# devmentality/LEAStereo

Hardware: AMD Instinct MI355X
Metric: stereo pairs/s at 576×960 D=192, 1/2/4/8 GPU; EPE vs reference (higher is better)
Workload: dtype f32; 1 GPU; SceneFlow 576x960 D=192 fp32, batch 1 per GPU (BASELINE configs[1]); height=576, width=960, maxdisp=192, global_batch=1, parallelism=dp1 (pairs sharded over ranks, no collective in the step), launch=hip graph replay

## Files before the change

### include/leastereo_hip.h

```cpp
#ifndef LEASTEREO_HIP_H
#define LEASTEREO_HIP_H

#include <stddef.h>
#include <stdint.h>

#ifdef __cplusplus
extern "C" {
#endif

#define LEA_ABI_VERSION 14

#define LEA_F32 0
#define LEA_BF16 1

#define LEA_OK 0
#define LEA_E_INVALID 1001
#define LEA_E_UNSUPPORTED 1002

#define LEA_RELU 1u
#define LEA_RESIDUAL 2u
#define LEA_PAIR_SUM 4u

int lea_abi_version(void);
const char* lea_last_error(void);
// ... 107 lines not shown
                             const uint8_t* exclude, int64_t exclude_bstride, int B, int C,
                             int H, int W, float c1, float c2, const double* sums,
                             const float* scales, float* ddisp, int64_t ddisp_bstride,
                             void* stream);

size_t lea_disparity_refine_workspace_bytes(int B, int H, int W);
int lea_disparity_refine_f32(const float* guide, int64_t guide_bstride, const float* disp,
                             const float* conf, const uint8_t* exclude, int B, int C, int H,
                             int W, float lambda, float sigma, int iterations, void* workspace,
                             float* refined, float* support, void* stream);

#define LEA_LR_SPECKLE 3
size_t lea_disparity_speckle_workspace_bytes(int B, int H, int W);
int lea_disparity_speckle_f32(const float* disp, const uint8_t* exclude, int B, int H, int W,
                              float max_diff, int max_size, float fill, void* workspace,
                              int32_t* labels, int32_t* size, uint8_t* state, float* filtered,
                              void* stream);


size_t lea_conv3d_packed_elems_bf16(int cout, int cin, int k);
int lea_conv3d_pack_weights_bf16(const float* w, void* packed, int cout, int cin, int k,
                                 void* stream);

int lea_conv3d_bnrelu_bf16(const void* x, int64_t x_bstride, const void* x2, int64_t x2_bstride,
                           int cin2, const void* w_packed, const float* scale, const float* shift,
                           const void* residual, int64_t r_bstride, void* y, int64_t y_bstride,
                           int B, int cin, int cout, int D, int H, int W, int k, unsigned flags,
                           void* stream);

int lea_conv3d_bnrelu_costvolume_bf16(const void* left, const void* right, int64_t f_bstride,
                                      const void* w_packed, const float* scale, const float* shift,
                                      void* y, int64_t y_bstride, int B, int C, int cout, int D3,
                                      int H, int W, unsigned flags, void* stream);


const char* lea_conv3d_kernel_name_bf16(int B, int cout, int cin, int D, int H, int W, int k,
                                        int costvolume);

int lea_conv3d_bf16_pair_supported(int B, int cin, int cout, int D, int H, int W);

int lea_conv1x1_resampled_bf16(const void* x, int64_t x_bstride, int Di, int Hi, int Wi,
                               const void* w_packed, const float* scale, const float* shift,
                               void* y, int64_t y_bstride, int B, int cin, int cout, int D, int H,
                               int W, unsigned flags, void* stream);

int lea_resample3d_trilinear_bf16(const void* x, int64_t x_bstride, void* y, int64_t y_bstride,
                                  int B, int C, int Di, int Hi, int Wi, int Do, int Ho, int Wo,
                                  int align_corners, const float* scale, const float* shift,
                                  unsigned flags, void* stream);


int lea_to_c8_bf16(const float* x, int64_t x_bstride, void* y, int64_t y_bstride, int B, int C,
                   int64_t vol, void* stream);
int lea_from_c8_bf16(const void* x, int64_t x_bstride, float* y, int64_t y_bstride, int B, int C,
                     int64_t vol, void* stream);


size_t lea_conv2d_packed_elems_bf16(int cout, int cin);
int lea_conv2d_pack_weights_bf16(const float* w, void* packed, int cout, int cin, void* stream);
int lea_conv2d_bnrelu_bf16(const void* x, int64_t x_bstride, const void* w_packed,
                           const float* scale, const float* shift, const void* residual,
                           int64_t r_bstride, void* y, int64_t y_bstride, int B, int cin, int cout,
                           int H, int W, unsigned flags, void* stream);

size_t lea_conv3d_wino_packed_floats(int cout, int cin);
int lea_conv3d_wino_pack_weights(const float* w, float* packed, int cout, int cin, void* stream);
int lea_conv3d_bnrelu_wino(const void* x, int64_t x_bstride, const void* x2, int64_t x2_bstride,
                           int cin2, const float* w_packed, const float* scale, const float* shift,
                           const void* residual, int64_t r_bstride, void* y, int64_t y_bstride,
                           int B, int cin, int cout, int D, int H, int W, unsigned flags, int dtype,
                           void* stream);
int lea_conv3d_bnrelu_costvolume_wino(const void* left, const void* right, int64_t f_bstride,
                                      const float* w_packed, const float* scale,
                                      const float* shift, void* y, int64_t y_bstride, int B, int C,
                                      int cout, int D3, int H, int W, unsigned flags, int dtype,
                                      void* stream);
const char* lea_conv3d_wino_kernel_name(int B, int cin, int cout, int D, int H, int W, int costvolume);
int lea_conv3d_wino_down2_supported(int B, int cin, int cout, int D, int H, int W);
const char* lea_conv3d_wino_down2_kernel_name(int B, int cin, int cout, int D, int H, int W);
int lea_conv3d_bnrelu_wino_down2(const void* x, int64_t x_bstride, const float* w_packed,
                                 const float* scale, const float* shift, void* y, int64_t y_bstride,
                                 int B, int cin, int cout, int D, int H, int W, unsigned flags, int dtype,
                                 void* stream);

int lea_cv_stem_split_weights(const float* w, float* wl, float* wr, int cout, int C, void* stream);
int lea_cv_stem_combine(const void* lmaps, int64_t l_bstride, const void* rmaps, int64_t r_bstride,
                        const float* scale, const float* shift, void* y, int64_t y_bstride, int B,
                        int cout, int D3, int H, int W, unsigned flags, int dtype, void* stream);
int lea_cv_stem_down2_supported(int cout, int D3, int H, int W, int dtype);
int lea_cv_stem_combine_down2(const void* lmaps, int64_t l_bstride, const void* rmaps, int64_t r_bstride,
                              const float* scale, const float* shift, void* y, int64_t y_bstride,
                              void* y2, int64_t y2_bstride, int B, int cout, int D3, int H, int W,
                              unsigned flags, int dtype, void* stream);


size_t lea_standardize_workspace_bytes(int B);
int lea_standardize_crop_u8(const void* left, const void* right, int B, int H, int W,
                            int pix_stride, float* out_left, float* out_right, int crop_h,
                            int crop_w, void* workspace, void* stream);

size_t lea_train_transform_workspace_bytes(int B);
int lea_train_transform_u8(const void* left, const void* right, int B, int H, int W, int pix_stride,
                           const float* disp_left, const float* disp_right, const int* params,
                           float* out_left, float* out_right, float* out_target, int crop_h,
                           int crop_w, float maxdisp, int* n_valid, void* workspace, void* stream);


size_t lea_standardize_tiles_workspace_bytes(void);
int lea_standardize_tiles_u8(const void* left, const void* right, int H, int W, int pix_stride,
                             const int* origins, int N, float* out_left, float* out_right, int tile_h,
                             int tile_w, void* workspace, void* stream);

int lea_tile_blend_f32(const float* tiles, int64_t tile_bstride, const int* ys, int ny, const int* xs,
                       int nx, int tile_h, int tile_w, int guard_y0, int guard_y1, int guard_x0,
                       int guard_x1, int ramp, float* out, int H, int W, int* n_uncovered, void* stream);

size_t lea_disparity_metrics_workspace_bytes(int B, int H, int W);
int lea_disparity_metrics(const float* pred, int64_t pred_bstride, const float* gt,
                          int64_t gt_bstride, int B, int H, int W, float maxdisp, int round_pred,
                          int z_shift, int thr1, int thr2, int thr3, unsigned char* correct,
                          double* out, void* workspace, void* stream);


size_t lea_conv3d_wgrad_workspace_bytes(int B, int cin, int cout, int D, int H, int W, int k);
int lea_conv3d_wgrad(const float* x, const float* dz, float* dw, void* workspace, size_t ws_bytes,
                     int B, int cin, int cout, int D, int H, int W, int k, void* stream);

size_t lea_conv2d_wgrad_workspace_bytes(int B, int cin, int cout, int H, int W);
int lea_conv2d_wgrad(const float* x, const float* dz, float* dw, void* workspace, size_t ws_bytes,
                     int B, int cin, int cout, int H, int W, void* stream);

int lea_conv2d_s3_backward_data(const float* dz, const float* w, float* dx, int B, int cin, int cout,
                                int Hi, int Wi, void* stream);
size_t lea_conv2d_s3_wgrad_workspace_bytes(int B, int cin, int cout, int Hi, int Wi);
int lea_conv2d_s3_wgrad(const float* x, const float* dz, float* dw, void* workspace, size_t ws_bytes,
                        int B, int cin, int cout, int Hi, int Wi, void* stream);

int lea_conv3d_flip_weights(const float* w, float* wt, int cout, int cin, int k, void* stream);

size_t lea_bn_workspace_bytes(int C);
int lea_bn_forward_f32(const float* z, float* y, int B, int C, int64_t V, const float* gamma,
                       const float* beta, float* running_mean, float* running_var, float momentum,
                       float eps, int training, unsigned flags, float* mean, float* invstd,
                       void* workspace, void* stream);

int lea_bn_backward_f32(const float* dy, const float* y, const float* z, float* dz, int B, int C,
                        int64_t V, const float* gamma, const float* mean, const float* invstd,
                        int training, unsigned flags, float* dgamma, float* dbeta, void* workspace,
                        void* stream);

size_t lea_resample3d_backward_workspace_bytes(int B, int C, int Di, int Hi, int Wi, int Do, int Ho,
                                               int Wo);
int lea_resample3d_trilinear_backward(const float* dy, float* dx, void* workspace, size_t ws_bytes,
                                      int B, int C, int Di, int Hi, int Wi, int Do, int Ho, int Wo,
                                      int align_corners, void* stream);

int lea_disparity_regression_backward(const float* cost, const float* disp, const float* dout,
                                      float* dV, int B, int D3, int H3, int W3, int maxdisp,
                                      void* stream);

int lea_build_cost_volume_backward(const float* dcost, float* dleft, float* dright, int B, int C,
                                   int H, int W, int D3, void* stream);

#ifdef __cplusplus
}
#endif
// ... 2 lines not shown
```

### leastereo_amd/_lib.py

```python
from __future__ import annotations

import ctypes
import os
import threading

LIB_PATH = os.environ.get(
    "LEASTEREO_HIP_LIB",
    os.path.join(os.path.dirname(os.path.abspath(__file__)), "libleastereo_hip.so"))

ABI_VERSION = 14
LEA_F32 = 0
LEA_BF16 = 1
LEA_RELU = 1
LEA_RESIDUAL = 2
LEA_PAIR_SUM = 4
LEA_E_INVALID = 1001

_p = ctypes.c_void_p
_i = ctypes.c_int
_i64 = ctypes.c_int64
_u = ctypes.c_uint

SIGNATURES = {
    "lea_abi_version": (_i, []),
    "lea_last_error": (ctypes.c_char_p, []),
    "lea_build_cost_volume": (_i, [_p, _p, _p, _i, _i, _i, _i, _i, _i, _p]),
    "lea_conv3d_packed_floats": (ctypes.c_size_t, [_i, _i, _i]),
    "lea_conv3d_pack_weights": (_i, [_p, _p, _i, _i, _i, _p]),
    "lea_conv3d_bnrelu": (_i, [_p, _i64, _p, _i64, _i, _p, _p, _p, _p, _i64, _p, _i64,
                               _i, _i, _i, _i, _i, _i, _i, _u, _i, _p]),
    "lea_conv3d_bnrelu_resampled": (_i, [_p, _i64, _i, _i, _i, _p, _p, _p, _p, _i64, _p, _i64,
                                         _i, _i, _i, _i, _i, _i, _i, _u, _i, _p]),
    "lea_conv3d_kernel_name": (ctypes.c_char_p, [_i, _i, _i, _i, _i, _i, _i]),
    "lea_conv3d_set_tile_override": (_i, [_i, _i, _i]),
    "lea_conv3d_bnrelu_costvolume": (_i, [_p, _p, _i64, _p, _p, _p, _p, _i64, _i, _i, _i, _i, _i,
                                          _i, _u, _i, _p]),
    "lea_conv3d_costvolume_kernel_name": (ctypes.c_char_p, [_i, _i, _i, _i, _i]),
    "lea_conv2d_packed_floats": (ctypes.c_size_t, [_i, _i]),
    "lea_conv2d_pack_weights": (_i, [_p, _p, _i, _i, _p]),
    "lea_conv2d_bnrelu": (_i, [_p, _i64, _p, _p, _p, _p, _i64, _p, _i64, _i, _i, _i, _i, _i, _u,
                               _i, _p]),
    "lea_conv2d_kernel_name": (ctypes.c_char_p, [_i, _i, _i, _i]),
    "lea_conv2d_s3_bnrelu": (_i, [_p, _i64, _p, _p, _p, _p, _i64, _i, _i, _i, _i, _i, _u, _i, _p]),
    "lea_feature_stem_bnrelu": (_i, [_p, _i64, _p, _p, _p, _p, _p, _p, _p, _i64, _i, _i, _i, _i, _i, _i,
                                     _i, _p]),
    "lea_resample3d_trilinear": (_i, [_p, _i64, _p, _i64, _i, _i, _i, _i, _i, _i, _i, _i,
                                      _i, _p, _p, _u, _i, _p]),
    "lea_tapsum_workspace_bytes": (ctypes.c_size_t, [_i, _i, _i, _i, _i]),
    "lea_tapsum_upsample": (_i, [_p, _i64, _p, _i64, _i, _i, _i, _i, _i, _i, _i, _i, _p, _p, _u,
                                 _p, _i, _p]),
    "lea_disparity_regression": (_i, [_p, _p, _i, _i, _i, _i, _i, _i, _p]),
    "lea_disparity_regression_stats": (_i, [_p, _p, _p, _p, _p, _i, _i, _i, _i, _i, _i, _i, _p]),
    "lea_disparity_regression_right": (_i, [_p, _p, _i, _i, _i, _i, _i, _i, _p]),
    "lea_disparity_lr_check": (_i, [_p, _p, _p, _p, _i, _i, _i, ctypes.c_float, _p]),
    "lea_median5x5_f32": (_i, [_p, _i64, _p, _i64, _i, _i, _i, _i, _p]),
    "lea_edge_loss_workspace_bytes": (ctypes.c_size_t, [_i, _i, _i]),
    "lea_edge_loss_f32": (_i, [_p, _i64, _p, _i64, _p, _i64, _i, _i, _i, ctypes.c_float, _p, _p, _p]),
    "lea_edge_loss_grad_f32": (_i, [_p, _i64, _p, _i64, _p, _i64, _p, _p, _p, _i64, _i, _i, _i,
                                    ctypes.c_float, _p]),
    "lea_photometric_workspace_bytes": (ctypes.c_size_t, [_i, _i, _i]),
    "lea_photometric_f32": (_i, [_p, _i64, _p, _i64, _p, _i64, _p, _i64, _i, _i, _i, _i, ctypes.c_float,
                                 ctypes.c_float, ctypes.c_float, _p, _p, _p, _p, _p]),
    "lea_photometric_grad_f32": (_i, [_p, _i64, _p, _i64, _p, _i64, _p, _i64, _i, _i, _i, _i, ctypes.c_float,
                                      ctypes.c_float, _p, _p, _p, _i64, _p]),
    "lea_disparity_refine_workspace_bytes": (ctypes.c_size_t, [_i, _i, _i]),
    "lea_disparity_refine_f32": (_i, [_p, _i64, _p, _p, _p, _i, _i, _i, _i, ctypes.c_float, ctypes.c_float, _i,
                                      _p, _p, _p, _p]),
    "lea_disparity_speckle_workspace_bytes": (ctypes.c_size_t, [_i, _i, _i]),
    "lea_disparity_speckle_f32": (_i, [_p, _p, _i, _i, _i, ctypes.c_float, _i, ctypes.c_float, _p, _p, _p, _p, _p,
                                       _p]),
    "lea_conv3d_packed_elems_bf16": (ctypes.c_size_t, [_i, _i, _i]),
    "lea_conv3d_pack_weights_bf16": (_i, [_p, _p, _i, _i, _i, _p]),
    "lea_conv3d_bnrelu_bf16": (_i, [_p, _i64, _p, _i64, _i, _p, _p, _p, _p, _i64, _p, _i64,
                                    _i, _i, _i, _i, _i, _i, _i, _u, _p]),
    "lea_conv3d_bnrelu_costvolume_bf16": (_i, [_p, _p, _i64, _p, _p, _p, _p, _i64, _i, _i, _i, _i,
                                               _i, _i, _u, _p]),
    "lea_conv3d_kernel_name_bf16": (ctypes.c_char_p, [_i, _i, _i, _i, _i, _i, _i, _i]),
    "lea_conv3d_bf16_pair_supported": (_i, [_i, _i, _i, _i, _i, _i]),
    "lea_conv3d_bf16_set_tile_override": (_i, [_i, _i, _i]),
    "lea_conv3d_bf16_set_variant": (_i, [_i]),
    "lea_resample3d_trilinear_bf16": (_i, [_p, _i64, _p, _i64, _i, _i, _i, _i, _i, _i, _i, _i,
                                           _i, _p, _p, _u, _p]),
    "lea_resample_bf16_set_batch": (_i, [_i]),
    "lea_resample_bf16_set_cols": (_i, [_i]),
    "lea_conv3d_wino_set_w22": (_i, [_i]),
    "lea_conv3d_bf16_set_pair_split": (_i, [_i]),
    "lea_disparity_set_register_form": (_i, [_i]),
    "lea_tapsum_set_rows": (_i, [_i]),
    "lea_staged_rows": (_i, [_i, _i, _i, _i, _i]),
    "lea_conv1x1_resampled_bf16": (_i, [_p, _i64, _i, _i, _i, _p, _p, _p, _p, _i64, _i, _i, _i, _i, _i,
                                        _i, _u, _p]),
    "lea_to_c8_bf16": (_i, [_p, _i64, _p, _i64, _i, _i, _i64, _p]),
    "lea_conv2d_packed_elems_bf16": (ctypes.c_size_t, [_i, _i]),
    "lea_conv2d_pack_weights_bf16": (_i, [_p, _p, _i, _i, _p]),
    "lea_conv2d_bnrelu_bf16": (_i, [_p, _i64, _p, _p, _p, _p, _i64, _p, _i64, _i, _i, _i, _i, _i,
                                    _u, _p]),
    "lea_from_c8_bf16": (_i, [_p, _i64, _p, _i64, _i, _i, _i64, _p]),
    "lea_conv3d_wino_packed_floats": (ctypes.c_size_t, [_i, _i]),
    "lea_conv3d_wino_pack_weights": (_i, [_p, _p, _i, _i, _p]),
    "lea_conv3d_bnrelu_wino": (_i, [_p, _i64, _p, _i64, _i, _p, _p, _p, _p, _i64, _p, _i64,
                                    _i, _i, _i, _i, _i, _i, _u, _i, _p]),
    "lea_conv3d_bnrelu_costvolume_wino": (_i, [_p, _p, _i64, _p, _p, _p, _p, _i64, _i, _i, _i,
                                               _i, _i, _i, _u, _i, _p]),
    "lea_conv3d_wino_kernel_name": (ctypes.c_char_p, [_i, _i, _i, _i, _i, _i, _i]),
    "lea_conv3d_wino_down2_supported": (_i, [_i, _i, _i, _i, _i, _i]),
    "lea_conv3d_wino_down2_kernel_name": (ctypes.c_char_p, [_i, _i, _i, _i, _i, _i]),
    "lea_conv3d_bnrelu_wino_down2": (_i, [_p, _i64, _p, _p, _p, _p, _i64, _i, _i, _i, _i, _i, _i, _u, _i, _p]),
    "lea_conv3d_wino_set_tile_override": (_i, [_i, _i, _i]),
    "lea_conv3d_wino_set_variant": (_i, [_i]),
    "lea_conv3d_wino2_set_walk": (_i, [_i]),
    "lea_conv3d_wino2_set_halo16": (_i, [_i]),
    "lea_conv3d_wino2_set_lane_halo16": (_i, [_i]),
    "lea_conv3d_wino_set_fence": (_i, [_i]),
    "lea_resample_set_mode": (_i, [_i]),
    "lea_conv2d_set_small": (_i, [_i]),
    "lea_conv2d_kernel_name_cin": (ctypes.c_char_p, [_i, _i, _i, _i, _i]),
    "lea_conv2d_bnrelu_pair": (_i, [_p, _i64, _p, _p, _p, _p, _i64, _p, _i64, _p, _i64, _i, _i, _i, _i, _i,
                                    _i, _u, _p]),
    "lea_conv3d_wino2_set_pipeline": (_i, [_i]),
    "lea_conv3d_wino2p_set_wpre": (_i, [_i]),
    "lea_conv3d_wino44_set": (_i, [_i]),
    "lea_conv3d_wino44_set_upre": (_i, [_i]),
    "lea_conv3d_wino44_set_sched": (_i, [_i]),
    "lea_conv3d_wino44_set_group": (_i, [_i]),
    "lea_conv3d_wino_set_epi_buf": (_i, [_i]),
    "lea_conv3d_set_rs_gather": (_i, [_i]),
    "lea_conv1x1_set_vector": (_i, [_i]),
    "lea_conv3d_bf16_set_stream1x1": (_i, [_i]),
    "lea_conv3d_wino_set_small_cout": (_i, [_i]),
    "lea_conv3d_wino_set_block48": (_i, [_i]),
    "lea_cv_stem_split_weights": (_i, [_p, _p, _p, _i, _i, _p]),
    "lea_cv_stem_combine": (_i, [_p, _i64, _p, _i64, _p, _p, _p, _i64, _i, _i, _i, _i, _i, _u, _i,
                                 _p]),
    "lea_cv_stem_down2_supported": (_i, [_i, _i, _i, _i, _i]),
    "lea_cv_stem_combine_down2": (_i, [_p, _i64, _p, _i64, _p, _p, _p, _i64, _p, _i64, _i, _i, _i, _i, _i,
                                       _u, _i, _p]),
    "lea_standardize_workspace_bytes": (ctypes.c_size_t, [_i]),
    "lea_standardize_crop_u8": (_i, [_p, _p, _i, _i, _i, _i, _p, _p, _i, _i, _p, _p]),
    "lea_train_transform_workspace_bytes": (ctypes.c_size_t, [_i]),
    "lea_train_transform_u8": (_i, [_p, _p, _i, _i, _i, _i, _p, _p, _p, _p, _p, _p, _i, _i,
                                    ctypes.c_float, _p, _p, _p]),
    "lea_standardize_tiles_workspace_bytes": (ctypes.c_size_t, []),
    "lea_standardize_tiles_u8": (_i, [_p, _p, _i, _i, _i, _p, _i, _p, _p, _i, _i, _p, _p]),
    "lea_tile_blend_f32": (_i, [_p, _i64, _p, _i, _p, _i, _i, _i, _i, _i, _i, _i, _i, _p, _i, _i, _p, _p]),
    "lea_disparity_metrics_workspace_bytes": (ctypes.c_size_t, [_i, _i, _i]),
    "lea_disparity_metrics": (_i, [_p, _i64, _p, _i64, _i, _i, _i, ctypes.c_float, _i, _i,
                                   _i, _i, _i, _p, _p, _p, _p]),
    "lea_conv3d_wgrad_workspace_bytes": (ctypes.c_size_t, [_i, _i, _i, _i, _i, _i, _i]),
    "lea_conv3d_wgrad": (_i, [_p, _p, _p, _p, ctypes.c_size_t, _i, _i, _i, _i, _i, _i, _i, _p]),
    "lea_conv2d_wgrad_workspace_bytes": (ctypes.c_size_t, [_i, _i, _i, _i, _i]),
    "lea_conv2d_wgrad": (_i, [_p, _p, _p, _p, ctypes.c_size_t, _i, _i, _i, _i, _i, _p]),
    "lea_conv2d_s3_backward_data": (_i, [_p, _p, _p, _i, _i, _i, _i, _i, _p]),
    "lea_conv2d_s3_wgrad_workspace_bytes": (ctypes.c_size_t, [_i, _i, _i, _i, _i]),
    "lea_conv2d_s3_wgrad": (_i, [_p, _p, _p, _p, ctypes.c_size_t, _i, _i, _i, _i, _i, _p]),
    "lea_conv3d_flip_weights": (_i, [_p, _p, _i, _i, _i, _p]),
    "lea_bn_workspace_bytes": (ctypes.c_size_t, [_i]),
    "lea_bn_forward_f32": (_i, [_p, _p, _i, _i, _i64, _p, _p, _p, _p, ctypes.c_float, ctypes.c_float,
                                _i, _u, _p, _p, _p, _p]),
    "lea_bn_backward_f32": (_i, [_p, _p, _p, _p, _i, _i, _i64, _p, _p, _p, _i, _u, _p, _p, _p, _p]),
    "lea_disparity_regression_backward": (_i, [_p, _p, _p, _p, _i, _i, _i, _i, _i, _p]),
    "lea_build_cost_volume_backward": (_i, [_p, _p, _p, _i, _i, _i, _i, _i, _p]),
    "lea_resample3d_backward_workspace_bytes": (ctypes.c_size_t, [_i, _i, _i, _i, _i, _i, _i, _i]),
    "lea_resample3d_trilinear_backward": (_i, [_p, _p, _p, ctypes.c_size_t, _i, _i, _i, _i, _i, _i, _i, _i,
                                               _i, _p]),
}

_lib = None
_lock = threading.Lock()


class HipKernelError(RuntimeError):
    pass


def load():
    global _lib
    if _lib is not None:
        return _lib
    with _lock:
        if _lib is None:
            if not os.path.exists(LIB_PATH):
                raise HipKernelError(
                    f"{LIB_PATH} not found: build it with `make` (hipcc --offload-arch=gfx950); "
                    "the LEAStereo hot path has no fallback")
            lib = ctypes.CDLL(LIB_PATH)
            for name, (res, args) in SIGNATURES.items():
                fn = getattr(lib, name)
                fn.restype = res
                fn.argtypes = args
            _apply_env_tuning(lib)
# ... 38 lines not shown
```

### leastereo_amd/csrc/conv3d_wino.hip

```cpp
#include "wino_common.h"

namespace lea {
namespace wino {

template <int F, int Q, int MT, int NP, int TD, bool H16 = false>
struct Cfg {
  static constexpr bool DP = MT == 0;
  static constexpr int MTE = DP ? 1 : MT;
  static constexpr int TDA = DP ? 1 : TD;
  static constexpr int NSTEP = DP ? 12 : 9;
  static_assert(!DP || TD == 2, "a depth-paired tile covers two output planes");
  static constexpr int NX = F + 2;
  static constexpr int COP = 16 * MTE;
  static constexpr bool SWZ = (COP % 32) == 0;
  static constexpr int RPG = 16 / Q;
  static constexpr int TW = F * Q;
  static constexpr int TH = 4 * NP * RPG;
  static constexpr int RH = TH + 2, RW = TW + 2;
  static constexpr int PLANE = RH * RW;
  static constexpr int PLANES = TD + 2;
  static constexpr int IMG = PLANES * PLANE;
  static constexpr int XSLOTS = (IMG + 63) / 64;
  static constexpr int CIS = conflict_free_cis<F, Q>(64 * XSLOTS, RW);
  static constexpr int RWA = TW + 8;
  static constexpr int PLANEA = RH * RWA;
  static constexpr int IMGA = PLANES * PLANEA;
  static constexpr int BLK16 = IMGA / 4;
  static constexpr int PIECES16 = (BLK16 + 63) / 64;
  static constexpr int cb2(int c) {
    int base = 1;
    for (int k = 1; k <= c; ++k) {
      const int want = (k & 1 ? 2 : 0) + (k & 2 ? 32 : 0) + 1, lo = base + IMGA;
      base = lo + ((want - lo) % 64 + 64) % 64;
    }
    return base;
  }
  static_assert(!H16 || (Q == 16 && F == 4), "16-byte halo: one tile row per lane group");
  static constexpr int CSH = PIECES16 * 256;
  static constexpr int cbh(int c) { return 1 + c * CSH; }
  static_assert(!H16 || (CSH % 64 == 0 && RWA % 4 == 0 && PLANEA % 4 == 0), "b128 halo map");
  static constexpr int XS = H16 ? (cbh(CIN_B) + 3) / 4 * 4 : CIN_B * CIS;
  static constexpr int RWX = H16 ? RWA : RW;
  static constexpr int PLX = H16 ? PLANEA : PLANE;
  static constexpr int WS = NSTEP * 3 * CIN_B * COP;
  static constexpr int WSLOTS = (WS + 255) / 256;
  static constexpr int STAGE = XS + 256 * WSLOTS;
  static_assert(XS % 4 == 0 && WS % 4 == 0 && RW % 2 == 0 && PLANE % 2 == 0, "aligned LDS regions and b64 reads");
  static_assert(2 * STAGE * 4 * 2 <= 160 * 1024, "two double-buffered workgroups per CU");
};

template <int F, int Q, int MT, int NP, int TD, bool CV, bool H16 = false, bool FENCE = false>
__global__ __launch_bounds__(kConvThreads, 2) void conv3d_wino_kernel(const ConvArgs a) {
  using C = Cfg<F, Q, MT, NP, TD, H16>;
  static_assert(!(CV && H16), "16-byte halo: plain volumes only");
  constexpr int NX = C::NX;
  constexpr int XSLOTS = C::XSLOTS;
  constexpr int XSLOTS_W = (XSLOTS + kConvWaves - 1) / kConvWaves;
  constexpr int WSLOTS = C::WSLOTS;
  constexpr int WSLOTS_W = (WSLOTS + kConvWaves - 1) / kConvWaves;
  __shared__ __attribute__((aligned(16))) float smem[2 * C::STAGE];
  const unsigned lds0 = lds_addr(smem);

  const int tid = threadIdx.x;
  const int lane = tid & 63;
  const int wave = __builtin_amdgcn_readfirstlane(tid >> 6);
  const int nblk = a.nblk;
  const int xcd = blockIdx.x % 8, idx = blockIdx.x / 8;
  const int q8 = nblk / 8, r8 = nblk % 8;
  const int lin = (xcd < r8 ? xcd * (q8 + 1) : r8 * (q8 + 1) + (xcd - r8) * q8) + idx;
  const int spw = a.spw > 0 ? a.spw : 1;
  const int ngz = (a.ndz + spw - 1) / spw;
  const int cob = lin % a.ncob;
  const int rest = lin / a.ncob;
  const int gz = rest % ngz;
  const int tile = (rest / ngz) % a.ntiles;
  const int b = rest / (ngz * a.ntiles);
  const int h0 = (tile / a.tiles_w) * C::TH;
  const int w0 = (tile % a.tiles_w) * C::TW;
  const int dz0 = gz * spw, ngroups = min(spw, a.ndz - dz0);
  const int co0 = cob * C::COP;
  const int nchunks = a.cin / CIN_B;
  const int nitems = ngroups * nchunks;
  const float* wp = a.wp + (long long)cob * nchunks * C::WS;
  const int HW = a.H * a.W;
  const unsigned nrec = (unsigned)(HW * a.D) * 4u;

  unsigned hwo[XSLOTS_W];
  int pln[XSLOTS_W], wco[CV ? XSLOTS_W : 1];
#pragma unroll
  for (int t = 0; t < XSLOTS_W; ++t) {
    const int e = (wave + kConvWaves * t) * 64 + lane;
    unsigned v = 0xFFFFFFF0u;
    int pl = -1000, wc_ = 0;
    if (e < C::IMG) {
      const int p = e / C::PLANE;
      const int r = e - p * C::PLANE;
      const int rr = r / C::RW;
      const int cc = r - rr * C::RW;
      const int h = h0 + rr - 1, w = w0 + cc - 1;
      if ((unsigned)h < (unsigned)a.H && (unsigned)w < (unsigned)a.W) {
        v = (unsigned)(h * a.W + w) * 4u;
        pl = p - 1;
        wc_ = w;
      }
    }
    hwo[t] = v;
    pln[t] = pl;
    if constexpr (CV) wco[t] = wc_;
  }
  unsigned voff[XSLOTS_W], voffr[CV ? XSLOTS_W : 1];
  constexpr int P16 = C::PIECES16, T16 = H16 ? (CIN_B * P16 + kConvWaves - 1) / kConvWaves : 1;
  unsigned hwo16[T16], voff16[T16];
  int pln16[T16];
  bool ok16[T16];
  if constexpr (H16) {
#pragma unroll
    for (int t = 0; t < T16; ++t) {
      const int k = wave + kConvWaves * t, e = 64 * (k % P16) + lane;
      ok16[t] = k < CIN_B * P16 && e < C::BLK16;
      const int p = e / (C::RH * (C::RWA / 4)), r = e - p * (C::RH * (C::RWA / 4));
      const int rr = r / (C::RWA / 4), blk = r - rr * (C::RWA / 4);
      const int h = h0 + rr - 1, w = w0 - 4 + 4 * blk;
      const bool in = ok16[t] && (unsigned)h < (unsigned)a.H && (unsigned)w < (unsigned)a.W;
      hwo16[t] = in ? (unsigned)(h * a.W + w) * 4u : 0xFFFFFFF0u;
      pln16[t] = in ? p - 1 : -1000;
    }
  }
  auto set_group = [&](int d0) {
    if constexpr (H16) {
#pragma unroll
      for (int t = 0; t < T16; ++t) {
        const int d = d0 + pln16[t];
        voff16[t] = (hwo16[t] != 0xFFFFFFF0u && (unsigned)d < (unsigned)a.D)
                        ? hwo16[t] + (unsigned)d * (unsigned)HW * 4u : 0xFFFFFFF0u;
      }
      return;
    }
#pragma unroll
    for (int t = 0; t < XSLOTS_W; ++t) {
      const int d = d0 + pln[t];
      const bool ok = hwo[t] != 0xFFFFFFF0u && (unsigned)d < (unsigned)a.D;
      if constexpr (CV) {
        const bool okc = ok && wco[t] >= d;
// ... 71 lines not shown
  for (int m = 0; m < C::MTE; ++m)
#pragma unroll
    for (int r = 0; r < 4; ++r) {
      const int co = C::DP ? 4 * (ci & 1) + r : co0 + 16 * m + 4 * ci + r;
      const bool cv = co < a.cout;
      sc[m][r] = (cv && a.scale) ? a.scale[co] : 1.f;
      sh[m][r] = (cv && a.shift) ? a.shift[co] : 0.f;
    }

  f32x4 acc[NX][C::TDA][C::MTE][NP];
#pragma unroll
  for (int x = 0; x < NX; ++x)
#pragma unroll
    for (int t = 0; t < C::TDA; ++t)
#pragma unroll
      for (int m = 0; m < C::MTE; ++m)
#pragma unroll
        for (int j = 0; j < NP; ++j) acc[x][t][m][j] = f32x4{0.f, 0.f, 0.f, 0.f};

  const bool relu = a.flags & LEA_RELU, resid = a.flags & LEA_RESIDUAL;
  const long long DHW = (long long)HW * a.D;
  const int w = w0 + F * pq;
  const bool ebuf = F == 4 && (a.flags & kEpiBuf);
  constexpr int NST = C::TDA * NP * C::MTE * 4;
  const int nco = C::DP ? a.cout : min(C::COP, a.cout - co0);
  const __amdgpu_buffer_rsrc_t yrs = block_rsrc(a.y + (long long)b * a.ybs + (long long)co0 * DHW, nco * DHW * 4);
  const __amdgpu_buffer_rsrc_t rrs =
      block_rsrc((resid ? a.res : a.y) + (long long)b * (resid ? a.rbs : a.ybs) + (long long)co0 * DHW, nco * DHW * 4);
  auto epilogue_buf = [&](int d0) {
    unsigned off[C::TDA][NP][C::MTE][4];
#pragma unroll
    for (int t = 0; t < C::TDA; ++t)
#pragma unroll
      for (int j = 0; j < NP; ++j)
#pragma unroll
        for (int m = 0; m < C::MTE; ++m)
#pragma unroll
          for (int r = 0; r < 4; ++r) {
            const int d = C::DP ? d0 + (ci >> 1) : d0 + t;
            const int h = h0 + (wave * NP + j) * C::RPG + pr;
            const int cr = C::DP ? 4 * (ci & 1) + r : 16 * m + 4 * ci + r;
            off[t][j][m][r] = (d < a.D && h < a.H && w < a.W && cr < nco)
                                  ? (unsigned)(cr * DHW + (long long)d * HW + h * a.W + w) * 4u
                                  : kEpiOob;
          }
    f32x4 rv[C::TDA][NP][C::MTE][4];
    if (resid) {
#pragma unroll
      for (int t = 0; t < C::TDA; ++t)
#pragma unroll
        for (int j = 0; j < NP; ++j)
#pragma unroll
          for (int m = 0; m < C::MTE; ++m)
#pragma unroll
            for (int r = 0; r < 4; ++r) rv[t][j][m][r] = buf_load4(rrs, off[t][j][m][r]);
    }
#pragma unroll
    for (int t = 0; t < C::TDA; ++t)
#pragma unroll
      for (int j = 0; j < NP; ++j)
#pragma unroll
        for (int m = 0; m < C::MTE; ++m)
#pragma unroll
          for (int r = 0; r < 4; ++r) {
            constexpr int X3 = NX > 4 ? 3 : 0, X4 = NX > 4 ? 4 : 0;
            const float m0 = 0.25f * acc[0][t][m][j][r];
            const float m1 = (-1.f / 6.f) * acc[1][t][m][j][r], m2 = (-1.f / 6.f) * acc[2][t][m][j][r];
            const float m3 = (1.f / 24.f) * acc[X3][t][m][j][r], m4 = (1.f / 24.f) * acc[X4][t][m][j][r];
            const float m5 = acc[NX - 1][t][m][j][r];
            const float sp = m1 + m2, sm = m1 - m2, tp = m3 + m4, tm = m3 - m4;
            f32x4 y;
            y[0] = (m0 + sp) + tp;
            y[1] = fmaf(2.f, tm, sm);
            y[2] = fmaf(4.f, tp, sp);
            y[3] = fmaf(8.f, tm, sm) + m5;
#pragma unroll
            for (int e = 0; e < 4; ++e) {
              float v = y[e] * sc[m][r] + sh[m][r];
              if (relu) v = fmaxf(v, 0.f);
              y[e] = resid ? v + rv[t][j][m][r][e] : v;
            }
            buf_store4(yrs, off[t][j][m][r], y);
          }
  };
  auto epilogue = [&](int d0) {
#pragma unroll
  for (int t = 0; t < C::TDA; ++t) {
    const int d = C::DP ? d0 + (ci >> 1) : d0 + t;
#pragma unroll
    for (int j = 0; j < NP; ++j) {
      const int h = h0 + (wave * NP + j) * C::RPG + pr;
      if (d >= a.D || h >= a.H || w >= a.W) continue;
      const int nv = min(F, a.W - w);
#pragma unroll
      for (int m = 0; m < C::MTE; ++m)
#pragma unroll
        for (int r = 0; r < 4; ++r) {
          const int co = C::DP ? 4 * (ci & 1) + r : co0 + 16 * m + 4 * ci + r;
          if (co >= a.cout) continue;
          float y[F];
          if constexpr (F == 2) {
            const float m0 = acc[0][t][m][j][r], m1 = 0.5f * acc[1][t][m][j][r];
            const float m2 = 0.5f * acc[2][t][m][j][r], m3 = acc[3][t][m][j][r];
            y[0] = (m0 + m1) + m2;
            y[1] = (m1 - m2) - m3;
          } else {
            const float m0 = 0.25f * acc[0][t][m][j][r];
            const float m1 = (-1.f / 6.f) * acc[1][t][m][j][r], m2 = (-1.f / 6.f) * acc[2][t][m][j][r];
            const float m3 = (1.f / 24.f) * acc[3][t][m][j][r], m4 = (1.f / 24.f) * acc[4][t][m][j][r];
            const float m5 = acc[NX - 1][t][m][j][r];
            const float sp = m1 + m2, sm = m1 - m2, tp = m3 + m4, tm = m3 - m4;
            y[0] = (m0 + sp) + tp;
            y[1] = fmaf(2.f, tm, sm);
            y[F / 2] = fmaf(4.f, tp, sp);
            y[F - 1] = fmaf(8.f, tm, sm) + m5;
          }
#pragma unroll
          for (int e = 0; e < F; ++e) {
            y[e] = y[e] * sc[m][r] + sh[m][r];
            if (relu) y[e] = fmaxf(y[e], 0.f);
          }
          const long long o = (long long)co * DHW + (long long)d * HW + (long long)h * a.W + w;
          float* yp = a.y + (long long)b * a.ybs + o;
          const float* rp = a.res + (long long)b * a.rbs + o;
          const bool vec = nv == F &&
              ((reinterpret_cast<uintptr_t>(yp) | (resid ? reinterpret_cast<uintptr_t>(rp) : 0)) & (4 * F - 1)) == 0;
          if (vec) {
            if constexpr (F == 2) {
              if (resid) {
                const float2 rv = *reinterpret_cast<const float2*>(rp);
                y[0] += rv.x;
                y[1] += rv.y;
              }
              *reinterpret_cast<float2*>(yp) = make_float2(y[0], y[1]);
            } else {
              if (resid) {
                const float4 rv = *reinterpret_cast<const float4*>(rp);
                y[0] += rv.x;
                y[1] += rv.y;
                y[F / 2] += rv.z;
                y[F - 1] += rv.w;
              }
              *reinterpret_cast<float4*>(yp) = make_float4(y[0], y[1], y[F / 2], y[F - 1]);
            }
          } else {
#pragma unroll
            for (int e = 0; e < F; ++e)
              if (e < nv) {
                if (resid) y[e] += rp[e];
                yp[e] = y[e];
              }
          }
        }
    }
  }
  };

  issue(0, smem);
  for (int it = 0; it < nitems; ++it) {
    const int ch = it % nchunks;
    wait_item<NST>(ebuf && ch == 0 && it > 0);
    __syncthreads();
    if (it + 1 < nitems) issue(it + 1, smem + ((it + 1) & 1) * C::STAGE);
    const float* xs = smem + (it & 1) * C::STAGE;
    const float* ws = xs + C::XS;
    struct StepOps {
      float2 x2[C::TDA][NP][F / 2 + 1];
      float g[3][C::MTE];
    };
    auto load_step = [&](int step, StepOps& o) {
      const int kd = step / 3, kh = step % 3;
#pragma unroll
      for (int t = 0; t < C::TDA; ++t)
#pragma unroll
        for (int j = 0; j < NP; ++j) {
          const float* sp = xs + xoff[j] + (t + kd) * C::PLX + kh * C::RWX;
          if constexpr (H16) {
            const float4 lo = *reinterpret_cast<const float4*>(sp);
            typedef const volatile __attribute__((address_space(3))) f32x4 lds_f32x4;
            const f32x4 hi = *(lds_f32x4*)(sp + 4);
            o.x2[t][j][0] = make_float2(lo.x, lo.y);
            o.x2[t][j][1] = make_float2(lo.z, lo.w);
            o.x2[t][j][2] = make_float2(hi[0], hi[1]);
            continue;
          }
#pragma unroll
          for (int q = 0; q <= F / 2; ++q) o.x2[t][j][q] = *reinterpret_cast<const float2*>(sp + 2 * q);
        }
      const float* wk = ws + step * 3 * CIN_B * C::COP;
#pragma unroll
      for (int m = 0; m < C::MTE; ++m)
#pragma unroll
        for (int r = 0; r < 3; ++r) o.g[r][m] = wk[r * CIN_B * C::COP + woff[m]];
    };
    struct Xf {
      float vb[C::TDA][NP][NX];
      float u[NX][C::MTE];
    };
    auto xform = [&](const StepOps& o, Xf& T) {
#pragma unroll
      for (int t = 0; t < C::TDA; ++t)
#pragma unroll
        for (int j = 0; j < NP; ++j) {
          const float x0 = o.x2[t][j][0].x, x1 = o.x2[t][j][0].y, x2 = o.x2[t][j][1].x, x3 = o.x2[t][j][1].y;
          if constexpr (F == 2) {
            T.vb[t][j][0] = x0 - x2;
            T.vb[t][j][1] = x1 + x2;
            T.vb[t][j][2] = x2 - x1;
            T.vb[t][j][3] = x1 - x3;
          } else {
            const float x4 = o.x2[t][j][F / 2].x, x5 = o.x2[t][j][F / 2].y;
            const float pa = fmaf(-4.f, x2, x4), pb = fmaf(-4.f, x1, x3);
            const float pc = x4 - x2, pd = 2.f * (x3 - x1);
            T.vb[t][j][0] = fmaf(4.f, x0, fmaf(-5.f, x2, x4));
            T.vb[t][j][1] = pa + pb;
            T.vb[t][j][2] = pa - pb;
            T.vb[t][j][3] = pc + pd;
            T.vb[t][j][4] = pc - pd;
            T.vb[t][j][NX - 1] = fmaf(4.f, x1, fmaf(-5.f, x3, x5));
          }
        }
#pragma unroll
      for (int m = 0; m < C::MTE; ++m) {
        const float g0 = o.g[0][m], g1 = o.g[1][m], g2 = o.g[2][m];
        const float s = g0 + g2;
        T.u[0][m] = g0;
        T.u[1][m] = s + g1;
        T.u[2][m] = s - g1;
        if constexpr (F == 4) {
          const float s4 = fmaf(4.f, g2, g0);
          T.u[3][m] = fmaf(2.f, g1, s4);
          T.u[4][m] = fmaf(-2.f, g1, s4);
        }
        T.u[NX - 1][m] = g2;
      }
    };
    auto mfmas = [&](const Xf& T) {
#pragma unroll
      for (int x = 0; x < NX; ++x)
#pragma unroll
        for (int t = 0; t < C::TDA; ++t)
#pragma unroll
          for (int m = 0; m < C::MTE; ++m)
#pragma unroll
            for (int j = 0; j < NP; ++j)
              acc[x][t][m][j] = __builtin_amdgcn_mfma_f32_16x16x4f32(T.u[x][m], T.vb[t][j][x], acc[x][t][m][j], 0, 0, 0);
    };
    StepOps ops[2];
    Xf xf[2];
    if constexpr (FENCE) {
      load_step(0, ops[0]);
      xform(ops[0], xf[0]);
      load_step(1, ops[1]);
#pragma unroll
      for (int step = 0; step < C::NSTEP; ++step) {
        __builtin_amdgcn_sched_barrier(0);
        mfmas(xf[step & 1]);
        __builtin_amdgcn_sched_barrier(0);
        if (step + 1 < C::NSTEP) xform(ops[(step + 1) & 1], xf[(step + 1) & 1]);
        if (step + 2 < C::NSTEP) load_step(step + 2, ops[step & 1]);
      }
    } else {
    __builtin_amdgcn_iglp_opt(0);
    load_step(0, ops[0]);
    load_step(1, ops[1]);
    xform(ops[0], xf[0]);
#pragma unroll
    for (int step = 0; step < C::NSTEP; ++step) {
      if (step + 1 < C::NSTEP) xform(ops[(step + 1) & 1], xf[(step + 1) & 1]);
      if (step + 2 < C::NSTEP) load_step(step + 2, ops[step & 1]);
      mfmas(xf[step & 1]);
    }
    }
    if (ch == nchunks - 1) {
      if (ebuf)
        epilogue_buf((dz0 + it / nchunks) * TD);
      else
        epilogue((dz0 + it / nchunks) * TD);
#pragma unroll
      for (int x = 0; x < NX; ++x)
#pragma unroll
        for (int t = 0; t < C::TDA; ++t)
#pragma unroll
          for (int m = 0; m < C::MTE; ++m)
#pragma unroll
            for (int j = 0; j < NP; ++j) acc[x][t][m][j] = f32x4{0.f, 0.f, 0.f, 0.f};
    }
  }
}

template <int MT>
__global__ void pack_wino_kernel(const float* __restrict__ w, float* __restrict__ packed, int cout,
                                 int cin, int nchunks, long long total) {
  constexpr int COP = 16 * MT;
  constexpr bool SWZ = (COP % 32) == 0;
  for (long long i = blockIdx.x * (long long)blockDim.x + threadIdx.x; i < total;
       i += (long long)gridDim.x * blockDim.x) {
    long long q = i;
    const int col = (int)(q % COP); q /= COP;
    const int ci = (int)(q % CIN_B); q /= CIN_B;
    const int kw = (int)(q % 3); q /= 3;
    const int kdkh = (int)(q % 9); q /= 9;
    const int ch = (int)(q % nchunks);
    const int cb = (int)(q / nchunks);
    const int mm = col / 16, n = col % 16;
    const int m = SWZ ? (mm ^ (ci & 1)) : mm;
    const int co = cb * COP + 16 * m + n;
    const int c = ch * CIN_B + ci;
    packed[i] = (co < cout && c < cin) ? w[(((long long)co * cin + c) * 9 + kdkh) * 3 + kw] : 0.f;
  }
}

__global__ void pack_wino_dp_kernel(const float* __restrict__ w, float* __restrict__ packed, int cout,
                                    int cin, int nchunks, long long total) {
  for (long long i = blockIdx.x * (long long)blockDim.x + threadIdx.x; i < total;
       i += (long long)gridDim.x * blockDim.x) {
    long long q = i;
    const int col = (int)(q % 16); q /= 16;
    const int ci = (int)(q % CIN_B); q /= CIN_B;
    const int kw = (int)(q % 3); q /= 3;
    const int step = (int)(q % 12); q /= 12;
    const int ch = (int)q;
    const int co = col & 7, kd = step / 3 - (col >> 3), kh = step % 3;
    const int c = ch * CIN_B + ci;
    packed[i] = (ch < nchunks && co < cout && c < cin && kd >= 0 && kd <= 2)
                    ? w[(((long long)co * cin + c) * 9 + kd * 3 + kh) * 3 + kw]
                    : 0.f;
  }
}

struct Plan {
  int f, q, mt, np, td;
  bool d2;
  Plan2 p2;
  bool h16;
};

int g_override[3] = {0, 0, 0};
int g_variant = 0;
int g_spw = 0;
int g_small16 = 0;
int g_block48 = 1;
int g_epibuf = 1;
int g_halo16 = 1;
int g_pipe = 1;
int g_wpre = 1;
int g_fence = 1;
int g_lane16 = 2;
int g_w22 = 0;
inline int host_mt(int cout) {
  if (g_small16 && cout <= 8) return 1;
  const int mt = mt_of(cout);
  return (mt == 3 && !g_block48) ? 2 : mt;
}
inline long long staged_floats(int cout, int cin) {
  const int mt = host_mt(cout), cop = cop_of(mt), nstep = mt == 0 ? 12 : 9;
  return (long long)((cout + cop - 1) / cop) * (cin / CIN_B) * nstep * 3 * CIN_B * cop + 256;
}
inline bool has_u22(int cout) { return cout <= 32; }
inline bool has_l44(int cout) { return host_mt(cout) == 1 || host_mt(cout) == 2; }
inline long long l44_offset(int cout, int cin) {
  return staged_floats(cout, cin) + (host_mt(cout) == 2 ? lane_weights_floats(cout, cin) : 0);
}
inline long long u22_offset(int cout, int cin) {
  return l44_offset(cout, cin) + (has_l44(cout) ? lane44_floats(cout, cin) : 0);
}

inline Plan2 plan2(int v, int mt, int q) {
  Plan2 t{0, 0, 0, 0, 0, 0, 0};
  if (mt != 1 && mt != 2) return t;
  if (v >= 5) {
// ... 347 lines not shown
  LEA_CHECK_ARG(spw >= 0 && spw <= 64, "lea_conv3d_wino2_set_walk: spw=%d", spw);
  wino::g_spw = spw;
  return 0;
}

extern "C" int lea_conv3d_wino_set_w22(int on) {
  clear_error();
  LEA_CHECK_ARG(on >= 0 && on <= 2, "lea_conv3d_wino_set_w22: on=%d", on);
  wino::g_w22 = on;
  return 0;
}

extern "C" int lea_conv3d_wino_set_variant(int variant) {
  clear_error();
  LEA_CHECK_ARG(variant >= 0 && variant <= 7, "lea_conv3d_wino_set_variant: bad variant %d", variant);
  wino::g_variant = variant;
  return 0;
}

extern "C" int lea_conv3d_bnrelu_wino(const void* x, int64_t x_bstride, const void* x2,
                                      int64_t x2_bstride, int cin2, const float* w_packed,
                                      const float* scale, const float* shift, const void* residual,
                                      int64_t r_bstride, void* y, int64_t y_bstride, int B, int cin,
                                      int cout, int D, int H, int W, unsigned flags, int dtype,
                                      void* stream) {
  clear_error();
  ConvArgs a{};
  a.x = (const float*)x;
  a.xbs = x_bstride;
  a.x2 = (const float*)x2;
  a.x2bs = x2_bstride;
  a.cin1 = cin - cin2;
  a.wp = w_packed;
  a.scale = scale;
  a.shift = shift;
  a.res = (const float*)residual;
  a.rbs = r_bstride;
  a.y = (float*)y;
  a.ybs = y_bstride;
  a.cin = cin;
  a.cout = cout;
  a.D = D;
  a.H = H;
  a.W = W;
  a.flags = flags;
  LEA_CHECK_FLAGS(flags, LEA_RELU | LEA_RESIDUAL | LEA_PAIR_SUM, "lea_conv3d_bnrelu_wino");
  LEA_CHECK_ARG(cin2 >= 0 && cin2 <= cin && (cin2 == 0 || x2), "lea_conv3d_bnrelu_wino: bad second source");
  return wino::common(a, B, false, dtype, stream);
}

extern "C" int lea_conv3d_bnrelu_costvolume_wino(const void* left, const void* right,
                                                 int64_t f_bstride, const float* w_packed,
                                                 const float* scale, const float* shift, void* y,
                                                 int64_t y_bstride, int B, int C, int cout, int D3,
                                                 int H, int W, unsigned flags, int dtype,
                                                 void* stream) {
  clear_error();
  ConvArgs a{};
  a.x = (const float*)left;
  a.xbs = f_bstride;
  a.x2 = (const float*)right;
  a.x2bs = f_bstride;
  a.cin1 = C;
  a.wp = w_packed;
  a.scale = scale;
  a.shift = shift;
  a.y = (float*)y;
  a.ybs = y_bstride;
  a.cin = 2 * C;
  a.cout = cout;
  a.D = D3;
  a.H = H;
  a.W = W;
  a.flags = flags & LEA_RELU;
  LEA_CHECK_FLAGS(flags, LEA_RELU, "lea_conv3d_bnrelu_costvolume_wino");
  LEA_CHECK_ARG(left && right && y != left && y != right,
                "lea_conv3d_bnrelu_costvolume_wino: null or aliased pointer");
  return wino::common(a, B, true, dtype, stream);
}

namespace lea {
namespace wino {

static bool down2_plan(int B, int cin, int cout, int D, int H, int W, ConvArgs* a, Plan2* out) {
  if (B <= 0 || cin <= 0 || cout <= 0 || D < 2 || H < 2 || W < 4 || D % 2 || H % 2 || W % 4 || cin % CIN_B)
    return false;
  if ((long long)D * H * W * 4 >= (1LL << 32) || (long long)(cout + 47) * D * H * W >= (1LL << 31)) return false;
  Plan p = make_plan(B, cout, D, H, W);
  if (g_w22 && (p.mt == 1 || (g_w22 == 2 && cout <= 32)) && g_variant == 0 && g_override[0] == 0) return false;
  plan_halo16(p, false, W, a, cin);
  if (!p.d2 || !g_w44 || g_w44u || g_w44s != 0 || !has_l44(cout)) return false;
  const Plan2& q = p.p2;
  if (!(q.q == 8 && q.wc == 2 && q.mte == 1 && q.nw == 4 && q.occ == 2 && q.pv == 3)) return false;
  if (out) *out = q;
  return true;
}

}
}

extern "C" int lea_conv3d_wino_down2_supported(int B, int cin, int cout, int D, int H, int W) {
  return wino::down2_plan(B, cin, cout, D, H, W, nullptr, nullptr) ? 1 : 0;
}

extern "C" const char* lea_conv3d_wino_down2_kernel_name(int B, int cin, int cout, int D, int H, int W) {
  return wino::down2_plan(B, cin, cout, D, H, W, nullptr, nullptr) ? "conv3d_wino44_down2_kernel" : nullptr;
}

extern "C" int lea_conv3d_bnrelu_wino_down2(const void* x, int64_t x_bstride, const float* w_packed,
                                            const float* scale, const float* shift, void* y,
                                            int64_t y_bstride, int B, int cin, int cout, int D, int H, int W,
                                            unsigned flags, int dtype, void* stream) {
  clear_error();
  ConvArgs a{};
  a.x = (const float*)x;
  a.xbs = x_bstride;
  a.cin1 = cin;
  a.wp = w_packed;
  a.scale = scale;
  a.shift = shift;
  a.y = (float*)y;
  a.ybs = y_bstride;
  a.cin = cin;
  a.cout = cout;
  a.D = D;
  a.H = H;
  a.W = W;
  LEA_CHECK_ARG(a.x && a.wp && a.y, "lea_conv3d_bnrelu_wino_down2: null pointer");
  LEA_CHECK_ARG((scale == nullptr) == (shift == nullptr),
                "lea_conv3d_bnrelu_wino_down2: scale/shift must both be set or both NULL");
  LEA_CHECK_ARG(B > 0 && cin > 0 && cout > 0 && D > 0 && H > 0 && W > 0,
                "lea_conv3d_bnrelu_wino_down2: bad shape B=%d cin=%d cout=%d D=%d H=%d W=%d", B, cin, cout, D, H, W);
  if (flags & (LEA_RESIDUAL | LEA_PAIR_SUM)) {
    set_error("lea_conv3d_bnrelu_wino_down2: LEA_RESIDUAL / LEA_PAIR_SUM are not supported with the "
              "down-sampling epilogue");
    return LEA_E_UNSUPPORTED;
  }
  LEA_CHECK_FLAGS(flags, LEA_RELU, "lea_conv3d_bnrelu_wino_down2");
  a.flags = flags;
  LEA_CHECK_ARG(D % 2 == 0 && H % 2 == 0 && W % 4 == 0,
                "lea_conv3d_bnrelu_wino_down2: D and H must be even and W %% 4 == 0 (D=%d H=%d W=%d)", D, H, W);
  LEA_CHECK_ARG(cin % wino::CIN_B == 0, "lea_conv3d_bnrelu_wino_down2: cin %d must be a multiple of %d", cin,
                wino::CIN_B);
  LEA_CHECK_ARG(a.x != a.y, "lea_conv3d_bnrelu_wino_down2: input aliases output");
  if (dtype != LEA_F32) {
    set_error("lea_conv3d_bnrelu_wino_down2: dtype %d unsupported", dtype);
    return LEA_E_UNSUPPORTED;
  }
  LEA_CHECK_ARG(((uintptr_t)y & 15) == 0 && y_bstride % 4 == 0,
                "lea_conv3d_bnrelu_wino_down2: y needs 16-byte alignment");
  wino::Plan2 q;
  if (!wino::down2_plan(B, cin, cout, D, H, W, &a, &q)) {
    set_error("lea_conv3d_bnrelu_wino_down2: the planner does not put B=%d cin=%d cout=%d D=%d H=%d W=%d on "
              "the F(4,3) x F(4,3) tile (or its settings / the operands' alignment rule it out)",
              B, cin, cout, D, H, W);
    return LEA_E_UNSUPPORTED;
  }
  a.rd = axis_ratio(D, D / 2, 1);
  a.rh = axis_ratio(H, H / 2, 1);
  a.rw = axis_ratio(W, W / 2, 1);
  a.uoff = wino::l44_offset(cout, cin);
  return wino::run44(a, B, q.spw, as_stream(stream), true);
}
```

### leastereo_amd/csrc/conv3d_wino44.hip

```cpp
#include <type_traits>

#include "wino_common.h"

namespace lea {
namespace wino {

namespace w44 {
constexpr int Q = 8, F = 4, TW = 32, TH = 2, TD = 4, PLANES = 6, RH = TH + 2, RWA = TW + 8;
constexpr int PLANEA = RH * RWA;
constexpr int BLK16 = PLANES * PLANEA / 4;
constexpr int CB0 = 1, CB1 = CB0 + 1024 + 2, CB2 = CB1 + 1024 + 30, CB3 = CB2 + 1024 + 2;
constexpr int XS = (CB3 + 1024 + 3) / 4 * 4;
constexpr int GS = 40, XHS = 20, TRS = 320, TCS = 1284, TS = 4 * TCS;
constexpr int KGL = 28;
constexpr int KGU = 56;
constexpr int NST = 8;
constexpr int NSTD = 2;
static_assert(CB1 % 64 == 3 && CB2 % 64 == 33 && CB3 % 64 == 35, "V-pass bank map");
static_assert(BLK16 <= 4 * 64 && 4 * 256 <= CB1 - CB0, "whole pieces per channel region");
static_assert(TRS % 64 == 0 && TCS % 8 == 4 && GS % 8 == 0 && XHS % 4 == 0 && TRS >= Q * GS && TCS >= RH * TRS,
              "V bank map");
static_assert(4 * 64 * 20 <= TS && 4 * 64 * 16 <= XS, "epilogue exchange fits a V and a halo buffer");
static_assert((2 * XS + 2 * TS) * 4 * 2 <= 160 * 1024, "two workgroups per CU");
}
// ... 438 lines not shown
                               o.v4[3].x, o.v4[3].y, o.v4[3].z, o.v4[3].w, o.v2[0], o.v2[1]};
  #pragma unroll
        for (int x = 0; x < NX; ++x)
  #pragma unroll
          for (int e = 0; e < NE; ++e) T.v[x][e] = e18[x * 6 + e];
        if constexpr (UPRE) {
          const float* u = reinterpret_cast<const float*>(gw) + kh * 18;
  #pragma unroll
          for (int x = 0; x < NX; ++x)
  #pragma unroll
            for (int e = 0; e < NE; ++e) T.u[x][e] = u[x * 6 + e];
        } else {
          const float* g = reinterpret_cast<const float*>(gw) + kh * 9;
  #pragma unroll
          for (int x = 0; x < NX; ++x) {
            const float g0 = g[x], g1 = g[3 + x], g2 = g[6 + x];
            const float s = g0 + g2, s4 = fmaf(4.f, g2, g0);
            T.u[x][0] = g0;
            T.u[x][1] = s + g1;
            T.u[x][2] = s - g1;
            T.u[x][3] = fmaf(2.f, g1, s4);
            T.u[x][4] = fmaf(-2.f, g1, s4);
            T.u[x][5] = g2;
          }
        }
      };
      auto mfmas = [&](const Xf& T) {
  #pragma unroll
        for (int x = 0; x < NX; ++x)
  #pragma unroll
          for (int e = 0; e < NE; ++e)
            acc[x][e] = __builtin_amdgcn_mfma_f32_16x16x4f32(T.u[x][e], T.v[x][e], acc[x][e], 0, 0, 0);
      };
      Raw raw[2];
      Xf xf[2];
      if constexpr (SCHED != 2) __builtin_amdgcn_iglp_opt(0);
      load_step(0, raw[0]);
      load_step(1, raw[1]);
      xform(0, raw[0], xf[0]);
      issue_halo(hch, hqd, it & 1);
      load_step(2, raw[0]);
      xform(1, raw[1], xf[1]);
      mfmas(xf[0]);
      if constexpr (SCHED == 0 || SCHED == 2) vpass(XHC, (it + 1) & 1);
      xform(2, raw[0], xf[0]);
      load_g(it + 1 < nitems ? (ich + 1 == nchunks ? 0 : ich + 1) : ich);
      mfmas(xf[1]);
      if constexpr (SCHED == 1) vpass(XHC, (it + 1) & 1);
      mfmas(xf[0]);
      if constexpr (SCHED == 3) vpass(XHC, (it + 1) & 1);
      after_epi = false;
      if (ich == nchunks - 1) {
        epilogue_xh(XHC, (pz0 + iqd) * TD, tvb + (it & 1) * TS, halo + ((it + 1) & 1) * XS);
        after_epi = true;
  #pragma unroll
        for (int x = 0; x < NX; ++x)
  #pragma unroll
          for (int e = 0; e < NE; ++e) acc[x][e] = f32x4{0.f, 0.f, 0.f, 0.f};
      }
      if (++ich == nchunks) {
        ich = 0;
        ++iqd;
      }
      if (it + 3 < nitems && ++hch == nchunks) {
        hch = 0;
        ++hqd;
      }
    }
  };
  if (xh == 0)
    run(std::integral_constant<int, 0>{});
  else
    run(std::integral_constant<int, 1>{});
  asm volatile("s_waitcnt vmcnt(0)" ::: "memory");
}

template <bool UPRE, int SCHED>
__global__ __launch_bounds__(256, 2) void conv3d_wino44_kernel(const ConvArgs a) {
  conv3d_wino44_body<UPRE, SCHED, false>(a);
}
__global__ __launch_bounds__(256, 2) void conv3d_wino44_down2_kernel(const ConvArgs a) {
  conv3d_wino44_body<false, 0, true>(a);
}

int g_w44 = 2;
int g_w44u = 0;
int g_w44s = 0;
int g_w44g = -1;

int run44(ConvArgs a, int B, int spw, hipStream_t st, bool down) {
  a.ncob = (a.cout + 31) / 32;
  a.tiles_w = (a.W + w44::TW - 1) / w44::TW;
  a.ntiles = a.tiles_w * ((a.H + w44::TH - 1) / w44::TH);
  a.ndz = (a.D + w44::TD - 1) / w44::TD;
  a.spw = std::max(1, std::min(spw > 0 ? spw : auto_walk(a, B, 2), a.ndz));
  const long long n_ = (long long)a.ntiles * ((a.ndz + a.spw - 1) / a.spw) * B * a.ncob;
  LEA_CHECK_ARG(n_ < (1LL << 31), "lea_conv3d(wino44): grid too large");
  a.nblk = (int)n_;
  a.grp = g_w44g >= 0 ? g_w44g : (n_ >= 2048 ? 16 : 0);
  const dim3 grid((unsigned)n_);
  if (down) {
    conv3d_wino44_down2_kernel<<<grid, 256, 0, st>>>(a);
    return launch_status("lea_conv3d(wino44 down2)");
  }
  if (g_w44u)
    conv3d_wino44_kernel<true, 0><<<grid, 256, 0, st>>>(a);
  else if (g_w44s == 1)
    conv3d_wino44_kernel<false, 1><<<grid, 256, 0, st>>>(a);
  else if (g_w44s == 2)
    conv3d_wino44_kernel<false, 2><<<grid, 256, 0, st>>>(a);
  else if (g_w44s == 3)
    conv3d_wino44_kernel<false, 3><<<grid, 256, 0, st>>>(a);
  else
    conv3d_wino44_kernel<false, 0><<<grid, 256, 0, st>>>(a);
  return launch_status("lea_conv3d(wino44)");
}

}
}
```

### leastereo_amd/csrc/cv_stem.hip

```cpp
#include "common.h"

namespace lea {
namespace cvs {

using bf16x8 = __attribute__((ext_vector_type(8))) __bf16;
constexpr int kThreads = 256;
constexpr int WS = 64;

struct Args {
  const void* lk;
  long long lbs;
  const void* rk;
  long long rbs;
  const float* scale;
  const float* shift;
  void* y;
  long long ybs;
  int cout, D, H, W, nseg, ncob;
  int nds, dchunk;
  unsigned flags;
  float* y2;
  long long y2bs;
  float rd, rh, rw;
};

constexpr int kLdsBytes = 80 * 1024;

__device__ __forceinline__ int stage_u(int p, int NU, int u0, int w0, int D) {
  return p < NU ? u0 + p : (p < NU + WS ? w0 + p - NU : w0 + p - NU - WS - (D - 1));
}
__device__ __forceinline__ float stage_sum(int p, int NU, const float bz[3]) {
  return p < NU ? bz[0] + bz[1] + bz[2] : (p < NU + WS ? bz[1] + bz[2] : bz[0] + bz[1]);
}
__device__ __forceinline__ long long bz_offset(int kd, int z, int o, int cout, long long HW, int W) {
  return (z >= 0 && z < W) ? (long long)(kd * cout + o) * HW + z : (long long)((3 + kd) * cout + o) * HW;
}
__device__ __forceinline__ bool bz_valid(int z, int W) { return z >= -1 && z < W; }
__device__ __forceinline__ bool plane_valid(int d, int kd, int D) {
  return d + kd - 1 >= 0 && d + kd - 1 < D;
}

__device__ __forceinline__ float left_sum(const float lk[3][3], int d, int u, int D) {
  float s = 0.f;
#pragma unroll
  for (int kd = 0; kd < 3; ++kd) {
    const int t = kd - u;
    const float v = t <= 0 ? lk[kd][0] : (t == 1 ? lk[kd][1] : (t == 2 ? lk[kd][2] : 0.f));
    if (plane_valid(d, kd, D)) s += v;
  }
  return s;
}

struct Tile {
  int D, H, W, NU, NT, h, cob, b, d0, d1, w0, u0;
  long long HW;
};

__device__ __forceinline__ Tile tile_of(const Args& a, int rows) {
  Tile t;
  t.D = a.D;
  t.H = a.H;
  t.W = a.W;
  t.NU = a.dchunk + WS - 1;
  t.NT = t.NU + 2 * WS;
  int blk = blockIdx.x;
  const int seg = blk % a.nseg;
  blk /= a.nseg;
  const int ds = blk % a.nds;
  blk /= a.nds;
  t.h = blk % rows;
  blk /= rows;
  t.cob = blk % a.ncob;
  t.b = blk / a.ncob;
  t.d0 = ds * a.dchunk;
  t.d1 = min(a.D, t.d0 + a.dchunk);
  t.w0 = seg * WS;
  t.u0 = t.w0 - (t.d0 + a.dchunk - 1);
  t.HW = (long long)a.H * a.W;
  return t;
}

constexpr int OB = 16;

__device__ __forceinline__ void stage_row_f32(const Args& a, const Tile& T, const float* rkh, float* rs,
                                              float* corr) {
  const int D = T.D, W = T.W, NU = T.NU, NT = T.NT, d0 = T.d0, d1 = T.d1, w0 = T.w0;
  const long long HW = T.HW;
  const int tid = threadIdx.x;
  const int NE = OB * NT;
  for (int e0 = 0; e0 < NE; e0 += 4 * kThreads) {
    float q[4][3];
#pragma unroll
    for (int k = 0; k < 4; ++k) {
      const int e = min(e0 + k * kThreads + tid, NE - 1);
      const int ol = e / NT, p = e % NT;
      const int o = min(T.cob * OB + ol, a.cout - 1), u = stage_u(p, NU, T.u0, w0, D);
#pragma unroll
      for (int kd = 0; kd < 3; ++kd) q[k][kd] = rkh[bz_offset(kd, u - kd + 1, o, a.cout, HW, W)];
    }
#pragma unroll
    for (int k = 0; k < 4; ++k) {
      const int e = e0 + k * kThreads + tid;
      if (e >= NE) break;
      const int ol = e / NT, p = e % NT;
      const bool ok = T.cob * OB + ol < a.cout;
      const int u = stage_u(p, NU, T.u0, w0, D);
      float bz[3];
#pragma unroll
      for (int kd = 0; kd < 3; ++kd) bz[kd] = (ok && bz_valid(u - kd + 1, W)) ? q[k][kd] : 0.f;
      rs[e] = stage_sum(p, NU, bz);
    }
  }
  if (w0 + WS >= W) {
    const int dl = d1 - d0;
    for (int e = tid; e < OB * dl; e += kThreads) {
      const int ol = e / dl, d = d0 + e % dl;
      const int o = min(T.cob * OB + ol, a.cout - 1);
      float v[3];
#pragma unroll
      for (int kd = 0; kd < 3; ++kd) {
        const int x = min(max(W + 1 - d - kd, 0), W - 1);
        v[kd] = rkh[(long long)((3 + kd) * a.cout + o) * HW + x];
      }
      float s = 0.f;
#pragma unroll
      for (int kd = 0; kd < 3; ++kd) {
        const int x = W + 1 - d - kd;
        if (plane_valid(d, kd, D) && x >= 0 && x < W) s += v[kd];
      }
      corr[ol * a.dchunk + (d - d0)] = s;
    }
  }
}

__global__ __launch_bounds__(kThreads) void cv_stem_f32_kernel(const Args a) {
  extern __shared__ float rs[];
  const Tile T = tile_of(a, a.H);
  const int D = T.D, W = T.W, NU = T.NU, NT = T.NT, d0 = T.d0, d1 = T.d1, w0 = T.w0;
  const long long HW = T.HW;
  if (a.flags & 0x100u) {
    const int ol = threadIdx.x >> 4, o = T.cob * OB + ol, w = w0 + 4 * (threadIdx.x & 15);
    if (o >= a.cout || w >= W) return;
    float* yp = static_cast<float*>(a.y) + T.b * a.ybs + (long long)o * D * HW + (long long)T.h * W + w;
    for (int d = d0; d < d1; ++d) *reinterpret_cast<float4*>(yp + (long long)d * HW) = make_float4(d, 0.f, 0.f, 1.f);
    return;
  }
  const float* lk = static_cast<const float*>(a.lk) + T.b * a.lbs;
  const float* rkh = static_cast<const float*>(a.rk) + T.b * a.rbs + (long long)T.h * W;
  float* corr = rs + OB * NT;
  const int tid = threadIdx.x;
  stage_row_f32(a, T, rkh, rs, corr);
  __syncthreads();

  const int ol = tid >> 4, o = T.cob * OB + ol;
  const int w = w0 + 4 * (tid & 15);
  if (o >= a.cout || w >= W) return;
  const bool band = w - (d1 - 1) <= 1;
  float lkv[3][3][4];
#pragma unroll
  for (int kd = 0; kd < 3; ++kd)
#pragma unroll
    for (int t = 0; t < 3; ++t) {
      float4 v = make_float4(0.f, 0.f, 0.f, 0.f);
      if (t == 0 || band)
        v = *reinterpret_cast<const float4*>(lk + (long long)((3 * kd + t) * a.cout + o) * HW +
                                             (long long)T.h * W + w);
      lkv[kd][t][0] = v.x;
      lkv[kd][t][1] = v.y;
      lkv[kd][t][2] = v.z;
      lkv[kd][t][3] = v.w;
    }
  const float sc = a.scale ? a.scale[o] : 1.f, sh = a.scale ? a.shift[o] : 0.f;
  const float lo = (a.flags & LEA_RELU) ? 0.f : -INFINITY;
  const float* r0 = rs + ol * NT;
  const float* cr = corr + ol * a.dchunk - d0;
  float* yp = static_cast<float*>(a.y) + T.b * a.ybs + (long long)o * D * HW + (long long)T.h * W + w;
  const int jedge = W - 1 - w;
  auto store = [&](int d, const float pre[4]) {
    float4 out;
    float* po = reinterpret_cast<float*>(&out);
#pragma unroll
    for (int j = 0; j < 4; ++j) {
      po[j] = fmaxf(pre[j] * sc + sh, lo);
    }
    *reinterpret_cast<float4*>(yp + (long long)d * HW) = out;
  };
  auto boundary = [&](int d, int pbase) {
    float pre[4];
#pragma unroll
    for (int j = 0; j < 4; ++j) {
      float l3[3][3];
#pragma unroll
      for (int kd = 0; kd < 3; ++kd)
#pragma unroll
        for (int t = 0; t < 3; ++t) l3[kd][t] = lkv[kd][t][j];
      pre[j] = left_sum(l3, d, w + j - d, D) + r0[pbase + (w - w0) + j] - (j == jedge ? cr[d] : 0.f);
    }
    store(d, pre);
  };
  if (d0 == 0) boundary(0, NU);
  if (d1 == D) boundary(D - 1, NU + WS);
  float gl[4], bl[4][4];
#pragma unroll
  for (int j = 0; j < 4; ++j) {
    float l3[3][3];
#pragma unroll
    for (int kd = 0; kd < 3; ++kd)
#pragma unroll
      for (int t = 0; t < 3; ++t) l3[kd][t] = lkv[kd][t][j];
    gl[j] = lkv[0][0][j] + lkv[1][0][j] + lkv[2][0][j];
#pragma unroll
    for (int m = 0; m < 4; ++m) bl[m][j] = left_sum(l3, 1, m - 2, D);
  }
  const int da = max(d0, 1), db = min(d1, D - 1);
  if (w0 - (db - 1) >= 2) {
    for (int d = da; d < db; ++d) {
      const int iu = w - d - T.u0;
      const float c = cr[d];
      float pre[4];
#pragma unroll
      for (int j = 0; j < 4; ++j) pre[j] = gl[j] + r0[iu + j] - (j == jedge ? c : 0.f);
      store(d, pre);
    }
    return;
  }
  for (int d = da; d < db; ++d) {
    const int iu = w - d - T.u0;
    const float c = cr[d];
    float pre[4];
#pragma unroll
    for (int j = 0; j < 4; ++j) {
      const int u = w + j - d;
      float l = u >= 2 ? gl[j] : 0.f;
#pragma unroll
      for (int m = 0; m < 4; ++m) l = u == m - 2 ? bl[m][j] : l;
      pre[j] = l + r0[iu + j] - (j == jedge ? c : 0.f);
    }
    store(d, pre);
  }
}

__device__ __forceinline__ float lerp2(float l0, float v0, float l1, float v1) {
#pragma clang fp contract(off)
  return l0 * v0 + l1 * v1;
}

__global__ __launch_bounds__(kThreads) void cv_stem_f32_down2_kernel(const Args a) {
  extern __shared__ float rs[];
  const Tile T = tile_of(a, a.H / 2);
  const int D = T.D, H = T.H, W = T.W, NU = T.NU, NT = T.NT, w0 = T.w0, hp = T.h;
  const long long HW = T.HW;
  const float* lk = static_cast<const float*>(a.lk) + T.b * a.lbs;
  const float* rk = static_cast<const float*>(a.rk) + T.b * a.rbs;
  const int rowf = OB * (NT + a.dchunk);
  const int tid = threadIdx.x;
#pragma unroll
  for (int r = 0; r < 2; ++r)
    stage_row_f32(a, T, rk + (long long)(2 * hp + r) * W, rs + r * rowf, rs + r * rowf + OB * NT);
  __syncthreads();

  const int ol = tid >> 4, o = T.cob * OB + ol;
  const int w = w0 + 4 * (tid & 15);
  if (o >= a.cout || w >= W) return;
  const bool band = w - (D - 1) <= 1;
  float gl[2][4], bl[2][4][4], lf[2][4], ll[2][4];
#pragma unroll
  for (int r = 0; r < 2; ++r) {
    float lkv[3][3][4];
#pragma unroll
    for (int kd = 0; kd < 3; ++kd)
#pragma unroll
      for (int t = 0; t < 3; ++t) {
        float4 v = make_float4(0.f, 0.f, 0.f, 0.f);
        if (t == 0 || band)
          v = *reinterpret_cast<const float4*>(lk + (long long)((3 * kd + t) * a.cout + o) * HW +
                                               (long long)(2 * hp + r) * W + w);
        lkv[kd][t][0] = v.x;
        lkv[kd][t][1] = v.y;
        lkv[kd][t][2] = v.z;
        lkv[kd][t][3] = v.w;
      }
#pragma unroll
    for (int j = 0; j < 4; ++j) {
      float l3[3][3];
#pragma unroll
      for (int kd = 0; kd < 3; ++kd)
#pragma unroll
        for (int t = 0; t < 3; ++t) l3[kd][t] = lkv[kd][t][j];
      gl[r][j] = lkv[0][0][j] + lkv[1][0][j] + lkv[2][0][j];
#pragma unroll
      for (int m = 0; m < 4; ++m) bl[r][m][j] = left_sum(l3, 1, m - 2, D);
      lf[r][j] = left_sum(l3, 0, w + j, D);
      ll[r][j] = left_sum(l3, D - 1, w + j - (D - 1), D);
    }
  }
  const float sc = a.scale ? a.scale[o] : 1.f, sh = a.scale ? a.shift[o] : 0.f;
  const float lo = (a.flags & LEA_RELU) ? 0.f : -INFINITY;
  const int jedge = W - 1 - w;
  const bool far = w0 - (D - 2) >= 2;
  float* yp = static_cast<float*>(a.y) + T.b * a.ybs + (long long)o * D * HW + (long long)(2 * hp) * W + w;
  const int D2 = D / 2, H2 = H / 2, W2 = W / 2;
  float* y2p = a.y2 + T.b * a.y2bs + ((long long)o * D2 * H2 + hp) * W2 + w / 2;
  Axis aw[2];
#pragma unroll
  for (int c = 0; c < 2; ++c) aw[c] = axis_index(a.rw, w / 2 + c, W, W2, 1);
  const Axis ah = axis_index(a.rh, hp, H, H2, 1);
  const bool h0odd = ah.i0 & 1, h1odd = ah.i1 & 1;

  float ev[2] = {0.f, 0.f};
  for (int d = 0; d < D; ++d) {
    float out[2][4];
#pragma unroll
    for (int r = 0; r < 2; ++r) {
      const float* r0 = rs + r * rowf + ol * NT;
      const float c = rs[r * rowf + OB * NT + ol * a.dchunk + d];
      float pre[4];
      if (d == 0 || d == D - 1) {
        const int pb = (d == 0 ? NU : NU + WS) + (w - w0);
#pragma unroll
        for (int j = 0; j < 4; ++j) pre[j] = (d == 0 ? lf[r][j] : ll[r][j]) + r0[pb + j] - (j == jedge ? c : 0.f);
      } else {
        const int iu = w - d - T.u0;
#pragma unroll
        for (int j = 0; j < 4; ++j) {
          const int u = w + j - d;
          float l = (far || u >= 2) ? gl[r][j] : 0.f;
          if (!far) {
#pragma unroll
            for (int m = 0; m < 4; ++m) l = u == m - 2 ? bl[r][m][j] : l;
          }
          pre[j] = l + r0[iu + j] - (j == jedge ? c : 0.f);
        }
      }
      float4 o4;
      float* po = reinterpret_cast<float*>(&o4);
#pragma unroll
      for (int j = 0; j < 4; ++j) {
        po[j] = fmaxf(pre[j] * sc + sh, lo);
        out[r][j] = po[j];
      }
      *reinterpret_cast<float4*>(yp + (long long)d * HW + r * W) = o4;
    }
    float hv[2];
#pragma unroll
    for (int c = 0; c < 2; ++c) {
      float wv[2];
#pragma unroll
      for (int r = 0; r < 2; ++r) {
        const float v0 = (aw[c].i0 & 1) ? out[r][2 * c + 1] : out[r][2 * c];
        const float v1 = (aw[c].i1 & 1) ? out[r][2 * c + 1] : out[r][2 * c];
        wv[r] = lerp2(aw[c].l0, v0, aw[c].l1, v1);
      }
      hv[c] = lerp2(ah.l0, h0odd ? wv[1] : wv[0], ah.l1, h1odd ? wv[1] : wv[0]);
    }
    if (!(d & 1)) {
      ev[0] = hv[0];
      ev[1] = hv[1];
    } else {
      const Axis ad = axis_index(a.rd, d >> 1, D, D2, 1);
      float2 o2;
      o2.x = lerp2(ad.l0, (ad.i0 & 1) ? hv[0] : ev[0], ad.l1, (ad.i1 & 1) ? hv[0] : ev[0]);
      o2.y = lerp2(ad.l0, (ad.i0 & 1) ? hv[1] : ev[1], ad.l1, (ad.i1 & 1) ? hv[1] : ev[1]);
      *reinterpret_cast<float2*>(y2p + (long long)(d >> 1) * H2 * W2) = o2;
    }
  }
}

constexpr int OB8 = 32;

__global__ __launch_bounds__(kThreads) void cv_stem_c8_kernel(const Args a) {
  extern __shared__ __attribute__((aligned(16))) float rs8[];
  const Tile T = tile_of(a, a.H);
  const int D = T.D, W = T.W, NU = T.NU, NT = T.NT, d0 = T.d0, d1 = T.d1, w0 = T.w0;
  const long long HW = T.HW;
  if (a.flags & 0x100u) {
    const int lb = threadIdx.x >> 6, cb = T.cob * (OB8 / 8) + lb, w = w0 + (threadIdx.x & 63);
    if (cb >= a.cout / 8 || w >= W) return;
    bf16x8* yp = reinterpret_cast<bf16x8*>(static_cast<__bf16*>(a.y) + T.b * a.ybs) +
                 (long long)cb * D * HW + (long long)T.h * W + w;
    bf16x8 z = {};
    for (int d = d0; d < d1; ++d) yp[(long long)d * HW] = z;
    return;
  }
  const __bf16* lk = static_cast<const __bf16*>(a.lk) + T.b * a.lbs;
  const __bf16* rk = static_cast<const __bf16*>(a.rk) + T.b * a.rbs;
  const int cbo = a.cout / 8;
  auto word = [&](const __bf16* m, int cb, int x) {
    return *reinterpret_cast<const bf16x8*>(m + ((long long)cb * HW + (long long)T.h * W + x) * 8);
  };
  float4* rs4 = reinterpret_cast<float4*>(rs8);
  float4* corr4 = rs4 + (OB8 / 8) * 2 * NT;
  const int tid = threadIdx.x;

  const int NE = (OB8 / 8) * NT;
  for (int e0 = 0; e0 < NE; e0 += 2 * kThreads) {
    bf16x8 q[2][3];
#pragma unroll
    for (int k = 0; k < 2; ++k) {
      const int e = min(e0 + k * kThreads + tid, NE - 1);
      const int lb = e / NT, p = e % NT;
      const int cb = min(T.cob * (OB8 / 8) + lb, cbo - 1), u = stage_u(p, NU, T.u0, w0, D);
#pragma unroll
      for (int kd = 0; kd < 3; ++kd) {
        const int z = u - kd + 1;
        q[k][kd] = (z >= 0 && z < W) ? word(rk, kd * cbo + cb, z) : word(rk, (3 + kd) * cbo + cb, 0);
      }
    }
#pragma unroll
    for (int k = 0; k < 2; ++k) {
      const int e = e0 + k * kThreads + tid;
      if (e >= NE) break;
      const int lb = e / NT, p = e % NT;
      const bool ok = T.cob * (OB8 / 8) + lb < cbo;
      const int u = stage_u(p, NU, T.u0, w0, D);
      float r[8];
#pragma unroll
      for (int j = 0; j < 8; ++j) {
        float bz[3];
#pragma unroll
        for (int kd = 0; kd < 3; ++kd) bz[kd] = (ok && bz_valid(u - kd + 1, W)) ? (float)q[k][kd][j] : 0.f;
        r[j] = stage_sum(p, NU, bz);
      }
      rs4[(lb * 2) * NT + p] = make_float4(r[0], r[1], r[2], r[3]);
      rs4[(lb * 2 + 1) * NT + p] = make_float4(r[4], r[5], r[6], r[7]);
    }
  }
  if (w0 + WS >= W) {
    const int dl = d1 - d0;
    for (int e = tid; e < (OB8 / 8) * dl; e += kThreads) {
      const int lb = e / dl, d = d0 + e % dl;
      const int cb = min(T.cob * (OB8 / 8) + lb, cbo - 1);
      bf16x8 v[3];
#pragma unroll
      for (int kd = 0; kd < 3; ++kd) v[kd] = word(rk, (3 + kd) * cbo + cb, min(max(W + 1 - d - kd, 0), W - 1));
      float s[8] = {0.f, 0.f, 0.f, 0.f, 0.f, 0.f, 0.f, 0.f};
#pragma unroll
      for (int kd = 0; kd < 3; ++kd) {
        const int x = W + 1 - d - kd;
        if (plane_valid(d, kd, D) && x >= 0 && x < W)
#pragma unroll
          for (int j = 0; j < 8; ++j) s[j] += (float)v[kd][j];
      }
      corr4[(lb * 2) * a.dchunk + (d - d0)] = make_float4(s[0], s[1], s[2], s[3]);
      corr4[(lb * 2 + 1) * a.dchunk + (d - d0)] = make_float4(s[4], s[5], s[6], s[7]);
    }
  }
// ... 161 lines not shown
  a.lbs = l_bstride;
  a.rk = rmaps;
  a.rbs = r_bstride;
  a.scale = scale;
  a.shift = shift;
  a.y = y;
  a.ybs = y_bstride;
  a.cout = cout;
  a.D = D3;
  a.H = H;
  a.W = W;
  LEA_CHECK_FLAGS(flags, LEA_RELU | 0x300u, "lea_cv_stem_combine");
  a.flags = flags & (LEA_RELU | 0x300u);
  a.nseg = (W + cvs::WS - 1) / cvs::WS;
  const int ob = dtype == LEA_F32 ? cvs::OB : cvs::OB8;
  a.dchunk = std::min(D3, (cvs::kLdsBytes / (int)sizeof(float) / ob - (3 * cvs::WS - 1)) / 2);
  a.nds = (D3 + a.dchunk - 1) / a.dchunk;
  a.ncob = (cout + ob - 1) / ob;
  const long long nblk = (long long)B * a.ncob * H * a.nds * a.nseg;
  LEA_CHECK_ARG(nblk < (1LL << 31), "lea_cv_stem_combine: grid too large");
  const size_t lds = (size_t)ob * (2 * a.dchunk + 3 * cvs::WS - 1) * sizeof(float);
  if (dtype == LEA_F32)
    cvs::cv_stem_f32_kernel<<<dim3((unsigned)nblk), cvs::kThreads, lds, as_stream(stream)>>>(a);
  else
    cvs::cv_stem_c8_kernel<<<dim3((unsigned)nblk), cvs::kThreads, lds, as_stream(stream)>>>(a);
  return launch_status("lea_cv_stem_combine");
}

static bool cv_stem_down2_ok(int cout, int D3, int H, int W, int dtype) {
  if (dtype != LEA_F32 || cout <= 0 || D3 < 2 || H < 2 || W < 4 || D3 % 2 || H % 2 || W % 4) return false;
  return (size_t)2 * cvs::OB * (2 * D3 + 3 * cvs::WS - 1) * sizeof(float) <= (size_t)cvs::kLdsBytes;
}

extern "C" int lea_cv_stem_down2_supported(int cout, int D3, int H, int W, int dtype) {
  return cv_stem_down2_ok(cout, D3, H, W, dtype) ? 1 : 0;
}

extern "C" int lea_cv_stem_combine_down2(const void* lmaps, int64_t l_bstride, const void* rmaps,
                                         int64_t r_bstride, const float* scale, const float* shift,
                                         void* y, int64_t y_bstride, void* y2, int64_t y2_bstride, int B,
                                         int cout, int D3, int H, int W, unsigned flags, int dtype,
                                         void* stream) {
  clear_error();
  LEA_CHECK_ARG(lmaps && rmaps && y && y2, "lea_cv_stem_combine_down2: null pointer");
  LEA_CHECK_ARG((scale == nullptr) == (shift == nullptr),
                "lea_cv_stem_combine_down2: scale/shift must both be set or both NULL");
  LEA_CHECK_ARG(B > 0 && cout > 0 && D3 >= 2 && H > 0 && W > 0,
                "lea_cv_stem_combine_down2: bad shape B=%d cout=%d D3=%d H=%d W=%d", B, cout, D3, H, W);
  LEA_CHECK_FLAGS(flags, LEA_RELU, "lea_cv_stem_combine_down2");
  if (!cv_stem_down2_ok(cout, D3, H, W, dtype)) {
    set_error("lea_cv_stem_combine_down2: needs f32, even D3 and H, W %% 4 == 0 and unsplit planes "
              "(D3=%d H=%d W=%d dtype=%d)", D3, H, W, dtype);
    return LEA_E_UNSUPPORTED;
  }
  LEA_CHECK_ARG((long long)cout * D3 * H * W < (1LL << 40), "lea_cv_stem_combine_down2: volume too large");
  LEA_CHECK_ARG((uintptr_t)y % 16 == 0 && y_bstride % 4 == 0 && (uintptr_t)y2 % 8 == 0 && y2_bstride % 2 == 0,
                "lea_cv_stem_combine_down2: y needs 16-byte, y2 8-byte alignment");
  const size_t ybytes = (size_t)((long long)(B - 1) * y_bstride + (long long)cout * D3 * H * W) * sizeof(float);
  const size_t y2bytes =
      (size_t)((long long)(B - 1) * y2_bstride + (long long)cout * (D3 / 2) * (H / 2) * (W / 2)) * sizeof(float);
  LEA_CHECK_ARG(!spans_overlap(y, ybytes, y2, y2bytes), "lea_cv_stem_combine_down2: y and y2 overlap");
  cvs::Args a{};
  a.lk = lmaps;
  a.lbs = l_bstride;
  a.rk = rmaps;
  a.rbs = r_bstride;
  a.scale = scale;
  a.shift = shift;
  a.y = y;
  a.ybs = y_bstride;
  a.y2 = static_cast<float*>(y2);
  a.y2bs = y2_bstride;
  a.cout = cout;
  a.D = D3;
  a.H = H;
  a.W = W;
  a.flags = flags & LEA_RELU;
  a.rd = axis_ratio(D3, D3 / 2, 1);
  a.rh = axis_ratio(H, H / 2, 1);
  a.rw = axis_ratio(W, W / 2, 1);
  a.nseg = (W + cvs::WS - 1) / cvs::WS;
  a.dchunk = D3;
  a.nds = 1;
  a.ncob = (cout + cvs::OB - 1) / cvs::OB;
  const long long nblk = (long long)B * a.ncob * (H / 2) * a.nseg;
  LEA_CHECK_ARG(nblk < (1LL << 31), "lea_cv_stem_combine_down2: grid too large");
  const size_t lds = (size_t)2 * cvs::OB * (2 * D3 + 3 * cvs::WS - 1) * sizeof(float);
  cvs::cv_stem_f32_down2_kernel<<<dim3((unsigned)nblk), cvs::kThreads, lds, as_stream(stream)>>>(a);
  return launch_status("lea_cv_stem_combine_down2");
}
```

### leastereo_amd/csrc/resample.hip

```cpp
#include "common.h"

namespace lea {

template <bool VEC>
__global__ __launch_bounds__(256) void resample3d_f32(const float* __restrict__ x, long long xbs,
                                                      float* __restrict__ y, long long ybs, int C,
                                                      int Di, int Hi, int Wi, int Do, int Ho, int Wo,
                                                      float rd, float rh, float rw, int ac,
                                                      const float* __restrict__ scale,
                                                      const float* __restrict__ shift,
                                                      unsigned flags) {
#pragma clang fp contract(off)
  const int plane = blockIdx.y;
  const int od = plane % Do;
  const int bc = plane / Do;
  const int b = bc / C, c = bc - b * C;
  const Axis ad = axis_index(rd, od, Di, Do, ac);
  const long long HWi = (long long)Hi * Wi;
  const float* xc = x + (long long)b * xbs + (long long)c * Di * HWi;
  const float* q0 = xc + ad.i0 * HWi;
  const float* q1 = xc + ad.i1 * HWi;
  float* yp = y + (long long)b * ybs + ((long long)c * Do + od) * Ho * Wo;
  const float sc = scale ? scale[c] : 1.f;
  const float sh = scale ? shift[c] : 0.f;
// ... 60 lines not shown
  const int cells = (oh1 - oh0) * wq;
  const float* l0 = rows;
  const float* l1 = rows + nrmax * Wi;
  for (int t = threadIdx.x; t < cells; t += blockDim.x) {
    const int oh = oh0 + t / wq;
    const int q = t % wq;
    const Axis ah = axis_index(rh, oh, Hi, Ho, ac);
    const int r0 = over ? 0 : (ah.i0 - r_lo) * Wi, r1 = over ? 0 : (ah.i1 - r_lo) * Wi;
    float v[VEC ? 4 : 1];
#pragma unroll
    for (int e = 0; e < (VEC ? 4 : 1); ++e) {
      const Axis aw = axis_index(rw, (VEC ? 4 * q : q) + e, Wi, Wo, ac);
      float r = trilerp(ad, ah, aw, l0 + r0, l0 + r1, l1 + r0, l1 + r1);
      if (scale) r = r * sc + sh;
      if (relu) r = fmaxf(r, 0.f);
      v[e] = over ? __builtin_nanf("") : r;
    }
    if constexpr (VEC)
      *reinterpret_cast<float4*>(yp + (long long)oh * Wo + 4 * q) = make_float4(v[0], v[1], v[2], v[3]);
    else
      yp[(long long)oh * Wo + q] = v[0];
  }
}

__global__ __launch_bounds__(256) void resample3d_sep_f32(
    const float* __restrict__ x, long long xbs, float* __restrict__ y, long long ybs, int C, int Di,
    int Hi, int Wi, int Do, int Ho, int Wo, float rd, float rh, float rw, int ac, int R, int nrmax,
    const float* __restrict__ scale, const float* __restrict__ shift, unsigned flags) {
#pragma clang fp contract(off)
  extern __shared__ float wrows[];
  const int plane = blockIdx.y;
  const int od = plane % Do;
  const int bc = plane / Do;
  const int b = bc / C, c = bc - b * C;
  const int oh0 = blockIdx.x * R;
  const int oh1 = min(oh0 + R, Ho);
  const Axis ad = axis_index(rd, od, Di, Do, ac);
  const int r_lo = axis_index(rh, oh0, Hi, Ho, ac).i0;
  const int r_hi = axis_index(rh, oh1 - 1, Hi, Ho, ac).i1;
  const bool over = r_hi - r_lo + 1 > nrmax;
  const int nr = over ? 0 : r_hi - r_lo + 1;
  const long long HWi = (long long)Hi * Wi;
  const float* xc = x + (long long)b * xbs + (long long)c * Di * HWi + (long long)r_lo * Wi;
  const float* src0 = xc + ad.i0 * HWi;
  const float* src1 = xc + ad.i1 * HWi;
  for (int xo = threadIdx.x; xo < Wo; xo += blockDim.x) {
    const Axis aw = axis_index(rw, xo, Wi, Wo, ac);
    for (int r = 0; r < nr; ++r) {
      const float* q0 = src0 + (long long)r * Wi;
      const float* q1 = src1 + (long long)r * Wi;
      wrows[r * Wo + xo] = aw.l0 * q0[aw.i0] + aw.l1 * q0[aw.i1];
      wrows[(nrmax + r) * Wo + xo] = aw.l0 * q1[aw.i0] + aw.l1 * q1[aw.i1];
    }
  }
  __syncthreads();
  float* yp = y + (long long)b * ybs + ((long long)c * Do + od) * Ho * Wo;
  const float sc = scale ? scale[c] : 1.f;
  const float sh = scale ? shift[c] : 0.f;
  const bool relu = flags & LEA_RELU;
  const int wq = Wo / 4;
  const int cells = (oh1 - oh0) * wq;
  const float4* w4 = reinterpret_cast<const float4*>(wrows);
  for (int t = threadIdx.x; t < cells; t += blockDim.x) {
    const int oh = oh0 + t / wq;
    const int q = t % wq;
    const Axis ah = axis_index(rh, oh, Hi, Ho, ac);
    const int r0 = over ? 0 : ah.i0 - r_lo, r1 = over ? 0 : ah.i1 - r_lo;
    const float4 a00 = w4[r0 * wq + q], a01 = w4[r1 * wq + q];
    const float4 a10 = w4[(nrmax + r0) * wq + q], a11 = w4[(nrmax + r1) * wq + q];
    const float p00[4] = {a00.x, a00.y, a00.z, a00.w}, p01[4] = {a01.x, a01.y, a01.z, a01.w};
    const float p10[4] = {a10.x, a10.y, a10.z, a10.w}, p11[4] = {a11.x, a11.y, a11.z, a11.w};
    float v[4];
#pragma unroll
    for (int e = 0; e < 4; ++e) {
      float r = ad.l0 * (ah.l0 * p00[e] + ah.l1 * p01[e]) + ad.l1 * (ah.l0 * p10[e] + ah.l1 * p11[e]);
      if (scale) r = r * sc + sh;
      if (relu) r = fmaxf(r, 0.f);
      v[e] = over ? __builtin_nanf("") : r;
    }
    *reinterpret_cast<float4*>(yp + (long long)oh * Wo + 4 * q) = make_float4(v[0], v[1], v[2], v[3]);
  }
}

int g_resample_mode = 0;

}

extern "C" int lea_resample_set_mode(int mode) {
  lea::clear_error();
  if (mode < 0 || mode > 2) {
    lea::set_error("lea_resample_set_mode: mode=%d", mode);
    return LEA_E_INVALID;
  }
  lea::g_resample_mode = mode;
  return 0;
}

extern "C" int lea_staged_rows(int Hi, int Ho, int ac, int R, int halo) {
  lea::clear_error();
  if (!(Hi > 0 && Ho > 0 && R > 0 && halo >= 0 && (ac == 0 || ac == 1))) {
    lea::set_error("lea_staged_rows: Hi=%d Ho=%d ac=%d R=%d halo=%d", Hi, Ho, ac, R, halo);
    return -1;
  }
  return lea::staged_rows(Hi, Ho, ac, R, halo);
}

extern "C" int lea_resample3d_trilinear(const void* x, int64_t x_bstride, void* y, int64_t y_bstride,
                                        int B, int C, int Di, int Hi, int Wi, int Do, int Ho, int Wo,
                                        int align_corners, const float* scale, const float* shift,
                                        unsigned flags, int dtype, void* stream) {
  using namespace lea;
  clear_error();
  LEA_CHECK_FLAGS(flags, LEA_RELU, "lea_resample3d_trilinear");
  LEA_CHECK_ARG(x && y && x != y, "lea_resample3d_trilinear: null or aliased pointer");
  LEA_CHECK_ARG((scale == nullptr) == (shift == nullptr),
                "lea_resample3d_trilinear: scale/shift must both be set or both NULL");
  LEA_CHECK_ARG(B > 0 && C > 0 && Di > 0 && Hi > 0 && Wi > 0 && Do > 0 && Ho > 0 && Wo > 0,
                "lea_resample3d_trilinear: bad shape");
  LEA_CHECK_ARG((long long)B * C * Do <= 65535 && (long long)Ho * Wo < (1LL << 31),
                "lea_resample3d_trilinear: grid too large (B*C*Do=%lld)", (long long)B * C * Do);
  if (dtype != LEA_F32) {
    set_error("lea_resample3d_trilinear: dtype %d unsupported", dtype);
    return LEA_E_UNSUPPORTED;
  }
  const bool vec = (Wo % 4) == 0 && ((uintptr_t)y % 16) == 0 && (y_bstride % 4) == 0;
  const int ac = align_corners ? 1 : 0;
  const long long cells = (long long)Ho * (vec ? Wo / 4 : Wo);
  const int threads = 256;
  const int gx = (int)((cells + threads * 8 - 1) / (threads * 8));
  dim3 grid(gx, B * C * Do);
  const float rd = axis_ratio(Di, Do, ac), rh = axis_ratio(Hi, Ho, ac), rw = axis_ratio(Wi, Wo, ac);
  if (vec && g_resample_mode == 0) {
    for (int R = 16; R >= 2; R /= 2) {
      const int nrmax = staged_rows(Hi, Ho, ac, R, 0);
      const size_t lds = (size_t)2 * nrmax * Wo * sizeof(float);
      if (lds > 65536) continue;
      dim3 g((Ho + R - 1) / R, B * C * Do);
      resample3d_sep_f32<<<g, threads, lds, as_stream(stream)>>>(
          (const float*)x, x_bstride, (float*)y, y_bstride, C, Di, Hi, Wi, Do, Ho, Wo, rd, rh, rw, ac, R, nrmax,
          scale, shift, flags);
      return launch_status("lea_resample3d_trilinear");
    }
  }
  for (int R = 16; R >= 2 && g_resample_mode != 2; R /= 2) {
    const int nrmax = staged_rows(Hi, Ho, ac, R, 0);
    const size_t lds = (size_t)2 * nrmax * Wi * sizeof(float);
    if (lds > 65536) continue;
    dim3 g((Ho + R - 1) / R, B * C * Do);
    if (vec)
      resample3d_rows_f32<true><<<g, threads, lds, as_stream(stream)>>>(
          (const float*)x, x_bstride, (float*)y, y_bstride, C, Di, Hi, Wi, Do, Ho, Wo, rd, rh, rw, ac,
          R, nrmax, scale, shift, flags);
    else
      resample3d_rows_f32<false><<<g, threads, lds, as_stream(stream)>>>(
          (const float*)x, x_bstride, (float*)y, y_bstride, C, Di, Hi, Wi, Do, Ho, Wo, rd, rh, rw, ac,
          R, nrmax, scale, shift, flags);
    return launch_status("lea_resample3d_trilinear");
  }
  if (vec)
    resample3d_f32<true><<<grid, threads, 0, as_stream(stream)>>>(
        (const float*)x, x_bstride, (float*)y, y_bstride, C, Di, Hi, Wi, Do, Ho, Wo, rd, rh, rw, ac,
        scale, shift, flags);
  else
    resample3d_f32<false><<<grid, threads, 0, as_stream(stream)>>>(
        (const float*)x, x_bstride, (float*)y, y_bstride, C, Di, Hi, Wi, Do, Ho, Wo, rd, rh, rw, ac,
        scale, shift, flags);
  return launch_status("lea_resample3d_trilinear");
}
```

### leastereo_amd/executor.py

```python
from __future__ import annotations

import os
from dataclasses import dataclass

import torch

from . import kernels
from .arch import scale_dimension


def _stacked(fl: torch.Tensor, fr: torch.Tensor) -> torch.Tensor:
    if (fl.is_contiguous() and fr.is_contiguous() and fl.shape == fr.shape and fl.dtype == fr.dtype
            and fl.device == fr.device
            and fl.untyped_storage().data_ptr() == fr.untyped_storage().data_ptr()
            and fr.data_ptr() == fl.data_ptr() + fl.numel() * fl.element_size()):
        return fl.as_strided((2 * fl.shape[0],) + tuple(fl.shape[1:]), fl.stride())
    return torch.cat((fl, fr), 0)


@dataclass
class ConvParams:
    packed: torch.Tensor
    scale: torch.Tensor | None
    shift: torch.Tensor | None
# ... 50 lines not shown
        with torch.no_grad():
            for name, mod in net.named_modules():
                if isinstance(mod, ConvBR):
                    self.p[name] = _conv_params(mod)
            self.s1_group = {}
            self.s1_split = set()
            for i, cell in enumerate(net.cells):
                group = []
                for k, terms in enumerate(cell.plan):
                    for op, j in terms:
                        if j == 1 and cell.op_kinds[op] == "conv":
                            group.append((k, op))
                            break
                first_cat_state = 2 + cell.steps - cell.block_multiplier
                steps = [k for k, _ in group]
                if (len(group) < 2 or steps != list(range(steps[0], steps[0] + len(steps)))
                        or 2 + steps[0] < first_cat_state):
                    continue
                mods = [cell._ops[op] for _, op in group]
                split = (self.SPLIT_S1_GROUP48 and WINOGRAD and len(mods) == 3 and cell.c_out == 16
                         and mods[0].conv.weight.dim() == 5 and mods[0].conv.weight.shape[2] == 3)
                for key, part in ((("s1_group_head", mods[:1]), ("s1_group", mods[1:])) if split
                                  else (("s1_group", mods),)):
                    w = torch.cat([m.conv.weight for m in part], 0)
                    folded = [m.folded_bn() for m in part]
                    scale = torch.cat([f[0] for f in folded]).contiguous()
                    shift = torch.cat([f[1] for f in folded]).contiguous()
                    self.p[f"cells.{i}.{key}"] = _conv_params(part[0], w, (scale, shift))
                self.s1_group[i] = group
                if split:
                    self.s1_split.add(i)
            self.s0_pair = {}
            for i, cell in enumerate(net.cells) if self.PAIR_S0 else ():
                pair = [(k, op) for k, terms in enumerate(cell.plan) for op, j in terms
                        if j == 0 and cell.op_kinds[op] == "conv"]
                first_cat_state = 2 + cell.steps - cell.block_multiplier
                if (len(pair) != 2 or getattr(cell, "dims", 3) != 2 or 2 + pair[0][0] < first_cat_state
                        or cell.c_out % 8 or 2 * cell.c_out > 32):
                    continue
                (k0, op0), (k1, op1) = pair
                m0, m1 = cell._ops[op0], cell._ops[op1]
                other = [(o, j) for o, j in cell.plan[k1] if o != op1]
                if {k for k, _ in self.s1_group.get(i, [])} & {k0, k1}:
                    continue
                if (m0.relu != m1.relu or m0.conv.weight.dim() != 4 or m0.conv.weight.shape[-1] != 3
                        or m0.stride != 1 or m1.stride != 1 or cell.plan[k1][0][0] != op1
                        or not other or cell.op_kinds[other[0][0]] != "conv"):
                    continue
                w = torch.cat([m0.conv.weight, m1.conv.weight], 0)
                folded = [m0.folded_bn(), m1.folded_bn()]
                self.p[f"cells.{i}.s0_pair"] = _conv_params(
                    m0, w, (torch.cat([f[0] for f in folded]).contiguous(),
                            torch.cat([f[1] for f in folded]).contiguous()))
                self.s0_pair[i] = pair
            self.pair_steps = {}
            for i, cell in enumerate(net.cells) if self.PAIR_STEPS else ():
                terms = [[(op, j) for op, j in t] for t in cell.plan]
                if (getattr(cell, "dims", 3) != 3 or not terms or cell.c_out not in self.PAIR_C
                        or any(len(t) != 2 or any(cell.op_kinds[op] != "conv" for op, _ in t) for t in terms)):
                    continue
                mods = [[cell._ops[op] for op, _ in t] for t in terms]
                if any(m.conv.weight.shape[-1] != 3 or not m.relu for ms in mods for m in ms):
                    continue
                for k, (ma, mb) in enumerate(mods):
                    folded = [ma.folded_bn(), mb.folded_bn()]
                    self.p[f"cells.{i}.pair{k}"] = self._pair_params(
                        ma, torch.cat([ma.conv.weight, mb.conv.weight], 1),
                        (torch.cat([f[0] for f in folded]).contiguous(),
                         torch.cat([f[1] for f in folded]).contiguous()))
                self.pair_steps[i] = terms
            cells = list(net.cells)
            for i, (cell, nxt) in enumerate(zip(cells, cells[1:])):
                if (self.SHARE_DOWNSAMPLE and cell.downup_sample != 0 and nxt.downup_sample == 0
                        and nxt.c_out == cell.c_out and 2 + cell.steps - cell.block_multiplier == 1
                        and cell.preprocess.conv.weight.shape[1] == nxt.pre_preprocess.conv.weight.shape[1]
                        and cell.preprocess.conv.weight.shape[1] != nxt.c_out):
                    mods = [nxt.pre_preprocess, cell.preprocess]
                    folded = [m.folded_bn() for m in mods]
                    self.p[f"cells.{i}.share"] = _conv_params(
                        mods[0], torch.cat([m.conv.weight for m in mods], 0),
                        (torch.cat([f[0] for f in folded]).contiguous(),
                         torch.cat([f[1] for f in folded]).contiguous()))

    def conv(self, name, x, out=None, accumulate=False, x2=None, size=None, residual=None):
        p = self.p[name]
        cin = x.shape[1] + (x2.shape[1] if x2 is not None else 0)
        if cin != p.cin:
            raise ValueError(f"{name}: expected {p.cin} input channels, got {cin}")
        resized = size is not None and tuple(size) != tuple(x.shape[2:5])
        if p.kind == "s3":
            return kernels.conv2d_s3_bnrelu(x, p.packed, p.scale, p.shift, p.relu)
        if p.kind == "2d":
            if resized or x2 is not None:
                raise ValueError(f"{name}: 2D 3x3 conv takes one input at its own size")
            return kernels.conv2d_bnrelu(x, p.packed, p.cout, p.scale, p.shift, p.relu, out,
                                         accumulate, residual)
        if resized:
            if x2 is not None or residual is not None:
                raise ValueError("resampled conv takes one input and no residual")
            up = all(int(o) >= int(i) for o, i in zip(size, x.shape[2:]))
            if p.k == 1 and up and not accumulate:
                z = kernels.conv3d_bnrelu(x, p.packed, p.cout, 1, None, None, relu=False)
                return kernels.resample_trilinear(z, size, True, out, p.scale, p.shift, p.relu)
            return kernels.conv3d_bnrelu_resampled(x, size, p.packed, p.cout, p.k, p.scale,
                                                   p.shift, p.relu, out, accumulate)
        if p.wino is not None and kernels.wino_preferred(x.shape[0], p.cout, p.cin, *x.shape[2:5]):
            return kernels.conv3d_bnrelu_wino(x, p.wino, p.cout, p.scale, p.shift, p.relu, out,
                                              accumulate, x2, residual)
        return kernels.conv3d_bnrelu(x, p.packed, p.cout, p.k, p.scale, p.shift, p.relu, out,
                                     accumulate, x2, residual)

    def _pair_params(self, mod, w, folded):
        p = _conv_params(mod, w, folded)
        p.cout = w.shape[0]
        return p

    def _pair_ok(self, x, x2, out):
        return kernels.pair_sum_supported(x, x2, out)

    def pair_conv(self, name, x, x2, out):
        p = self.p[name]
        return kernels.conv3d_bnrelu_wino(x, p.wino, p.cout, p.scale, p.shift, True, out, x2=x2, pair_sum=True)

    def _use_winograd(self):
        if not WINOGRAD:
            return
        with torch.no_grad():
            for name, p in self.p.items():
                if p.kind != "3d" or not kernels.wino_eligible(p.cout, p.cin, p.k):
                    continue
                if ".pair" in name:
                    i, k = int(name.split(".")[1]), int(name.rsplit("pair", 1)[1])
                    cell = self.m.cells[i]
                    w = torch.cat([cell._ops[op].conv.weight for op, _ in self.pair_steps[i][k]], 1)
                elif name.endswith("s1_group") or name.endswith("s1_group_head"):
                    i = int(name.split(".")[1])
                    mods = [self.m.cells[i]._ops[op] for _, op in self.s1_group[i]]
                    if i in self.s1_split:
                        mods = mods[:1] if name.endswith("_head") else mods[1:]
                    w = torch.cat([m.conv.weight for m in mods], 0)
                else:
                    w = self.m.get_submodule(name).conv.weight
                p.wino = kernels.pack_conv_weight_wino(w)

    def _empty(self, b, c, size, like):
        return torch.empty((b, c) + tuple(size), device=like.device, dtype=like.dtype)

    @staticmethod
    def _channels(t, c0, c1):
        return t[:, c0:c1]

    @staticmethod
    def _nchannels(t):
        return t.shape[1]

    @staticmethod
    def _volume(t):
        return tuple(t.shape[2:5])

    @staticmethod
    def _resample(x, size):
        return kernels.resample_trilinear(x, size)

    def cell(self, i, s0, s1, down=None):
        cell = self.m.cells[i]
        c = cell.c_out
        if down is not None and down[0] is not None:
            s0 = down[0]
        s1_down = down is not None and down[1] is not None
        if s1_down:
            s1 = down[1]
        prev_input = s1
        size = self._volume(s1)
        if cell.downup_sample != 0 and not s1_down:
            sc = 0.5 if cell.downup_sample < 0 else 2
            size = tuple(n if (cell.dims == 2 and ax == 0) else scale_dimension(n, sc)
                         for ax, n in enumerate(size))
        b = s1.shape[0]
        bm = cell.block_multiplier
        n_states = 2 + cell.steps
        memo, self._share_memo = getattr(self, "_share_memo", None), None
        share = f"cells.{i}.share" in self.p
        if share:
            big = self._empty(b, c + bm * c, size, s1)
            out = self._channels(big, c, c + bm * c)
        else:
            out = self._empty(b, bm * c, size, s1)
        slot = {idx: self._channels(out, k * c, (k + 1) * c)
                for k, idx in enumerate(range(n_states - bm, n_states))}
        group = self.s1_group.get(i, [])
        if memo is not None and memo[0] is s0 and memo[1] == size:
            s0 = memo[2]
            if 0 in slot:
                slot[0].copy_(s0)
        elif self._nchannels(s0) != c:
            s0 = self.conv(f"cells.{i}.pre_preprocess", s0, out=slot.get(0), size=size)
        else:
            if self._volume(s0) != size:
                s0 = self._resample(s0, size)
            if 0 in slot:
                slot[0].copy_(s0)
        if share:
            self.conv(f"cells.{i}.share", s1, out=self._channels(big, 0, 2 * c), size=size)
            self._share_memo = (prev_input, size, self._channels(big, 0, c))
            s1 = self._channels(big, c, 2 * c)
        else:
            s1 = self.conv(f"cells.{i}.preprocess", s1, out=slot.get(1), size=size)
        states = [s0, s1]
        pairs = self.pair_steps.get(i)
        if pairs is not None:
            dsts = [slot.get(2 + k) for k in range(len(pairs))]
            if all(d is not None for d in dsts) and all(
                    self._pair_ok(states[t[0][1]] if t[0][1] < 2 else dsts[t[0][1] - 2],
                                  states[t[1][1]] if t[1][1] < 2 else dsts[t[1][1] - 2], dsts[k])
                    for k, t in enumerate(pairs)):
                for k, ((_, ja), (_, jb)) in enumerate(pairs):
                    self.pair_conv(f"cells.{i}.pair{k}", states[ja], states[jb], dsts[k])
                    states.append(dsts[k])
                return prev_input, out
        written = set()
        done = set(group)
        consumed = set()
        pair = self.s0_pair.get(i)
        if pair is not None and self._nchannels(s0) == c and self._volume(s0) == size:
            (k0, op0), (k1, op1) = pair
            skips0 = [states[j] for o, j in cell.plan[k0] if cell.op_kinds[o] != "conv"]
            p = self.p[f"cells.{i}.s0_pair"]
            kernels.conv2d_bnrelu_pair(s0, p.packed, c, 2 * c, p.scale, p.shift, p.relu,
                                       slot[2 + k0], slot[2 + k1], skips0[-1] if skips0 else None)
            done |= {(k0, op0), (k1, op1)}
            written |= {k0, k1}
            if skips0:
                consumed.add(k0)
        if group:
            k0 = 2 + group[0][0] - (n_states - bm)
            if i in self.s1_split:
                self.conv(f"cells.{i}.s1_group", s1, out=self._channels(out, (k0 + 1) * c, (k0 + 3) * c))
                self.conv(f"cells.{i}.s1_group_head", s1, out=self._channels(out, k0 * c, (k0 + 1) * c))
            else:
                self.conv(f"cells.{i}.s1_group", s1, out=self._channels(out, k0 * c, (k0 + len(group)) * c))
            written |= {k for k, _ in group}
        for step, terms in enumerate(cell.plan):
            dst = slot.get(len(states))
            if dst is None:
                dst = self._empty(b, c, size, s1)
            skips = [states[j] for k, j in terms if cell.op_kinds[k] != "conv"]
            if step in consumed:
                skips.pop()
            for k, j in terms:
                if (step, k) in done or cell.op_kinds[k] != "conv":
                    continue
                residual = None
                if step not in written and skips:
                    residual = skips.pop()
                self.conv(f"cells.{i}._ops.{k}", states[j], out=dst, accumulate=step in written,
                          residual=residual)
                written.add(step)
            for t in skips:
                if step in written:
                    dst.add_(t)
                else:
                    dst.copy_(t)
                written.add(step)
            states.append(dst)
        return prev_input, out


class MatchingExecutor(CellGraphExecutor):
    SPLIT_S1_GROUP48 = os.environ.get("LEASTEREO_SPLIT_GROUP48", "1") != "0"
    PAIR_STEPS = WINOGRAD and os.environ.get("LEASTEREO_PAIR_STEPS", "0") != "0"
    FUSED_DOWN = os.environ.get("LEASTEREO_FUSED_DOWN", "1") != "0"

    def run(self, x):
        return self._from_stem0(self.conv("stem0", x))

    def run_features(self, fl, fr, maxdisp):
        p = self.p["stem0"]
        if fl.shape[1] * 2 != p.cin:
            raise ValueError(f"stem0 expects {p.cin} cost-volume channels, got 2*{fl.shape[1]}")
        d3 = int(maxdisp / 3)
        if self.cv is not None and kernels.cv_stem_supported(p.cout, d3, fl.shape[3], False):
            return self._from_stem0(*self._cv_stem(fl.unsqueeze(2), fr.unsqueeze(2), d3))
        if p.wino is not None and kernels.wino_preferred(fl.shape[0], p.cout, p.cin, int(maxdisp / 3),
                                                         *fl.shape[2:4]):
            stem0 = kernels.conv3d_bnrelu_costvolume_wino(fl, fr, maxdisp, p.wino, p.cout, p.scale,
                                                          p.shift, p.relu)
        else:
            stem0 = kernels.conv3d_bnrelu_costvolume(fl, fr, maxdisp, p.packed, p.cout, p.scale,
                                                     p.shift, p.relu)
        return self._from_stem0(stem0)

    def _cv_stem(self, fl5, fr5, d3):
        p, (wl, wr) = self.p["stem0"], self.cv
        lm = kernels.conv2d_bnrelu(fl5, wl, 9 * p.cout, None, None, relu=False)
        rm = kernels.conv2d_bnrelu(fr5, wr, 6 * p.cout, None, None, relu=False)
        if self._cell0_takes_down((d3,) + tuple(lm.shape[3:5])) and kernels.cv_stem_down2_supported(lm, p.cout, d3):
            return kernels.cv_stem_combine_down2(lm, rm, p.cout, d3, p.scale, p.shift, p.relu)
        return kernels.cv_stem_combine(lm, rm, p.cout, d3, p.scale, p.shift, p.relu), None

    def _cell0_takes_down(self, vol):
        cells = self.m.cells
        return (self.FUSED_DOWN and self.tap is None and not isinstance(self, _C8Layout) and len(cells) > 0
                and cells[0].downup_sample < 0 and cells[0].dims == 3
                and all(n % 2 == 0 and scale_dimension(n, 0.5) == n // 2 for n in vol))

    def _cv_stem_pack(self, wl, wr):
        return kernels.pack_conv2d_weight(wl), kernels.pack_conv2d_weight(wr)

    def _from_stem0(self, stem0, stem0_down=None):
        out = self._matching_body(stem0, stem0_down)
        if self.tap is not None:
            self.tap("matching", out.detach().clone())
        return out

    def _matching_body(self, stem0, stem0_down=None):
        d, h, w = self._volume(stem0)
        self._emit("stem0", stem0)
        stem1 = stem1_down = None
        p1 = self.p["stem1"]
        if ("cells.0.share" in self.p and self._cell0_takes_down((d, h, w)) and p1.wino is not None
                and kernels.wino_preferred(stem0.shape[0], p1.cout, p1.cin, d, h, w)
                and kernels.conv3d_wino_down2_supported(stem0, p1.cout)):
            stem1_down = kernels.conv3d_bnrelu_wino_down2(stem0, p1.wino, p1.cout, p1.scale, p1.shift, p1.relu)
        else:
            stem1 = self.conv("stem1", stem0)
            self._emit("stem1", stem1)
        outs = []
        prev = (stem0, stem1)
        n = len(self.m.cells)
        for i in range(n):
            if i == 5 and n == 12:
                fused = self.conv("conv1", outs[1][1], x2=outs[4][1])
                self._emit("conv1", fused)
                prev = (outs[4][0], fused)
            elif i == 9 and n == 12:
                fused = self.conv("conv2", outs[4][1], x2=outs[8][1])
                self._emit("conv2", fused)
                prev = (outs[8][0], fused)
            o = self.cell(i, prev[0], prev[1], down=(stem0_down, stem1_down) if i == 0 else None)
            self._emit(f"cell{i}", o[1])
            outs.append(o)
            prev = o
        last = outs[-1][1]
        lh = self._volume(last)[1]
        full, half, quarter = (d, h, w), (d // 2, h // 2, w // 2), (d // 4, h // 4, w // 4)
        if lh == h:
            return self._last3_same_size(last)
        if lh == h // 2:
            y = self.conv("last_6", last)
        elif lh == h // 4:
            y = self.conv("last_6", self.conv("last_12", last), size=half)
        elif lh == h // 8:
            y = self.conv("last_12", self.conv("last_24", last), size=quarter)
            y = self.conv("last_6", y, size=half)
        else:
            raise ValueError(f"matching-net output size {tuple(last.shape[2:])} has no head")
        p3 = self.p["last_3"]
        q = self.conv("last_3.taps", y)
        return self._tapsum(q, p3, full)

    @staticmethod
    def _tapsum(q, p3, full):
        return kernels.tapsum_upsample(q, p3.cout, full, p3.scale, p3.shift, p3.relu)

    def _last3_same_size(self, last):
        return self.conv("last_3", last)

    def __init__(self, matching):
        super().__init__(matching)
        with torch.no_grad():
            last3 = matching.last_3.conv.weight
            co, ci = last3.shape[:2]
            taps = last3.permute(0, 2, 3, 4, 1).reshape(co * 27, ci, 1, 1, 1)
            self.p["last_3.taps"] = ConvParams(kernels.pack_conv_weight(taps), None, None,
                                               ci, co * 27, 1, False)
            self.cv = None
            if CV_STEM:
                self.cv = self._cv_stem_pack(*kernels.cv_stem_split_weights(matching.stem0.conv.weight))
        self._use_winograd()


class MatchingExecutorDirect(MatchingExecutor):

    SPLIT_S1_GROUP48 = False
    PAIR_STEPS = False

    def __init__(self, matching):
        super().__init__(matching)
        self.cv = None

    def _use_winograd(self):
        """Direct engine only."""


class FeatureExecutor(CellGraphExecutor):
    FUSED_STEM = os.environ.get("LEASTEREO_FEATURE_STEM", "1") != "0"
    PAIR_S0 = os.environ.get("LEASTEREO_PAIR_S0", "1") != "0"

    def _stems(self, x, c8=False, x2=None):
        p0, p1 = self.p["stem0"], self.p["stem1"]
        if (self.FUSED_STEM and p0.relu and p1.relu and (p0.cin, p0.cout, p1.cout) == (3, 16, 32)
                and p1.kind == "s3"):
            return kernels.feature_stem(x, self.m.stem0.conv.weight, p0.scale, p0.shift, p1.packed,
                                        p1.scale, p1.shift, c8, x2)
        if x2 is not None:
            x = torch.cat((x, x2), 0)
        stem1 = self.conv("stem1", self.conv("stem0", x.unsqueeze(2)))
        return kernels.to_c8(stem1) if c8 else stem1

    def run(self, x, x2=None):
        stem1 = self._stems(x, x2=x2)
        stem2 = self.conv("stem2", stem1)
        out = (stem1, stem2)
        for i in range(len(self.m.cells)):
            out = self.cell(i, out[0], out[1])
        last = out[-1]
        h, w = stem2.shape[3:]
        lh = last.shape[3]
        full, half, quarter = (1, h, w), (1, h // 2, w // 2), (1, h // 4, w // 4)
        if lh == h:
            y = last
        elif lh == h // 2:
# ... 240 lines not shown
```

### leastereo_amd/kernels.py

```python
from __future__ import annotations

import collections
import contextlib
import math
import os

import torch

from . import _lib
from ._lib import LEA_F32, LEA_PAIR_SUM, LEA_RELU, LEA_RESIDUAL, check


def _stream():
    return torch.cuda.current_stream().cuda_stream


class KernelProbe:

    def __init__(self, names=None):
        self.names = None if names is None else set(names)
        self.records = []

    def __enter__(self):
        global _probe
# ... 301 lines not shown
def feature_stem(x: torch.Tensor, w0: torch.Tensor, scale0, shift0, w1: torch.Tensor, scale1, shift1,
                 c8: bool = False, x2: torch.Tensor | None = None) -> torch.Tensor:
    _require_cuda(x, x2, scale0, shift0, scale1, shift1)
    w0, w1 = w0.detach().contiguous(), w1.detach().contiguous()
    _require_cuda(w0, w1)
    x = x.contiguous()
    srcs = [x]
    if x2 is not None:
        if tuple(x2.shape) != tuple(x.shape):
            raise ValueError(f"feature_stem: x2 {tuple(x2.shape)} differs from x {tuple(x.shape)}")
        x2 = x2.contiguous()
        srcs.append(x2)
    b, cin, hi, wi = x.shape
    c0, c1 = w0.shape[0], w1.shape[0]
    if tuple(w0.shape) != (c0, cin, 3, 3) or tuple(w1.shape) != (c1, c0, 3, 3):
        raise ValueError(f"feature_stem: weights {tuple(w0.shape)} / {tuple(w1.shape)} do not chain")
    ho, wo = (hi - 1) // 3 + 1, (wi - 1) // 3 + 1
    nb = b * len(srcs)
    if c8:
        out = torch.empty((nb, c1 // 8, 1, ho, wo, 8), device=x.device, dtype=torch.bfloat16)
    else:
        out = torch.empty((nb, c1, 1, ho, wo), device=x.device, dtype=torch.float32)
    ptr = lambda t: t.data_ptr() if t is not None else None
    if len(srcs) == 2 and b == 1:
        srcs, b, xbs = [x], 2, (x2.data_ptr() - x.data_ptr()) // x.element_size()
    else:
        xbs = x.stride(0)
    rec = None if _probe is None else _probe_launch(
        "feature_stem_kernel", 2.0 * nb * ho * wo * (9 * 9 * cin * c0 + 9 * c0 * c1),
        4.0 * nb * cin * hi * wi + out.numel() * out.element_size(), 0.0)
    for i, src in enumerate(srcs):
        check(_lib.load().lea_feature_stem_bnrelu(
            src.data_ptr(), xbs, w0.data_ptr(), ptr(scale0), ptr(shift0), w1.data_ptr(),
            ptr(scale1), ptr(shift1), out[i * b:].data_ptr(), out.stride(0), b, cin, c0, c1, hi, wi,
            _lib.LEA_BF16 if c8 else LEA_F32, _stream()), "lea_feature_stem_bnrelu")
    _probe_end(rec)
    return out


def conv2d_s3_bnrelu(x: torch.Tensor, w: torch.Tensor, scale: torch.Tensor | None,
                     shift: torch.Tensor | None, relu: bool = True) -> torch.Tensor:
    _require_cuda(x, w, scale, shift)
    b, cin, d, hi, wi = x.shape
    if d != 1:
        raise ValueError("conv2d_s3_bnrelu takes [B, C, 1, H, W] views")
    w = w.detach().contiguous()
    cout = w.shape[0]
    if tuple(w.shape) != (cout, cin, 3, 3):
        raise ValueError(f"weight {tuple(w.shape)} does not match cin={cin}")
    xbs = _check_volume_view(x, "x")
    out = torch.empty((b, cout, 1, (hi - 1) // 3 + 1, (wi - 1) // 3 + 1), device=x.device,
                      dtype=x.dtype)
    rec = None if _probe is None else _probe_launch(
        "conv2d_s3_kernel", 2.0 * out.numel() * cin * 9, 4.0 * (x.numel() + out.numel()), 0.0)
    check(_lib.load().lea_conv2d_s3_bnrelu(
        x.data_ptr(), xbs, w.data_ptr(), scale.data_ptr() if scale is not None else None,
        shift.data_ptr() if shift is not None else None, out.data_ptr(), out.stride(0), b, cin,
        cout, hi, wi, LEA_RELU if relu else 0, LEA_F32, _stream()), "lea_conv2d_s3_bnrelu")
    _probe_end(rec)
    return out


def resample_trilinear(x: torch.Tensor, size, align_corners: bool = True,
                       out: torch.Tensor | None = None, scale: torch.Tensor | None = None,
                       shift: torch.Tensor | None = None, relu: bool = False) -> torch.Tensor:
    _require_cuda(x, out, scale, shift)
    b, c, di, hi, wi = x.shape
    do, ho, wo = (int(s) for s in size)
    xbs = _check_volume_view(x, "x")
    if out is None:
        out = torch.empty((b, c, do, ho, wo), device=x.device, dtype=x.dtype)
    if tuple(out.shape) != (b, c, do, ho, wo):
        raise ValueError(f"out shape {tuple(out.shape)} != {(b, c, do, ho, wo)}")
    ybs = _check_volume_view(out, "out")
    rec = None if _probe is None else _probe_launch(
        "resample3d_f32", 0.0, 4.0 * b * c * (di * hi * wi + do * ho * wo))
    check(_lib.load().lea_resample3d_trilinear(
        x.data_ptr(), xbs, out.data_ptr(), ybs, b, c, di, hi, wi, do, ho, wo,
        1 if align_corners else 0, scale.data_ptr() if scale is not None else None,
        shift.data_ptr() if shift is not None else None, LEA_RELU if relu else 0, LEA_F32,
        _stream()), "lea_resample3d_trilinear")
    _probe_end(rec)
    return out


def tapsum_upsample(q: torch.Tensor, cout: int, size, scale: torch.Tensor | None = None,
                    shift: torch.Tensor | None = None, relu: bool = False) -> torch.Tensor:
    _require_cuda(q, scale, shift)
    b, c27, di, hi, wi = q.shape
    if c27 != 27 * cout:
        raise ValueError(f"q has {c27} channels, expected 27*{cout}")
    qbs = _check_volume_view(q, "q")
    do, ho, wo = (int(s) for s in size)
    out = torch.empty((b, cout, do, ho, wo), device=q.device, dtype=q.dtype)
    lib = _lib.load()
    ws = torch.empty(lib.lea_tapsum_workspace_bytes(b, cout, hi, wi, do) // 4, device=q.device,
                     dtype=torch.float32)
    rec = None if _probe is None else _probe_launch(
        "tapsum_f32", 0.0, 4.0 * (q.shape[0] * q.shape[1] * di * hi * wi + out.numel()))
    check(lib.lea_tapsum_upsample(
        q.data_ptr(), qbs, out.data_ptr(), out.stride(0), b, cout, di, hi, wi, do, ho, wo,
        scale.data_ptr() if scale is not None else None,
        shift.data_ptr() if shift is not None else None, LEA_RELU if relu else 0,
        ws.data_ptr(), LEA_F32, _stream()), "lea_tapsum_upsample")
    _probe_end(rec)
    return out


def disparity_regression(cost: torch.Tensor, maxdisp: int, fast_exp: bool = False) -> torch.Tensor:
    _require_cuda(cost)
    if cost.dim() != 5 or cost.shape[1] != 1:
        raise ValueError("cost must be [B, 1, D3, H3, W3]")
    cost = cost.contiguous()
    b, _, d3, h3, w3 = cost.shape
    disp = torch.empty((b, 3 * h3, 3 * w3), device=cost.device, dtype=torch.float32)
    rec = None if _probe is None else _probe_launch(
        "disparity_regression", 0.0, 4.0 * (cost.numel() + disp.numel()))
    check(_lib.load().lea_disparity_regression(cost.data_ptr(), disp.data_ptr(), b, d3, h3, w3,
                                               maxdisp, _lib.LEA_BF16 if fast_exp else LEA_F32,
                                               _stream()),
          "lea_disparity_regression")
    _probe_end(rec)
    return disp


class DisparityStats(collections.namedtuple("DisparityStats", "disp entropy peak disp_local")):

    def __new__(cls, disp, entropy=None, peak=None, disp_local=None, maxdisp=None):
        self = super().__new__(cls, disp, entropy, peak, disp_local)
        self.maxdisp = maxdisp
        return self

    @property
    def confidence(self) -> torch.Tensor:
        if self.entropy is None or not self.maxdisp:
            raise ValueError("confidence needs the entropy output (entropy=True) and maxdisp")
        return 1.0 - self.entropy / math.log(self.maxdisp)


def disparity_regression_stats(cost: torch.Tensor, maxdisp: int, radius: int = 4, fast_exp: bool = False,
                               entropy: bool = True, peak: bool = True, local: bool = True) -> DisparityStats:
    _require_cuda(cost)
    if cost.dim() != 5 or cost.shape[1] != 1:
        raise ValueError("cost must be [B, 1, D3, H3, W3]")
    if not (entropy or peak or local):
        raise ValueError("disparity_regression_stats: ask for at least one of entropy, peak, local "
                         "(disparity_regression gives the disparity alone)")
    cost = cost.contiguous()
    b, _, d3, h3, w3 = cost.shape
    outs = [torch.empty((b, 3 * h3, 3 * w3), device=cost.device, dtype=torch.float32) if want else None
            for want in (True, entropy, peak, local)]
    rec = None if _probe is None else _probe_launch(
        "disparity_regression_stats", 0.0, 4.0 * (cost.numel() + sum(o.numel() for o in outs if o is not None)))
    check(_lib.load().lea_disparity_regression_stats(
        cost.data_ptr(), *(None if o is None else o.data_ptr() for o in outs), b, d3, h3, w3, maxdisp,
        radius, _lib.LEA_BF16 if fast_exp else LEA_F32, _stream()), "lea_disparity_regression_stats")
    _probe_end(rec)
    return DisparityStats(*outs, maxdisp)


LR_CONSISTENT, LR_INCONSISTENT, LR_OUT_OF_VIEW = 0, 1, 2
LR_SPECKLE = 3

DisparityLR = collections.namedtuple("DisparityLR", "disp disp_right state disp_filled")
DisparityLR.__doc__ = """What ``LEAStereo.forward_lr`` / ``lr_check`` return (``None`` where not asked for):
  disp         the left-view disparity, [B, H, W] float32
# ... 825 lines not shown
        cop = 16 * wc * mte
        return (-(-cout // cop) * cop) / cout / 3.0
    f = int(name.split("<", 1)[1].split(",", 1)[0])
    if cout <= 8:
        return (f + 2) / (3.0 * f) * 12 / 9 * 8 / cout
    cop = 16 if cout <= 16 else (48 if cout % 32 != 0 and cout % 48 == 0 else 32)
    return (f + 2) / (3.0 * f) * (-(-cout // cop) * cop) / cout


@contextlib.contextmanager
def wino_depth_f2():
    lib = _lib.load()
    check(lib.lea_conv3d_wino44_set(0), "lea_conv3d_wino44_set")
    try:
        yield
    finally:
        check(lib.lea_conv3d_wino44_set(int(os.environ.get("LEASTEREO_WINO44") or 2)), "lea_conv3d_wino44_set")


def wino_kernel_name(b, cout, d, h, w, costvolume=False, cin=0):
    name = _lib.load().lea_conv3d_wino_kernel_name(b, cin, cout, d, h, w, 1 if costvolume else 0)
    return name.decode() if name else None


def pack_conv_weight_wino(w: torch.Tensor) -> torch.Tensor:
    _require_cuda(w)
    w = w.detach().contiguous()
    if w.dim() != 5 or tuple(w.shape[2:]) != (3, 3, 3):
        raise ValueError(f"expected a [cout, cin, 3, 3, 3] weight, got {tuple(w.shape)}")
    cout, cin = w.shape[0], w.shape[1]
    n = _lib.load().lea_conv3d_wino_packed_floats(cout, cin)
    if n == 0:
        raise ValueError(f"unsupported Winograd conv shape cout={cout} cin={cin}")
    packed = torch.empty(n, device=w.device, dtype=torch.float32)
    check(_lib.load().lea_conv3d_wino_pack_weights(w.data_ptr(), packed.data_ptr(), cout, cin,
                                                   _stream()), "lea_conv3d_wino_pack_weights")
    return packed


def pair_sum_supported(x: torch.Tensor, x2: torch.Tensor, out: torch.Tensor) -> bool:
    b, c, d, h, w = x.shape
    ok = out.shape[1] <= 32 and w % 4 == 0 and x2.shape[2:] == x.shape[2:] and x.shape[1] % 4 == 0
    for t, al in ((x, 16), (x2, 16), (out, 8)):
        ok = ok and t.data_ptr() % al == 0 and t.stride(0) % (al // 4) == 0 and \
            t.stride()[1:] == (d * h * w, h * w, w, 1)
    return bool(ok and 16 * d * h * w * 4 < 0xFFFFFF00)


def conv3d_bnrelu_wino(x: torch.Tensor, packed: torch.Tensor, cout: int,
                       scale: torch.Tensor | None, shift: torch.Tensor | None, relu: bool = True,
                       out: torch.Tensor | None = None, accumulate: bool = False,
                       x2: torch.Tensor | None = None,
                       residual: torch.Tensor | None = None, pair_sum: bool = False) -> torch.Tensor:
    _require_cuda(x, x2, packed, scale, shift, out)
    if pair_sum and (x2 is None or accumulate or residual is not None):
        raise ValueError("pair_sum takes two sources and no residual")
    b, cin, d, h, w = x.shape
    xbs = _check_volume_view(x, "x")
    cin2, x2bs = 0, 0
    if x2 is not None:
        if x2.shape[0] != b or tuple(x2.shape[2:]) != (d, h, w):
            raise ValueError("x2 must match x in batch and volume")
        cin2 = x2.shape[1]
        x2bs = _check_volume_view(x2, "x2")
    out, ybs = _conv_out(x.shape, cout, (d, h, w), out, accumulate, x.device, x.dtype)
    rptr, rbs = _residual(out, accumulate, residual, ybs)
    flags = (LEA_RELU if relu else 0) | (LEA_RESIDUAL if rptr is not None else 0) | (LEA_PAIR_SUM if pair_sum else 0)
    rec = None
    if _probe is not None:
        name = "conv3d_wino22_kernel" if pair_sum else wino_kernel_name(b, cout, d, h, w, cin=cin + cin2)
        rec = _probe_begin(b, cin + cin2, cout, d, h, w, 3, rptr is not None, b * d * h * w, False,
                           name=name, mfma_scale=wino_mfma_scale(cout, name))
    check(_lib.load().lea_conv3d_bnrelu_wino(
        x.data_ptr(), xbs, x2.data_ptr() if x2 is not None else None, x2bs, cin2,
        packed.data_ptr(),
        scale.data_ptr() if scale is not None else None,
        shift.data_ptr() if shift is not None else None,
        rptr, rbs, out.data_ptr(), ybs, b, cin + cin2, cout, d, h, w, flags, LEA_F32, _stream()),
        "lea_conv3d_bnrelu_wino")
    _probe_end(rec)
    return out


def wino_down2_kernel_name(b, cin, cout, d, h, w):
    name = _lib.load().lea_conv3d_wino_down2_kernel_name(b, cin, cout, d, h, w)
    return name.decode() if name else None


def conv3d_wino_down2_supported(x: torch.Tensor, cout: int) -> bool:
    if not x.is_cuda or x.dtype != torch.float32 or x.dim() != 5:
        return False
    b, cin, d, h, w = x.shape
    if x.data_ptr() % 16 or x.stride(0) % 4 or x.stride()[1:] != (d * h * w, h * w, w, 1):
        return False
    return bool(_lib.load().lea_conv3d_wino_down2_supported(b, cin, cout, d, h, w))


def conv3d_bnrelu_wino_down2(x: torch.Tensor, packed: torch.Tensor, cout: int,
                             scale: torch.Tensor | None, shift: torch.Tensor | None,
                             relu: bool = True) -> torch.Tensor:
    _require_cuda(x, packed, scale, shift)
    b, cin, d, h, w = x.shape
    xbs = _check_volume_view(x, "x")
    out = torch.empty((b, cout, d // 2, h // 2, w // 2), device=x.device, dtype=x.dtype)
    rec = None
    if _probe is not None:
        name = wino_down2_kernel_name(b, cin, cout, d, h, w) or "conv3d_wino44_down2_kernel"
        rec = _probe_begin(b, cin, cout, d, h, w, 3, False, b * d * h * w, False, name=name,
                           mfma_scale=wino_mfma_scale(cout, "conv3d_wino44_kernel"))
        if rec is not None:
            nbytes = 4.0 * (x.numel() + out.numel()) + 4.0 * cout * cin * 27
            rec = rec[:3] + (nbytes,) + rec[4:]
    check(_lib.load().lea_conv3d_bnrelu_wino_down2(
        x.data_ptr(), xbs, packed.data_ptr(),
        scale.data_ptr() if scale is not None else None,
        shift.data_ptr() if shift is not None else None,
        out.data_ptr(), out.stride(0), b, cin, cout, d, h, w, LEA_RELU if relu else 0, LEA_F32, _stream()),
        "lea_conv3d_bnrelu_wino_down2")
    _probe_end(rec)
    return out


def conv3d_bnrelu_costvolume_wino(fl: torch.Tensor, fr: torch.Tensor, maxdisp: int,
                                  packed: torch.Tensor, cout: int, scale: torch.Tensor | None,
                                  shift: torch.Tensor | None, relu: bool = True) -> torch.Tensor:
    _require_cuda(fl, fr, packed, scale, shift)
    if fl.shape != fr.shape or fl.dim() != 4:
        raise ValueError("left/right features must both be [B, C, H, W]")
    if fl.stride() != fr.stride() or fl.stride()[1:] != (fl.shape[2] * fl.shape[3], fl.shape[3], 1):
        raise ValueError("left/right features need contiguous C,H,W and equal strides")
    b, c, h, w = fl.shape
    d3 = int(maxdisp / 3)
    out = torch.empty((b, cout, d3, h, w), device=fl.device, dtype=fl.dtype)
    rec = None
    if _probe is not None:
        name = wino_kernel_name(b, cout, d3, h, w, True, cin=2 * c)
        rec = _probe_begin(b, 2 * c, cout, d3, h, w, 3, False, 0, False,
                           name=name, mfma_scale=wino_mfma_scale(cout, name))
    check(_lib.load().lea_conv3d_bnrelu_costvolume_wino(
        fl.data_ptr(), fr.data_ptr(), fl.stride(0), packed.data_ptr(),
        scale.data_ptr() if scale is not None else None,
        shift.data_ptr() if shift is not None else None, out.data_ptr(), out.stride(0), b, c, cout,
        d3, h, w, LEA_RELU if relu else 0, LEA_F32, _stream()), "lea_conv3d_bnrelu_costvolume_wino")
    _probe_end(rec)
    return out
```

Measured before the change: 160.7 pairs/s.

## Fuse trilinear 2x downsample into depth-paired Winograd conv epilogue and add concat down2 path

Adds a down-sampling epilogue to the depth-paired F(4,3) Winograd conv3d kernel. It computes the trilinear half-resolution output in registers, using lane shuffles and a small LDS exchange region, and can optionally skip the full-resolution store. It also adds a concatenated-input variant of the strided down2 conv and a standalone fused trilinear down2 resample. The aim is to remove separate resample kernel launches and the extra full-volume reads of conv outputs in the 3D matching network cells. The cost is a larger LDS footprint, an extra barrier in the epilogue, and more template variants.

```diff
diff --git a/include/leastereo_hip.h b/include/leastereo_hip.h
--- a/include/leastereo_hip.h
+++ b/include/leastereo_hip.h
@@ -213,6 +213,24 @@
                                  const float* scale, const float* shift, void* y, int64_t y_bstride,
                                  int B, int cin, int cout, int D, int H, int W, unsigned flags, int dtype,
                                  void* stream);
+int lea_conv3d_wino_down2_cat_supported(int B, int cin, int cin2, int cout, int D, int H, int W);
+const char* lea_conv3d_wino_down2_cat_kernel_name(int B, int cin, int cin2, int cout, int D, int H, int W);
+int lea_conv3d_bnrelu_wino_down2_cat(const void* x, int64_t x_bstride, const void* x2, int64_t x2_bstride,
+                                     int cin2, const float* w_packed, const float* scale, const float* shift,
+                                     void* y, int64_t y_bstride, int B, int cin, int cout, int D, int H,
+                                     int W, unsigned flags, int dtype, void* stream);
+int lea_conv3d_wino_dp_down2_supported(int B, int cin, int cout, int D, int H, int W);
+const char* lea_conv3d_wino_dp_down2_kernel_name(int B, int cin, int cout, int D, int H, int W, int only);
+int lea_conv3d_bnrelu_wino_dp_down2(const void* x, int64_t x_bstride, const float* w_packed,
+                                    const float* scale, const float* shift, const void* residual,
+                                    int64_t r_bstride, void* y, int64_t y_bstride, void* y2,
+                                    int64_t y2_bstride, int B, int cin, int cout, int D, int H, int W,
+                                    unsigned flags, int dtype, void* stream);
+int lea_resample3d_down2_supported(int Di, int Hi, int Wi, int Do, int Ho, int Wo, int dtype);
+int lea_resample3d_trilinear_down2(const void* x, int64_t x_bstride, void* y, int64_t y_bstride, void* y2,
+                                   int64_t y2_bstride, int B, int C, int Di, int Hi, int Wi, int Do, int Ho,
+                                   int Wo, const float* scale, const float* shift, unsigned flags, int dtype,
+                                   void* stream);
 
 int lea_cv_stem_split_weights(const float* w, float* wl, float* wr, int cout, int C, void* stream);
 int lea_cv_stem_combine(const void* lmaps, int64_t l_bstride, const void* rmaps, int64_t r_bstride,
diff --git a/leastereo_amd/_lib.py b/leastereo_amd/_lib.py
--- a/leastereo_amd/_lib.py
+++ b/leastereo_amd/_lib.py
@@ -106,6 +106,17 @@
     "lea_conv3d_wino_down2_supported": (_i, [_i, _i, _i, _i, _i, _i]),
     "lea_conv3d_wino_down2_kernel_name": (ctypes.c_char_p, [_i, _i, _i, _i, _i, _i]),
     "lea_conv3d_bnrelu_wino_down2": (_i, [_p, _i64, _p, _p, _p, _p, _i64, _i, _i, _i, _i, _i, _i, _u, _i, _p]),
+    "lea_conv3d_wino_down2_cat_supported": (_i, [_i, _i, _i, _i, _i, _i, _i]),
+    "lea_conv3d_wino_down2_cat_kernel_name": (ctypes.c_char_p, [_i, _i, _i, _i, _i, _i, _i]),
+    "lea_conv3d_bnrelu_wino_down2_cat": (_i, [_p, _i64, _p, _i64, _i, _p, _p, _p, _p, _i64, _i, _i, _i, _i, _i, _i,
+                                              _u, _i, _p]),
+    "lea_conv3d_wino_dp_down2_supported": (_i, [_i, _i, _i, _i, _i, _i]),
+    "lea_conv3d_wino_dp_down2_kernel_name": (ctypes.c_char_p, [_i, _i, _i, _i, _i, _i, _i]),
+    "lea_conv3d_bnrelu_wino_dp_down2": (_i, [_p, _i64, _p, _p, _p, _p, _i64, _p, _i64, _p, _i64, _i, _i, _i, _i, _i,
+                                             _i, _u, _i, _p]),
+    "lea_resample3d_down2_supported": (_i, [_i, _i, _i, _i, _i, _i, _i]),
+    "lea_resample3d_trilinear_down2": (_i, [_p, _i64, _p, _i64, _p, _i64, _i, _i, _i, _i, _i, _i, _i, _i, _p, _p,
+                                            _u, _i, _p]),
     "lea_conv3d_wino_set_tile_override": (_i, [_i, _i, _i]),
     "lea_conv3d_wino_set_variant": (_i, [_i]),
     "lea_conv3d_wino2_set_walk": (_i, [_i]),
diff --git a/leastereo_amd/csrc/conv3d_wino.hip b/leastereo_amd/csrc/conv3d_wino.hip
--- a/leastereo_amd/csrc/conv3d_wino.hip
+++ b/leastereo_amd/csrc/conv3d_wino.hip
@@ -49,16 +49,26 @@
   static_assert(2 * STAGE * 4 * 2 <= 160 * 1024, "two double-buffered workgroups per CU");
 };
 
-template <int F, int Q, int MT, int NP, int TD, bool CV, bool H16 = false, bool FENCE = false>
-__global__ __launch_bounds__(kConvThreads, 2) void conv3d_wino_kernel(const ConvArgs a) {
+constexpr int kDownXch = 4 * 64 * 4;
+__device__ __forceinline__ float lerp_dp(float l0, float v0, float l1, float v1) {
+#pragma clang fp contract(off)
+  return l0 * v0 + l1 * v1;
+}
+
+template <int F, int Q, int MT, int NP, int TD, bool CV, bool H16, bool FENCE, int DOWN>
+__device__ __forceinline__ void conv3d_wino_body(const ConvArgs& a) {
   using C = Cfg<F, Q, MT, NP, TD, H16>;
   static_assert(!(CV && H16), "16-byte halo: plain volumes only");
+  static_assert(DOWN == 0 || (C::DP && F == 4 && NP == 1 && !CV && (Q == 16 || Q == 8)),
+                "down-sampling epilogue: the depth-paired F(4,3) tiles");
+  constexpr int XCH = (DOWN != 0 && Q == 16) ? kDownXch : 0;
+  static_assert((2 * C::STAGE + XCH) * 4 * 2 <= 160 * 1024, "two workgroups per CU with the exchange region");
   constexpr int NX = C::NX;
   constexpr int XSLOTS = C::XSLOTS;
   constexpr int XSLOTS_W = (XSLOTS + kConvWaves - 1) / kConvWaves;
   constexpr int WSLOTS = C::WSLOTS;
   constexpr int WSLOTS_W = (WSLOTS + kConvWaves - 1) / kConvWaves;
-  __shared__ __attribute__((aligned(16))) float smem[2 * C::STAGE];
+  __shared__ __attribute__((aligned(16))) float smem[2 * C::STAGE + XCH];
   const unsigned lds0 = lds_addr(smem);
 
   const int tid = threadIdx.x;
@@ -296,6 +306,97 @@
             }
             buf_store4(yrs, off[t][j][m][r], y);
           }
+  };
+  constexpr int NSD = 1;
+  const Axis aw0 = axis_index(a.rw, w / 2, a.W, a.W / 2, 1), aw1 = axis_index(a.rw, w / 2 + 1, a.W, a.W / 2, 1);
+  const Axis ah = axis_index(a.rh, (h0 + wave * C::RPG + pr) / 2, a.H, a.H / 2, 1);
+  auto epilogue_down = [&](int d0) {
+    if constexpr (DOWN != 0) {
+      const int dp = ci >> 1;
+      const int d = d0 + dp;
+      const int h = h0 + wave * C::RPG + pr;
+      const bool lv = d < a.D && h < a.H && w < a.W;
+      const int D2 = a.D / 2, H2 = a.H / 2, W2 = a.W / 2;
+      const long long V2 = (long long)D2 * H2 * W2;
+      unsigned off[4];
+#pragma unroll
+      for (int r = 0; r < 4; ++r)
+        off[r] = (lv && 4 * (ci & 1) + r < nco)
+                     ? (unsigned)((4 * (ci & 1) + r) * DHW + (long long)d * HW + h * a.W + w) * 4u
+                     : kEpiOob;
+      f32x4 rv[4];
+      if (resid) {
+#pragma unroll
+        for (int r = 0; r < 4; ++r) rv[r] = buf_load4(rrs, off[r]);
+      }
+      const Axis ad = axis_index(a.rd, d0 / 2, a.D, D2, 1);
+      float wv[4][2];
+#pragma unroll
+      for (int r = 0; r < 4; ++r) {
+        const float m0 = 0.25f * acc[0][0][0][0][r];
+        const float m1 = (-1.f / 6.f) * acc[1][0][0][0][r], m2 = (-1.f / 6.f) * acc[2][0][0][0][r];
+        const float m3 = (1.f / 24.f) * acc[3][0][0][0][r], m4 = (1.f / 24.f) * acc[4][0][0][0][r];
+        const float m5 = acc[NX - 1][0][0][0][r];
+        const float sp = m1 + m2, sm = m1 - m2, tp = m3 + m4, tm = m3 - m4;
+        f32x4 y;
+        y[0] = (m0 + sp) + tp;
+        y[1] = fmaf(2.f, tm, sm);
+        y[2] = fmaf(4.f, tp, sp);
+        y[3] = fmaf(8.f, tm, sm) + m5;
+#pragma unroll
+        for (int e = 0; e < 4; ++e) {
+          float v = y[e] * sc[0][r] + sh[0][r];
+          if (relu) v = fmaxf(v, 0.f);
+          y[e] = resid ? v + rv[r][e] : v;
+        }
+        if constexpr (DOWN == 1) buf_store4(yrs, off[r], y);
+        wv[r][0] = lerp_dp(aw0.l0, (aw0.i0 & 1) ? y[1] : y[0], aw0.l1, (aw0.i1 & 1) ? y[1] : y[0]);
+        wv[r][1] = lerp_dp(aw1.l0, (aw1.i0 & 1) ? y[3] : y[2], aw1.l1, (aw1.i1 & 1) ? y[3] : y[2]);
+      }
+      const int odd = Q == 8 ? pr : (wave & 1);
+      float mine[2][2], oth[2][2];
+      if constexpr (Q == 8) {
+#pragma unroll
+        for (int k = 0; k < 2; ++k)
+#pragma unroll
+          for (int c = 0; c < 2; ++c) {
+            mine[k][c] = odd ? wv[2 + k][c] : wv[k][c];
+            oth[k][c] = __shfl_xor(odd ? wv[k][c] : wv[2 + k][c], 8);
+          }
+      } else {
+        f32x4* const xq = reinterpret_cast<f32x4*>(smem + 2 * C::STAGE) + (wave >> 1) * 128 + lane;
+        if (odd) {
+          xq[64] = f32x4{wv[0][0], wv[0][1], wv[1][0], wv[1][1]};
+          mine[0][0] = wv[2][0], mine[0][1] = wv[2][1], mine[1][0] = wv[3][0], mine[1][1] = wv[3][1];
+        } else {
+          xq[0] = f32x4{wv[2][0], wv[2][1], wv[3][0], wv[3][1]};
+          mine[0][0] = wv[0][0], mine[0][1] = wv[0][1], mine[1][0] = wv[1][0], mine[1][1] = wv[1][1];
+        }
+        __syncthreads();
+        const f32x4 t = xq[64 * (1 - odd)];
+        oth[0][0] = t[0];
+        oth[0][1] = t[1];
+        oth[1][0] = t[2];
+        oth[1][1] = t[3];
+      }
+      float o[2][2];
+#pragma unroll
+      for (int k = 0; k < 2; ++k)
+#pragma unroll
+        for (int c = 0; c < 2; ++c) {
+          const float row0 = odd ? oth[k][c] : mine[k][c], row1 = odd ? mine[k][c] : oth[k][c];
+          const float hv = lerp_dp(ah.l0, (ah.i0 & 1) ? row1 : row0, ah.l1, (ah.i1 & 1) ? row1 : row0);
+          const float hp = __shfl_xor(hv, 32);
+          const float pl0 = dp ? hp : hv, pl1 = dp ? hv : hp;
+          o[k][c] = lerp_dp(ad.l0, (ad.i0 & 1) ? pl1 : pl0, ad.l1, (ad.i1 & 1) ? pl1 : pl0);
+        }
+      const __amdgpu_buffer_rsrc_t y2rs = block_rsrc(a.y2 + (long long)b * a.y2bs, nco * V2 * 4);
+      const long long vox = ((long long)(d0 / 2) * H2 + h / 2) * W2 + w / 2;
+      const int cr = 4 * (ci & 1) + 2 * odd + dp;
+      const f32x2 v2 = dp ? f32x2{o[1][0], o[1][1]} : f32x2{o[0][0], o[0][1]};
+      const unsigned off2 = (lv && cr < nco) ? (unsigned)(cr * V2 + vox) * 4u : kEpiOob;
+      __builtin_amdgcn_raw_buffer_store_b64(__builtin_bit_cast(u32x2_t, v2), y2rs, off2, 0, 0);
+    }
   };
   auto epilogue = [&](int d0) {
 #pragma unroll
@@ -373,7 +474,7 @@
   issue(0, smem);
   for (int it = 0; it < nitems; ++it) {
     const int ch = it % nchunks;
-    wait_item<NST>(ebuf && ch == 0 && it > 0);
+    wait_item<DOWN == 0 ? NST : DOWN == 1 ? NST + NSD : NSD>((DOWN != 0 || ebuf) && ch == 0 && it > 0);
     __syncthreads();
     if (it + 1 < nitems) issue(it + 1, smem + ((it + 1) & 1) * C::STAGE);
     const float* xs = smem + (it & 1) * C::STAGE;
@@ -487,7 +588,9 @@
     }
     }
     if (ch == nchunks - 1) {
-      if (ebuf)
+      if constexpr (DOWN != 0)
+        epilogue_down((dz0 + it / nchunks) * TD);
+      else if (ebuf)
         epilogue_buf((dz0 + it / nchunks) * TD);
       else
         epilogue((dz0 + it / nchunks) * TD);
@@ -501,6 +604,15 @@
             for (int j = 0; j < NP; ++j) acc[x][t][m][j] = f32x4{0.f, 0.f, 0.f, 0.f};
     }
   }
+}
+
+template <int F, int Q, int MT, int NP, int TD, bool CV, bool H16 = false, bool FENCE = false>
+__global__ __launch_bounds__(kConvThreads, 2) void conv3d_wino_kernel(const ConvArgs a) {
+  conv3d_wino_body<F, Q, MT, NP, TD, CV, H16, FENCE, 0>(a);
+}
+template <int Q, bool ONLY>
+__global__ __launch_bounds__(kConvThreads, 2) void conv3d_wino_dp_down2_kernel(const ConvArgs a) {
+  conv3d_wino_body<4, Q, 0, 1, 2, false, Q == 16, Q == 16, ONLY ? 2 : 1>(a);
 }
 
 template <int MT>
@@ -1014,6 +1126,125 @@
 namespace lea {
 namespace wino {
 
+static int dp_down2_plan(int B, int cin, int cout, int D, int H, int W, ConvArgs* a) {
+  if (B <= 0 || cin <= 0 || cout <= 0 || cout > 8 || D < 2 || H < 2 || W < 4 || D % 2 || H % 2 || W % 4 ||
+      cin % CIN_B)
+    return 0;
+  if ((long long)D * H * W * 4 >= (1LL << 32) || (long long)(cout + 47) * D * H * W >= (1LL << 31)) return 0;
+  if (!g_epibuf || g_w22 == 2 || g_variant != 0 || g_override[0] != 0) return 0;
+  Plan p = make_plan(B, cout, D, H, W);
+  if (p.mt != 0 || p.d2 || p.f != 4 || p.np != 1 || p.td != 2) return 0;
+  plan_halo16(p, false, W, a, cin);
+  if (a && !epi_buf_ok(*a)) return 0;
+  if (p.q == 16) return (p.h16 && g_fence) ? 16 : 0;
+  return p.q == 8 ? 8 : 0;
+}
+
+static int run_dp_down2(ConvArgs a, int B, int q, bool only, hipStream_t st) {
+  a.ncob = 1;
+  const int tw = 4 * q, th = 4 * (16 / q);
+  a.tiles_w = (a.W + tw - 1) / tw;
+  a.ntiles = a.tiles_w * ((a.H + th - 1) / th);
+  a.ndz = (a.D + 1) / 2;
+  a.spw = std::max(1, std::min(g_spw > 0 ? g_spw : auto_walk(a, B, 2), a.ndz));
+  const long long n_ = (long long)a.ntiles * ((a.ndz + a.spw - 1) / a.spw) * B * a.ncob;
+  LEA_CHECK_ARG(n_ < (1LL << 31), "lea_conv3d_bnrelu_wino_dp_down2: grid too large");
+  a.nblk = (int)n_;
+  const dim3 grid((unsigned)n_);
+  if (q == 16) {
+    if (only)
+      conv3d_wino_dp_down2_kernel<16, true><<<grid, kConvThreads, 0, st>>>(a);
+    else
+      conv3d_wino_dp_down2_kernel<16, false><<<grid, kConvThreads, 0, st>>>(a);
+  } else {
+    if (only)
+      conv3d_wino_dp_down2_kernel<8, true><<<grid, kConvThreads, 0, st>>>(a);
+    else
+      conv3d_wino_dp_down2_kernel<8, false><<<grid, kConvThreads, 0, st>>>(a);
+  }
+  return launch_status("lea_conv3d_bnrelu_wino_dp_down2");
+}
+
+}
+}
+
+extern "C" int lea_conv3d_wino_dp_down2_supported(int B, int cin, int cout, int D, int H, int W) {
+  return wino::dp_down2_plan(B, cin, cout, D, H, W, nullptr) ? 1 : 0;
+}
+
+extern "C" const char* lea_conv3d_wino_dp_down2_kernel_name(int B, int cin, int cout, int D, int H, int W,
+                                                            int only) {
+  const int q = wino::dp_down2_plan(B, cin, cout, D, H, W, nullptr);
+  if (!q) return nullptr;
+  snprintf(wino::g_name, sizeof(wino::g_name), "conv3d_wino_dp_down2_kernel<%d, %s>", q, only ? "true" : "false");
+  return wino::g_name;
+}
+
+extern "C" int lea_conv3d_bnrelu_wino_dp_down2(const void* x, int64_t x_bstride, const float* w_packed,
+                                               const float* scale, const float* shift, const void* residual,
+                                               int64_t r_bstride, void* y, int64_t y_bstride, void* y2,
+                                               int64_t y2_bstride, int B, int cin, int cout, int D, int H, int W,
+                                               unsigned flags, int dtype, void* stream) {
+  const char* what = "lea_conv3d_bnrelu_wino_dp_down2";
+  clear_error();
+  ConvArgs a{};
+  a.x = (const float*)x;
+  a.xbs = x_bstride;
+  a.cin1 = cin;
+  a.wp = w_packed;
+  a.scale = scale;
+  a.shift = shift;
+  a.res = (const float*)residual;
+  a.rbs = r_bstride;
+  a.y = (float*)y;
+  a.ybs = y_bstride;
+  a.y2 = (float*)y2;
+  a.y2bs = y2_bstride;
+  a.cin = cin;
+  a.cout = cout;
+  a.D = D;
+  a.H = H;
+  a.W = W;
+  LEA_CHECK_ARG(a.x && a.wp && a.y2, "%s: null pointer", what);
+  LEA_CHECK_ARG((scale == nullptr) == (shift == nullptr), "%s: scale/shift must both be set or both NULL", what);
+  LEA_CHECK_ARG(!(flags & LEA_RESIDUAL) || a.res, "%s: LEA_RESIDUAL without residual", what);
+  LEA_CHECK_ARG(B > 0 && cin > 0 && cout > 0 && D > 0 && H > 0 && W > 0,
+                "%s: bad shape B=%d cin=%d cout=%d D=%d H=%d W=%d", what, B, cin, cout, D, H, W);
+  LEA_CHECK_FLAGS(flags, LEA_RELU | LEA_RESIDUAL, what);
+  a.flags = flags;
+  if (dtype != LEA_F32) {
+    set_error("%s: dtype %d unsupported", what, dtype);
+    return LEA_E_UNSUPPORTED;
+  }
+  if (cout > 8 || D % 2 || H % 2 || W % 4 || cin % wino::CIN_B) {
+    set_error("%s: needs cout <= 8, even D and H, W %% 4 == 0, cin %% %d == 0 (cin=%d cout=%d D=%d H=%d W=%d)", what,
+              wino::CIN_B, cin, cout, D, H, W);
+    return LEA_E_UNSUPPORTED;
+  }
+  LEA_CHECK_ARG(a.x != a.y && a.x != a.y2 && a.y != a.y2 && a.res != a.y2, "%s: aliased output", what);
+  LEA_CHECK_ARG(((uintptr_t)y2 & 15) == 0 && y2_bstride % 4 == 0, "%s: y2 needs 16-byte alignment", what);
+  const bool only = a.y == nullptr;
+  if (only) {
+    a.y = const_cast<float*>(a.res ? a.res : a.x);
+    a.ybs = a.res ? a.rbs : a.xbs;
+  }
+  const int q = wino::dp_down2_plan(B, cin, cout, D, H, W, &a);
+  if (!q) {
+    set_error("%s: the planner does not put B=%d cin=%d cout=%d D=%d H=%d W=%d on a depth-paired tile with the "
+              "buffer-addressed epilogue (or its settings / the operands' alignment rule it out)",
+              what, B, cin, cout, D, H, W);
+    return LEA_E_UNSUPPORTED;
+  }
+  a.flags |= wino::kEpiBuf;
+  a.rd = axis_ratio(D, D / 2, 1);
+  a.rh = axis_ratio(H, H / 2, 1);
+  a.rw = axis_ratio(W, W / 2, 1);
+  return wino::run_dp_down2(a, B, q, only, as_stream(stream));
+}
+
+namespace lea {
+namespace wino {
+
 static bool down2_plan(int B, int cin, int cout, int D, int H, int W, ConvArgs* a, Plan2* out) {
   if (B <= 0 || cin <= 0 || cout <= 0 || D < 2 || H < 2 || W < 4 || D % 2 || H % 2 || W % 4 || cin % CIN_B)
     return false;
@@ -1039,15 +1270,28 @@
   return wino::down2_plan(B, cin, cout, D, H, W, nullptr, nullptr) ? "conv3d_wino44_down2_kernel" : nullptr;
 }
 
-extern "C" int lea_conv3d_bnrelu_wino_down2(const void* x, int64_t x_bstride, const float* w_packed,
-                                            const float* scale, const float* shift, void* y,
-                                            int64_t y_bstride, int B, int cin, int cout, int D, int H, int W,
-                                            unsigned flags, int dtype, void* stream) {
+extern "C" int lea_conv3d_wino_down2_cat_supported(int B, int cin, int cin2, int cout, int D, int H, int W) {
+  if (cin2 <= 0 || cin2 >= cin || cin2 % wino::CIN_B) return 0;
+  return wino::down2_plan(B, cin, cout, D, H, W, nullptr, nullptr) ? 1 : 0;
+}
+
+extern "C" const char* lea_conv3d_wino_down2_cat_kernel_name(int B, int cin, int cin2, int cout, int D, int H,
+                                                             int W) {
+  return lea_conv3d_wino_down2_cat_supported(B, cin, cin2, cout, D, H, W) ? "conv3d_wino44_down2_cat_kernel"
+                                                                          : nullptr;
+}
+
+static int wino_down2_entry(const char* what, const void* x, int64_t x_bstride, const void* x2, int64_t x2_bstride,
+                            int cin2, const float* w_packed, const float* scale, const float* shift, void* y,
+                            int64_t y_bstride, int B, int cin, int cout, int D, int H, int W, unsigned flags,
+                            int dtype, void* stream) {
   clear_error();
   ConvArgs a{};
   a.x = (const float*)x;
   a.xbs = x_bstride;
-  a.cin1 = cin;
+  a.x2 = (const float*)x2;
+  a.x2bs = x2_bstride;
+  a.cin1 = cin - cin2;
   a.wp = w_packed;
   a.scale = scale;
   a.shift = shift;
@@ -1058,34 +1302,35 @@
   a.D = D;
   a.H = H;
   a.W = W;
-  LEA_CHECK_ARG(a.x && a.wp && a.y, "lea_conv3d_bnrelu_wino_down2: null pointer");
-  LEA_CHECK_ARG((scale == nullptr) == (shift == nullptr),
-                "lea_conv3d_bnrelu_wino_down2: scale/shift must both be set or both NULL");
+  LEA_CHECK_ARG(a.x && a.wp && a.y, "%s: null pointer", what);
+  LEA_CHECK_ARG((scale == nullptr) == (shift == nullptr), "%s: scale/shift must both be set or both NULL", what);
   LEA_CHECK_ARG(B > 0 && cin > 0 && cout > 0 && D > 0 && H > 0 && W > 0,
-                "lea_conv3d_bnrelu_wino_down2: bad shape B=%d cin=%d cout=%d D=%d H=%d W=%d", B, cin, cout, D, H, W);
+                "%s: bad shape B=%d cin=%d cout=%d D=%d H=%d W=%d", what, B, cin, cout, D, H, W);
   if (flags & (LEA_RESIDUAL | LEA_PAIR_SUM)) {
-    set_error("lea_conv3d_bnrelu_wino_down2: LEA_RESIDUAL / LEA_PAIR_SUM are not supported with the "
-              "down-sampling epilogue");
+    set_error("%s: LEA_RESIDUAL / LEA_PAIR_SUM are not supported with the down-sampling epilogue", what);
     return LEA_E_UNSUPPORTED;
   }
-  LEA_CHECK_FLAGS(flags, LEA_RELU, "lea_conv3d_bnrelu_wino_down2");
+  LEA_CHECK_FLAGS(flags, LEA_RELU, what);
   a.flags = flags;
   LEA_CHECK_ARG(D % 2 == 0 && H % 2 == 0 && W % 4 == 0,
-                "lea_conv3d_bnrelu_wino_down2: D and H must be even and W %% 4 == 0 (D=%d H=%d W=%d)", D, H, W);
-  LEA_CHECK_ARG(cin % wino::CIN_B == 0, "lea_conv3d_bnrelu_wino_down2: cin %d must be a multiple of %d", cin,
-                wino::CIN_B);
-  LEA_CHECK_ARG(a.x != a.y, "lea_conv3d_bnrelu_wino_down2: input aliases output");
+                "%s: D and H must be even and W %% 4 == 0 (D=%d H=%d W=%d)", what, D, H, W);
+  LEA_CHECK_ARG(cin % wino::CIN_B == 0, "%s: cin %d must be a multiple of %d", what, cin, wino::CIN_B);
+  if (x2) {
+    LEA_CHECK_ARG(cin2 > 0 && cin2 < cin && cin2 % wino::CIN_B == 0,
+                  "%s: the second source's %d of %d channels must be a multiple of %d in (0, cin)", what, cin2, cin,
+                  wino::CIN_B);
+    LEA_CHECK_ARG(((uintptr_t)x2 & 15) == 0 && x2_bstride % 4 == 0, "%s: x2 needs 16-byte alignment", what);
+  }
+  LEA_CHECK_ARG(a.x != a.y && a.x2 != a.y, "%s: input aliases output", what);
   if (dtype != LEA_F32) {
-    set_error("lea_conv3d_bnrelu_wino_down2: dtype %d unsupported", dtype);
+    set_error("%s: dtype %d unsupported", what, dtype);
     return LEA_E_UNSUPPORTED;
   }
-  LEA_CHECK_ARG(((uintptr_t)y & 15) == 0 && y_bstride % 4 == 0,
-                "lea_conv3d_bnrelu_wino_down2: y needs 16-byte alignment");
+  LEA_CHECK_ARG(((uintptr_t)y & 15) == 0 && y_bstride % 4 == 0, "%s: y needs 16-byte alignment", what);
   wino::Plan2 q;
   if (!wino::down2_plan(B, cin, cout, D, H, W, &a, &q)) {
-    set_error("lea_conv3d_bnrelu_wino_down2: the planner does not put B=%d cin=%d cout=%d D=%d H=%d W=%d on "
-              "the F(4,3) x F(4,3) tile (or its settings / the operands' alignment rule it out)",
-              B, cin, cout, D, H, W);
+    set_error("%s: the planner does not put B=%d cin=%d cout=%d D=%d H=%d W=%d on the F(4,3) x F(4,3) tile "
+              "(or its settings / the operands' alignment rule it out)", what, B, cin, cout, D, H, W);
     return LEA_E_UNSUPPORTED;
   }
   a.rd = axis_ratio(D, D / 2, 1);
@@ -1094,3 +1339,22 @@
   a.uoff = wino::l44_offset(cout, cin);
   return wino::run44(a, B, q.spw, as_stream(stream), true);
 }
+
+extern "C" int lea_conv3d_bnrelu_wino_down2(const void* x, int64_t x_bstride, const float* w_packed,
+                                            const float* scale, const float* shift, void* y,
+                                            int64_t y_bstride, int B, int cin, int cout, int D, int H, int W,
+                                            unsigned flags, int dtype, void* stream) {
+  return wino_down2_entry("lea_conv3d_bnrelu_wino_down2", x, x_bstride, nullptr, 0, 0, w_packed, scale, shift, y,
+                          y_bstride, B, cin, cout, D, H, W, flags, dtype, stream);
+}
+
+extern "C" int lea_conv3d_bnrelu_wino_down2_cat(const void* x, int64_t x_bstride, const void* x2,
+                                                int64_t x2_bstride, int cin2, const float* w_packed,
+                                                const float* scale, const float* shift, void* y,
+                                                int64_t y_bstride, int B, int cin, int cout, int D, int H, int W,
+                                                unsigned flags, int dtype, void* stream) {
+  clear_error();
+  LEA_CHECK_ARG(x2, "lea_conv3d_bnrelu_wino_down2_cat: null pointer");
+  return wino_down2_entry("lea_conv3d_bnrelu_wino_down2_cat", x, x_bstride, x2, x2_bstride, cin2, w_packed, scale,
+                          shift, y, y_bstride, B, cin, cout, D, H, W, flags, dtype, stream);
+}
diff --git a/leastereo_amd/csrc/conv3d_wino44.hip b/leastereo_amd/csrc/conv3d_wino44.hip
--- a/leastereo_amd/csrc/conv3d_wino44.hip
+++ b/leastereo_amd/csrc/conv3d_wino44.hip
@@ -544,6 +544,9 @@
 __global__ __launch_bounds__(256, 2) void conv3d_wino44_down2_kernel(const ConvArgs a) {
   conv3d_wino44_body<false, 0, true>(a);
 }
+__global__ __launch_bounds__(256, 2) void conv3d_wino44_down2_cat_kernel(const ConvArgs a) {
+  conv3d_wino44_body<false, 0, true>(a);
+}
 
 int g_w44 = 2;
 int g_w44u = 0;
@@ -562,7 +565,10 @@
   a.grp = g_w44g >= 0 ? g_w44g : (n_ >= 2048 ? 16 : 0);
   const dim3 grid((unsigned)n_);
   if (down) {
-    conv3d_wino44_down2_kernel<<<grid, 256, 0, st>>>(a);
+    if (a.x2 && a.cin1 < a.cin)
+      conv3d_wino44_down2_cat_kernel<<<grid, 256, 0, st>>>(a);
+    else
+      conv3d_wino44_down2_kernel<<<grid, 256, 0, st>>>(a);
     return launch_status("lea_conv3d(wino44 down2)");
   }
   if (g_w44u)
diff --git a/leastereo_amd/csrc/cv_stem.hip b/leastereo_amd/csrc/cv_stem.hip
--- a/leastereo_amd/csrc/cv_stem.hip
+++ b/leastereo_amd/csrc/cv_stem.hip
@@ -82,6 +82,7 @@
 
 constexpr int OB = 16;
 
+template <int OB = 16>
 __device__ __forceinline__ void stage_row_f32(const Args& a, const Tile& T, const float* rkh, float* rs,
                                               float* corr) {
   const int D = T.D, W = T.W, NU = T.NU, NT = T.NT, d0 = T.d0, d1 = T.d1, w0 = T.w0;
@@ -245,6 +246,8 @@
   return l0 * v0 + l1 * v1;
 }
 
+constexpr int OBD = 8;
+
 __global__ __launch_bounds__(kThreads) void cv_stem_f32_down2_kernel(const Args a) {
   extern __shared__ float rs[];
   const Tile T = tile_of(a, a.H / 2);
@@ -252,20 +255,20 @@
   const long long HW = T.HW;
   const float* lk = static_cast<const float*>(a.lk) + T.b * a.lbs;
   const float* rk = static_cast<const float*>(a.rk) + T.b * a.rbs;
-  const int rowf = OB * (NT + a.dchunk);
+  const int rowf = OBD * (NT + a.dchunk);
   const int tid = threadIdx.x;
 #pragma unroll
   for (int r = 0; r < 2; ++r)
-    stage_row_f32(a, T, rk + (long long)(2 * hp + r) * W, rs + r * rowf, rs + r * rowf + OB * NT);
+    stage_row_f32<OBD>(a, T, rk + (long long)(2 * hp + r) * W, rs + r * rowf, rs + r * rowf + OBD * NT);
   __syncthreads();
 
-  const int ol = tid >> 4, o = T.cob * OB + ol;
+  const int r = (tid >> 5) & 1;
+  const int ol = ((tid >> 6) << 1) | ((tid >> 4) & 1), o = T.cob * OBD + ol;
   const int w = w0 + 4 * (tid & 15);
   if (o >= a.cout || w >= W) return;
   const bool band = w - (D - 1) <= 1;
-  float gl[2][4], bl[2][4][4], lf[2][4], ll[2][4];
-#pragma unroll
-  for (int r = 0; r < 2; ++r) {
+  float gl[4], bl[4][4], lf[4], ll[4];
+  {
     float lkv[3][3][4];
 #pragma unroll
     for (int kd = 0; kd < 3; ++kd)
@@ -287,81 +290,71 @@
       for (int kd = 0; kd < 3; ++kd)
 #pragma unroll
         for (int t = 0; t < 3; ++t) l3[kd][t] = lkv[kd][t][j];
-      gl[r][j] = lkv[0][0][j] + lkv[1][0][j] + lkv[2][0][j];
-#pragma unroll
-      for (int m = 0; m < 4; ++m) bl[r][m][j] = left_sum(l3, 1, m - 2, D);
-      lf[r][j] = left_sum(l3, 0, w + j, D);
-      ll[r][j] = left_sum(l3, D - 1, w + j - (D - 1), D);
+      gl[j] = lkv[0][0][j] + lkv[1][0][j] + lkv[2][0][j];
+#pragma unroll
+      for (int m = 0; m < 4; ++m) bl[m][j] = left_sum(l3, 1, m - 2, D);
+      lf[j] = left_sum(l3, 0, w + j, D);
+      ll[j] = left_sum(l3, D - 1, w + j - (D - 1), D);
     }
   }
   const float sc = a.scale ? a.scale[o] : 1.f, sh = a.scale ? a.shift[o] : 0.f;
   const float lo = (a.flags & LEA_RELU) ? 0.f : -INFINITY;
   const int jedge = W - 1 - w;
   const bool far = w0 - (D - 2) >= 2;
-  float* yp = static_cast<float*>(a.y) + T.b * a.ybs + (long long)o * D * HW + (long long)(2 * hp) * W + w;
+  float* yp = static_cast<float*>(a.y) + T.b * a.ybs + (long long)o * D * HW + (long long)(2 * hp + r) * W + w;
   const int D2 = D / 2, H2 = H / 2, W2 = W / 2;
-  float* y2p = a.y2 + T.b * a.y2bs + ((long long)o * D2 * H2 + hp) * W2 + w / 2;
+  float* y2p = a.y2 + T.b * a.y2bs + ((long long)o * D2 * H2 + hp) * W2 + w / 2 + r;
   Axis aw[2];
 #pragma unroll
   for (int c = 0; c < 2; ++c) aw[c] = axis_index(a.rw, w / 2 + c, W, W2, 1);
   const Axis ah = axis_index(a.rh, hp, H, H2, 1);
   const bool h0odd = ah.i0 & 1, h1odd = ah.i1 & 1;
+  const float* r0 = rs + r * rowf + ol * NT;
+  const float* cr = rs + r * rowf + OBD * NT + ol * a.dchunk;
 
   float ev[2] = {0.f, 0.f};
   for (int d = 0; d < D; ++d) {
-    float out[2][4];
-#pragma unroll
-    for (int r = 0; r < 2; ++r) {
-      const float* r0 = rs + r * rowf + ol * NT;
-      const float c = rs[r * rowf + OB * NT + ol * a.dchunk + d];
-      float pre[4];
-      if (d == 0 || d == D - 1) {
-        const int pb = (d == 0 ? NU : NU + WS) + (w - w0);
-#pragma unroll
-        for (int j = 0; j < 4; ++j) pre[j] = (d == 0 ? lf[r][j] : ll[r][j]) + r0[pb + j] - (j == jedge ? c : 0.f);
-      } else {
-        const int iu = w - d - T.u0;
-#pragma unroll
-        for (int j = 0; j < 4; ++j) {
-          const int u = w + j - d;
-          float l = (far || u >= 2) ? gl[r][j] : 0.f;
-          if (!far) {
-#pragma unroll
-            for (int m = 0; m < 4; ++m) l = u == m - 2 ? bl[r][m][j] : l;
-          }
-          pre[j] = l + r0[iu + j] - (j == jedge ? c : 0.f);
+    const float c = cr[d];
+    float pre[4];
+    if (d == 0 || d == D - 1) {
+      const int pb = (d == 0 ? NU : NU + WS) + (w - w0);
+#pragma unroll
+      for (int j = 0; j < 4; ++j) pre[j] = (d == 0 ? lf[j] : ll[j]) + r0[pb + j] - (j == jedge ? c : 0.f);
+    } else {
+      const int iu = w - d - T.u0;
+#pragma unroll
+      for (int j = 0; j < 4; ++j) {
+        const int u = w + j - d;
+        float l = (far || u >= 2) ? gl[j] : 0.f;
+        if (!far) {
+#pragma unroll
+          for (int m = 0; m < 4; ++m) l = u == m - 2 ? bl[m][j] : l;
         }
+        pre[j] = l + r0[iu + j] - (j == jedge ? c : 0.f);
       }
-      float4 o4;
-      float* po = reinterpret_cast<float*>(&o4);
-#pragma unroll
-      for (int j = 0; j < 4; ++j) {
-        po[j] = fmaxf(pre[j] * sc + sh, lo);
-        out[r][j] = po[j];
-      }
-      *reinterpret_cast<float4*>(yp + (long long)d * HW + r * W) = o4;
-    }
+    }
+    float4 o4;
+    float* out = reinterpret_cast<float*>(&o4);
+#pragma unroll
+    for (int j = 0; j < 4; ++j) out[j] = fmaxf(pre[j] * sc + sh, lo);
+    *reinterpret_cast<float4*>(yp + (long long)d * HW) = o4;
     float hv[2];
 #pragma unroll
-    for (int c = 0; c < 2; ++c) {
-      float wv[2];
-#pragma unroll
-      for (int r = 0; r < 2; ++r) {
-        const float v0 = (aw[c].i0 & 1) ? out[r][2 * c + 1] : out[r][2 * c];
-        const float v1 = (aw[c].i1 & 1) ? out[r][2 * c + 1] : out[r][2 * c];
-        wv[r] = lerp2(aw[c].l0, v0, aw[c].l1, v1);
-      }
-      hv[c] = lerp2(ah.l0, h0odd ? wv[1] : wv[0], ah.l1, h1odd ? wv[1] : wv[0]);
+    for (int k = 0; k < 2; ++k) {
+      const float v0 = (aw[k].i0 & 1) ? out[2 * k + 1] : out[2 * k];
+      const float v1 = (aw[k].i1 & 1) ? out[2 * k + 1] : out[2 * k];
+      const float mine = lerp2(aw[k].l0, v0, aw[k].l1, v1);
+      const float other = __shfl_xor(mine, 32);
+      const float row0 = r ? other : mine, row1 = r ? mine : other;
+      hv[k] = lerp2(ah.l0, h0odd ? row1 : row0, ah.l1, h1odd ? row1 : row0);
     }
     if (!(d & 1)) {
       ev[0] = hv[0];
       ev[1] = hv[1];
     } else {
       const Axis ad = axis_index(a.rd, d >> 1, D, D2, 1);
-      float2 o2;
-      o2.x = lerp2(ad.l0, (ad.i0 & 1) ? hv[0] : ev[0], ad.l1, (ad.i1 & 1) ? hv[0] : ev[0]);
-      o2.y = lerp2(ad.l0, (ad.i0 & 1) ? hv[1] : ev[1], ad.l1, (ad.i1 & 1) ? hv[1] : ev[1]);
-      *reinterpret_cast<float2*>(y2p + (long long)(d >> 1) * H2 * W2) = o2;
+      const float e = r ? ev[1] : ev[0], v = r ? hv[1] : hv[0];
+      y2p[(long long)(d >> 1) * H2 * W2] = lerp2(ad.l0, (ad.i0 & 1) ? v : e, ad.l1, (ad.i1 & 1) ? v : e);
     }
   }
 }
@@ -689,10 +682,10 @@
   a.nseg = (W + cvs::WS - 1) / cvs::WS;
   a.dchunk = D3;
   a.nds = 1;
-  a.ncob = (cout + cvs::OB - 1) / cvs::OB;
+  a.ncob = (cout + cvs::OBD - 1) / cvs::OBD;
   const long long nblk = (long long)B * a.ncob * (H / 2) * a.nseg;
   LEA_CHECK_ARG(nblk < (1LL << 31), "lea_cv_stem_combine_down2: grid too large");
-  const size_t lds = (size_t)2 * cvs::OB * (2 * D3 + 3 * cvs::WS - 1) * sizeof(float);
+  const size_t lds = (size_t)2 * cvs::OBD * (2 * D3 + 3 * cvs::WS - 1) * sizeof(float);
   cvs::cv_stem_f32_down2_kernel<<<dim3((unsigned)nblk), cvs::kThreads, lds, as_stream(stream)>>>(a);
   return launch_status("lea_cv_stem_combine_down2");
 }
diff --git a/leastereo_amd/csrc/resample.hip b/leastereo_amd/csrc/resample.hip
--- a/leastereo_amd/csrc/resample.hip
+++ b/leastereo_amd/csrc/resample.hip
@@ -166,6 +166,95 @@
   }
 }
 
+__global__ __launch_bounds__(256) void resample3d_sep_down2_f32(
+    const float* __restrict__ x, long long xbs, float* __restrict__ y, long long ybs, float* __restrict__ y2,
+    long long y2bs, int C, int Di, int Hi, int Wi, int Do, int Ho, int Wo, float rd, float rh, float rw,
+    float rd2, float rh2, float rw2, int R, int nrmax, const float* __restrict__ scale,
+    const float* __restrict__ shift, unsigned flags) {
+#pragma clang fp contract(off)
+  extern __shared__ float wrows[];
+  const int D2 = Do / 2, H2 = Ho / 2, W2 = Wo / 2;
+  const int pp = blockIdx.y % D2;
+  const int bc = blockIdx.y / D2;
+  const int b = bc / C, c = bc - b * C;
+  const int oh0 = blockIdx.x * R;
+  const int oh1 = min(oh0 + R, Ho);
+  const Axis ad[2] = {axis_index(rd, 2 * pp, Di, Do, 1), axis_index(rd, 2 * pp + 1, Di, Do, 1)};
+  const int db = ad[0].i0;
+  const int r_lo = axis_index(rh, oh0, Hi, Ho, 1).i0;
+  const int r_hi = axis_index(rh, oh1 - 1, Hi, Ho, 1).i1;
+  const bool over = r_hi - r_lo + 1 > nrmax || ad[1].i1 - db > 2;
+  const int nr = over ? 0 : r_hi - r_lo + 1;
+  const long long HWi = (long long)Hi * Wi;
+  const float* xc = x + (long long)b * xbs + (long long)c * Di * HWi + (long long)r_lo * Wi;
+  for (int xo = threadIdx.x; xo < Wo; xo += blockDim.x) {
+    const Axis aw = axis_index(rw, xo, Wi, Wo, 1);
+#pragma unroll
+    for (int p = 0; p < 3; ++p) {
+      const float* src = xc + min(db + p, Di - 1) * HWi;
+      for (int r = 0; r < nr; ++r) {
+        const float* q = src + (long long)r * Wi;
+        wrows[(p * nrmax + r) * Wo + xo] = aw.l0 * q[aw.i0] + aw.l1 * q[aw.i1];
+      }
+    }
+  }
+  __syncthreads();
+  const float sc = scale ? scale[c] : 1.f;
+  const float sh = scale ? shift[c] : 0.f;
+  const bool relu = flags & LEA_RELU;
+  const int wq = Wo / 4;
+  const int cells = ((oh1 - oh0) / 2) * wq;
+  const float4* w4 = reinterpret_cast<const float4*>(wrows);
+  const Axis ad2 = axis_index(rd2, pp, Do, D2, 1);
+  float* yc = y + (long long)b * ybs + (long long)c * Do * Ho * Wo;
+  float* y2c = y2 + (long long)b * y2bs + ((long long)c * D2 + pp) * H2 * W2;
+  for (int t = threadIdx.x; t < cells; t += blockDim.x) {
+    const int j = t / wq, q = t % wq;
+    const int oh = oh0 + 2 * j;
+    float v[2][2][4];
+#pragma unroll
+    for (int rr = 0; rr < 2; ++rr) {
+      const Axis ah = axis_index(rh, oh + rr, Hi, Ho, 1);
+      const int r0 = over ? 0 : ah.i0 - r_lo, r1 = over ? 0 : ah.i1 - r_lo;
+#pragma unroll
+      for (int pl = 0; pl < 2; ++pl) {
+        const int k0 = over ? 0 : ad[pl].i0 - db, k1 = over ? 0 : ad[pl].i1 - db;
+        const float4 a00 = w4[(k0 * nrmax + r0) * wq + q], a01 = w4[(k0 * nrmax + r1) * wq + q];
+        const float4 a10 = w4[(k1 * nrmax + r0) * wq + q], a11 = w4[(k1 * nrmax + r1) * wq + q];
+        const float p00[4] = {a00.x, a00.y, a00.z, a00.w}, p01[4] = {a01.x, a01.y, a01.z, a01.w};
+        const float p10[4] = {a10.x, a10.y, a10.z, a10.w}, p11[4] = {a11.x, a11.y, a11.z, a11.w};
+#pragma unroll
+        for (int e = 0; e < 4; ++e) {
+          float r = ad[pl].l0 * (ah.l0 * p00[e] + ah.l1 * p01[e]) + ad[pl].l1 * (ah.l0 * p10[e] + ah.l1 * p11[e]);
+          if (scale) r = r * sc + sh;
+          if (relu) r = fmaxf(r, 0.f);
+          v[pl][rr][e] = over ? __builtin_nanf("") : r;
+        }
+        *reinterpret_cast<float4*>(yc + ((long long)(2 * pp + pl) * Ho + oh + rr) * Wo + 4 * q) =
+            make_float4(v[pl][rr][0], v[pl][rr][1], v[pl][rr][2], v[pl][rr][3]);
+      }
+    }
+    const Axis ah2 = axis_index(rh2, oh / 2, Ho, H2, 1);
+    float o2[2];
+#pragma unroll
+    for (int k = 0; k < 2; ++k) {
+      const Axis aw2 = axis_index(rw2, 2 * q + k, Wo, W2, 1);
+      float hl[2];
+#pragma unroll
+      for (int pl = 0; pl < 2; ++pl) {
+        float wl[2];
+#pragma unroll
+        for (int rr = 0; rr < 2; ++rr)
+          wl[rr] = aw2.l0 * ((aw2.i0 & 1) ? v[pl][rr][2 * k + 1] : v[pl][rr][2 * k]) +
+                   aw2.l1 * ((aw2.i1 & 1) ? v[pl][rr][2 * k + 1] : v[pl][rr][2 * k]);
+        hl[pl] = ah2.l0 * ((ah2.i0 & 1) ? wl[1] : wl[0]) + ah2.l1 * ((ah2.i1 & 1) ? wl[1] : wl[0]);
+      }
+      o2[k] = ad2.l0 * ((ad2.i0 & 1) ? hl[1] : hl[0]) + ad2.l1 * ((ad2.i1 & 1) ? hl[1] : hl[0]);
+    }
+    *reinterpret_cast<float2*>(y2c + (long long)(oh / 2) * W2 + 2 * q) = make_float2(o2[0], o2[1]);
+  }
+}
+
 int g_resample_mode = 0;
 
 }
@@ -251,3 +340,51 @@
         scale, shift, flags);
   return launch_status("lea_resample3d_trilinear");
 }
+
+static int sep_down2_rows(int Hi, int Ho, int Wo, int* nrmax) {
+  for (int R = 8; R >= 2; R /= 2) {
+    const int n = lea::staged_rows(Hi, Ho, 1, R, 0);
+    if ((size_t)3 * n * Wo * sizeof(float) > 65536) continue;
+    if (nrmax) *nrmax = n;
+    return R;
+  }
+  return 0;
+}
+
+extern "C" int lea_resample3d_down2_supported(int Di, int Hi, int Wi, int Do, int Ho, int Wo, int dtype) {
+  if (dtype != LEA_F32 || Di <= 0 || Hi <= 0 || Wi <= 0 || Do < 2 || Ho < 2 || Wo < 4) return 0;
+  if (Do < Di || Do % 2 || Ho % 2 || Wo % 4 || Do > 2048) return 0;
+  return sep_down2_rows(Hi, Ho, Wo, nullptr) ? 1 : 0;
+}
+
+extern "C" int lea_resample3d_trilinear_down2(const void* x, int64_t x_bstride, void* y, int64_t y_bstride,
+                                              void* y2, int64_t y2_bstride, int B, int C, int Di, int Hi, int Wi,
+                                              int Do, int Ho, int Wo, const float* scale, const float* shift,
+                                              unsigned flags, int dtype, void* stream) {
+  using namespace lea;
+  const char* what = "lea_resample3d_trilinear_down2";
+  clear_error();
+  LEA_CHECK_FLAGS(flags, LEA_RELU, what);
+  LEA_CHECK_ARG(x && y && y2 && x != y && x != y2 && y != y2, "%s: null or aliased pointer", what);
+  LEA_CHECK_ARG((scale == nullptr) == (shift == nullptr), "%s: scale/shift must both be set or both NULL", what);
+  LEA_CHECK_ARG(B > 0 && C > 0 && Di > 0 && Hi > 0 && Wi > 0 && Do > 0 && Ho > 0 && Wo > 0, "%s: bad shape", what);
+  if (!lea_resample3d_down2_supported(Di, Hi, Wi, Do, Ho, Wo, dtype)) {
+    set_error("%s: needs LEA_F32, an output volume with even D and H and W %% 4 == 0, no down-sampling along D "
+              "and rows that fit the LDS (%d x %d x %d -> %d x %d x %d, dtype %d)", what, Di, Hi, Wi, Do, Ho, Wo,
+              dtype);
+    return LEA_E_UNSUPPORTED;
+  }
+  LEA_CHECK_ARG((long long)B * C * (Do / 2) <= 65535 && (long long)Ho * Wo < (1LL << 31),
+                "%s: grid too large (B*C*Do/2=%lld)", what, (long long)B * C * (Do / 2));
+  LEA_CHECK_ARG((uintptr_t)y % 16 == 0 && y_bstride % 4 == 0 && (uintptr_t)y2 % 8 == 0 && y2_bstride % 2 == 0,
+                "%s: y needs 16-byte, y2 8-byte alignment", what);
+  int nrmax = 0;
+  const int R = sep_down2_rows(Hi, Ho, Wo, &nrmax);
+  const size_t lds = (size_t)3 * nrmax * Wo * sizeof(float);
+  dim3 g((Ho + R - 1) / R, B * C * (Do / 2));
+  resample3d_sep_down2_f32<<<g, 256, lds, as_stream(stream)>>>(
+      (const float*)x, x_bstride, (float*)y, y_bstride, (float*)y2, y2_bstride, C, Di, Hi, Wi, Do, Ho, Wo,
+      axis_ratio(Di, Do, 1), axis_ratio(Hi, Ho, 1), axis_ratio(Wi, Wo, 1), axis_ratio(Do, Do / 2, 1),
+      axis_ratio(Ho, Ho / 2, 1), axis_ratio(Wo, Wo / 2, 1), R, nrmax, scale, shift, flags);
+  return launch_status(what);
+}
diff --git a/leastereo_amd/executor.py b/leastereo_amd/executor.py
--- a/leastereo_amd/executor.py
+++ b/leastereo_amd/executor.py
@@ -156,7 +156,8 @@
                         (torch.cat([f[0] for f in folded]).contiguous(),
                          torch.cat([f[1] for f in folded]).contiguous()))
 
-    def conv(self, name, x, out=None, accumulate=False, x2=None, size=None, residual=None):
+    def conv(self, name, x, out=None, accumulate=False, x2=None, size=None, residual=None, down=None,
+             down_only=False):
         p = self.p[name]
         cin = x.shape[1] + (x2.shape[1] if x2 is not None else 0)
         if cin != p.cin:
@@ -175,12 +176,24 @@
             up = all(int(o) >= int(i) for o, i in zip(size, x.shape[2:]))
             if p.k == 1 and up and not accumulate:
                 z = kernels.conv3d_bnrelu(x, p.packed, p.cout, 1, None, None, relu=False)
+                if down is not None:
+                    return kernels.resample_trilinear_down2(z, size, out, down, p.scale, p.shift, p.relu)[0]
                 return kernels.resample_trilinear(z, size, True, out, p.scale, p.shift, p.relu)
+            if down is not None:
+                raise ValueError(f"{name}: no down-sampling form of this resampled conv")
             return kernels.conv3d_bnrelu_resampled(x, size, p.packed, p.cout, p.k, p.scale,
                                                    p.shift, p.relu, out, accumulate)
         if p.wino is not None and kernels.wino_preferred(x.shape[0], p.cout, p.cin, *x.shape[2:5]):
+            if down is not None:
+                if x2 is not None:
+                    raise ValueError(f"{name}: the down-sampling epilogue takes one input")
+                kernels.conv3d_bnrelu_wino_dp_down2(x, p.wino, p.cout, p.scale, p.shift, p.relu, out, down,
+                                                    accumulate, residual, only=down_only)
+                return out
             return kernels.conv3d_bnrelu_wino(x, p.wino, p.cout, p.scale, p.shift, p.relu, out,
                                               accumulate, x2, residual)
+        if down is not None:
+            raise ValueError(f"{name}: no down-sampling epilogue on this conv's engine")
         return kernels.conv3d_bnrelu(x, p.packed, p.cout, p.k, p.scale, p.shift, p.relu, out,
                                      accumulate, x2, residual)
 
@@ -235,6 +248,9 @@
     @staticmethod
     def _resample(x, size):
         return kernels.resample_trilinear(x, size)
+
+    def _cell_output_takes_down(self, i, size):
+        return False
 
     def cell(self, i, s0, s1, down=None):
         cell = self.m.cells[i]
@@ -262,6 +278,11 @@
             out = self._empty(b, bm * c, size, s1)
         slot = {idx: self._channels(out, k * c, (k + 1) * c)
                 for k, idx in enumerate(range(n_states - bm, n_states))}
+        dn = None
+        if self._cell_output_takes_down(i, size) and self._down_kernels_take(s1, c, self._volume(s1), size):
+            dn = self._empty(b, bm * c, tuple(n // 2 for n in size), s1)
+        self._cell_down = dn
+        dslot = {} if dn is None else {idx: self._channels(dn, k * c, (k + 1) * c) for k, idx in enumerate(slot)}
         group = self.s1_group.get(i, [])
         if memo is not None and memo[0] is s0 and memo[1] == size:
             s0 = memo[2]
@@ -279,7 +300,8 @@
             self._share_memo = (prev_input, size, self._channels(big, 0, c))
             s1 = self._channels(big, c, 2 * c)
         else:
-            s1 = self.conv(f"cells.{i}.preprocess", s1, out=slot.get(1), size=size)
+            s1 = self.conv(f"cells.{i}.preprocess", s1, out=slot.get(1), size=size,
+                           **({} if dn is None else {"down": dslot[1]}))
         states = [s0, s1]
         pairs = self.pair_steps.get(i)
         if pairs is not None:
@@ -321,14 +343,18 @@
             skips = [states[j] for k, j in terms if cell.op_kinds[k] != "conv"]
             if step in consumed:
                 skips.pop()
+            todo = [k for k, _ in terms if (step, k) not in done and cell.op_kinds[k] == "conv"]
             for k, j in terms:
                 if (step, k) in done or cell.op_kinds[k] != "conv":
                     continue
                 residual = None
                 if step not in written and skips:
                     residual = skips.pop()
+                kw = {}
+                if dn is not None and k == todo[-1]:
+                    kw = {"down": dslot[len(states)], "down_only": len(states) == n_states - 1}
                 self.conv(f"cells.{i}._ops.{k}", states[j], out=dst, accumulate=step in written,
-                          residual=residual)
+                          residual=residual, **kw)
                 written.add(step)
             for t in skips:
                 if step in written:
@@ -344,6 +370,7 @@
     SPLIT_S1_GROUP48 = os.environ.get("LEASTEREO_SPLIT_GROUP48", "1") != "0"
     PAIR_STEPS = WINOGRAD and os.environ.get("LEASTEREO_PAIR_STEPS", "0") != "0"
     FUSED_DOWN = os.environ.get("LEASTEREO_FUSED_DOWN", "1") != "0"
+    FUSED_DOWN_CELLS = os.environ.get("LEASTEREO_FUSED_DOWN_CELLS", "1") != "0"
 
     def run(self, x):
         return self._from_stem0(self.conv("stem0", x))
@@ -378,6 +405,45 @@
                 and cells[0].downup_sample < 0 and cells[0].dims == 3
                 and all(n % 2 == 0 and scale_dimension(n, 0.5) == n // 2 for n in vol))
 
+    def _conv1_takes_down(self, vol):
+        cells = self.m.cells
+        return (self.FUSED_DOWN_CELLS and self.tap is None and not isinstance(self, _C8Layout)
+                and len(cells) == 12 and "cells.5.share" in self.p
+                and cells[5].downup_sample < 0 and cells[5].dims == 3
+                and all(n % 2 == 0 and scale_dimension(n, 0.5) == n // 2 for n in vol))
+
+    def _cell_output_takes_down(self, i, size):
+        cells = self.m.cells
+        n = len(cells)
+        if not (self.FUSED_DOWN_CELLS and self.tap is None and not isinstance(self, _C8Layout)
+                and 0 <= i and i + 2 == n and not (n == 12 and i in (1, 4, 8))):
+            return False
+        cell, nxt = cells[i], cells[i + 1]
+        pre = self.p.get(f"cells.{i}.preprocess")
+        return (cell.dims == 3 and nxt.dims == 3
+                and nxt.downup_sample < 0 and f"cells.{i + 1}.share" not in self.p
+                and cell.downup_sample > 0 and f"cells.{i}.share" not in self.p
+                and pre is not None and pre.k == 1
+                and 2 + cell.steps - cell.block_multiplier == 1
+                and self.pair_steps.get(i) is None and self.s0_pair.get(i) is None
+                and all(cell.op_kinds[op] == "conv" for terms in cell.plan for op, _ in terms)
+                and all(self._finishing_op(i, step) is not None for step in range(len(cell.plan)))
+                and all(m % 2 == 0 and scale_dimension(m, 0.5) == m // 2 for m in size) and size[2] % 4 == 0)
+
+    def _finishing_op(self, i, step):
+        group = self.s1_group.get(i, [])
+        rest = [op for op, _ in self.m.cells[i].plan[step] if (step, op) not in group]
+        if not rest or self.p[f"cells.{i}._ops.{rest[-1]}"].wino is None:
+            return None
+        return rest[-1]
+
+    def _down_kernels_take(self, like, c, in_size, size):
+        b = like.shape[0]
+        return (like.is_cuda and like.dtype == torch.float32
+                and kernels.wino_preferred(b, c, c, *size)
+                and kernels.wino_dp_down2_kernel_name(b, c, c, *size) is not None
+                and kernels.resample_down2_shape_supported(in_size, size))
+
     def _cv_stem_pack(self, wl, wr):
         return kernels.pack_conv2d_weight(wl), kernels.pack_conv2d_weight(wr)
 
@@ -401,17 +467,30 @@
             self._emit("stem1", stem1)
         outs = []
         prev = (stem0, stem1)
+        cell_down = None
         n = len(self.m.cells)
         for i in range(n):
+            down = (stem0_down, stem1_down) if i == 0 else None
+            if cell_down is not None:
+                down = (None, cell_down)
             if i == 5 and n == 12:
-                fused = self.conv("conv1", outs[1][1], x2=outs[4][1])
-                self._emit("conv1", fused)
-                prev = (outs[4][0], fused)
+                pc, xa, xb = self.p["conv1"], outs[1][1], outs[4][1]
+                if (self._conv1_takes_down(self._volume(xa)) and pc.wino is not None
+                        and kernels.wino_preferred(xa.shape[0], pc.cout, pc.cin, *xa.shape[2:5])
+                        and kernels.conv3d_wino_down2_cat_supported(xa, xb, pc.cout)):
+                    down = (None, kernels.conv3d_bnrelu_wino_down2_cat(xa, xb, pc.wino, pc.cout, pc.scale,
+                                                                       pc.shift, pc.relu))
+                    prev = (outs[4][0], None)
+                else:
+                    fused = self.conv("conv1", xa, x2=xb)
+                    self._emit("conv1", fused)
+                    prev = (outs[4][0], fused)
             elif i == 9 and n == 12:
                 fused = self.conv("conv2", outs[4][1], x2=outs[8][1])
                 self._emit("conv2", fused)
                 prev = (outs[8][0], fused)
-            o = self.cell(i, prev[0], prev[1], down=(stem0_down, stem1_down) if i == 0 else None)
+            o = self.cell(i, prev[0], prev[1], down=down)
+            cell_down, self._cell_down = self._cell_down, None
             self._emit(f"cell{i}", o[1])
             outs.append(o)
             prev = o
diff --git a/leastereo_amd/kernels.py b/leastereo_amd/kernels.py
--- a/leastereo_amd/kernels.py
+++ b/leastereo_amd/kernels.py
@@ -407,6 +407,45 @@
         _stream()), "lea_resample3d_trilinear")
     _probe_end(rec)
     return out
+
+
+def resample_down2_shape_supported(in_size, size) -> bool:
+    return bool(_lib.load().lea_resample3d_down2_supported(*(int(n) for n in in_size), *(int(n) for n in size),
+                                                          LEA_F32))
+
+
+def resample_down2_supported(x: torch.Tensor, size) -> bool:
+    if not x.is_cuda or x.dtype != torch.float32 or x.dim() != 5:
+        return False
+    d, h, w = x.shape[2:]
+    if x.stride()[1:] != (d * h * w, h * w, w, 1):
+        return False
+    return resample_down2_shape_supported((d, h, w), size)
+
+
+def resample_trilinear_down2(x: torch.Tensor, size, out: torch.Tensor | None = None,
+                             down: torch.Tensor | None = None, scale: torch.Tensor | None = None,
+                             shift: torch.Tensor | None = None, relu: bool = False):
+    _require_cuda(x, out, down, scale, shift)
+    b, c, di, hi, wi = x.shape
+    do, ho, wo = (int(n) for n in size)
+    xbs = _check_volume_view(x, "x")
+    if out is None:
+        out = torch.empty((b, c, do, ho, wo), device=x.device, dtype=x.dtype)
+    if down is None:
+        down = torch.empty((b, c, do // 2, ho // 2, wo // 2), device=x.device, dtype=x.dtype)
+    if tuple(out.shape) != (b, c, do, ho, wo) or tuple(down.shape) != (b, c, do // 2, ho // 2, wo // 2):
+        raise ValueError(f"out / down shapes {tuple(out.shape)} / {tuple(down.shape)} for {(b, c, do, ho, wo)}")
+    ybs, dbs = _check_volume_view(out, "out"), _check_volume_view(down, "down")
+    rec = None if _probe is None else _probe_launch(
+        "resample3d_sep_down2_f32", 0.0, 4.0 * (x.numel() + out.numel() + down.numel()))
+    check(_lib.load().lea_resample3d_trilinear_down2(
+        x.data_ptr(), xbs, out.data_ptr(), ybs, down.data_ptr(), dbs, b, c, di, hi, wi, do, ho, wo,
+        scale.data_ptr() if scale is not None else None,
+        shift.data_ptr() if shift is not None else None, LEA_RELU if relu else 0, LEA_F32,
+        _stream()), "lea_resample3d_trilinear_down2")
+    _probe_end(rec)
+    return out, down
 
 
 def tapsum_upsample(q: torch.Tensor, cout: int, size, scale: torch.Tensor | None = None,
@@ -1398,43 +1437,147 @@
     return out
 
 
-def wino_down2_kernel_name(b, cin, cout, d, h, w):
-    name = _lib.load().lea_conv3d_wino_down2_kernel_name(b, cin, cout, d, h, w)
+def wino_down2_kernel_name(b, cin, cout, d, h, w, cin2=0):
+    lib = _lib.load()
+    if cin2:
+        name = lib.lea_conv3d_wino_down2_cat_kernel_name(b, cin, cin2, cout, d, h, w)
+    else:
+        name = lib.lea_conv3d_wino_down2_kernel_name(b, cin, cout, d, h, w)
     return name.decode() if name else None
 
 
 def conv3d_wino_down2_supported(x: torch.Tensor, cout: int) -> bool:
+    return _wino_down2_supported(x, cout, None)
+
+
+def conv3d_wino_down2_cat_supported(x: torch.Tensor, x2: torch.Tensor, cout: int) -> bool:
+    return _wino_down2_supported(x, cout, x2)
+
+
+def _wino_down2_supported(x, cout, x2):
+    for t in (x,) if x2 is None else (x, x2):
+        if not t.is_cuda or t.dtype != torch.float32 or t.dim() != 5:
+            return False
+        d, h, w = t.shape[2:]
+        if t.data_ptr() % 16 or t.stride(0) % 4 or t.stride()[1:] != (d * h * w, h * w, w, 1):
+            return False
+    b, cin, d, h, w = x.shape
+    if x2 is None:
+        return bool(_lib.load().lea_conv3d_wino_down2_supported(b, cin, cout, d, h, w))
+    if x2.shape[0] != b or tuple(x2.shape[2:]) != (d, h, w) or x2.device != x.device:
+        return False
+    return bool(_lib.load().lea_conv3d_wino_down2_cat_supported(b, cin + x2.shape[1], x2.shape[1], cout, d, h, w))
+
+
+def conv3d_bnrelu_wino_down2(x: torch.Tensor, packed: torch.Tensor, cout: int,
+                             scale: torch.Tensor | None, shift: torch.Tensor | None,
+                             relu: bool = True) -> torch.Tensor:
+    return _wino_down2(x, None, packed, cout, scale, shift, relu)
+
+
+def conv3d_bnrelu_wino_down2_cat(x: torch.Tensor, x2: torch.Tensor, packed: torch.Tensor, cout: int,
+                                 scale: torch.Tensor | None, shift: torch.Tensor | None,
+                                 relu: bool = True) -> torch.Tensor:
+    return _wino_down2(x, x2, packed, cout, scale, shift, relu)
+
+
+def _wino_down2(x, x2, packed, cout, scale, shift, relu):
+    _require_cuda(x, x2, packed, scale, shift)
+    b, cin, d, h, w = x.shape
+    xbs = _check_volume_view(x, "x")
+    cin2, x2bs = 0, 0
+    if x2 is not None:
+        if x2.shape[0] != b or tuple(x2.shape[2:]) != (d, h, w):
+            raise ValueError("x2 must match x in batch and volume")
+        cin2 = x2.shape[1]
+        x2bs = _check_volume_view(x2, "x2")
+    cin += cin2
+    out = torch.empty((b, cout, d // 2, h // 2, w // 2), device=x.device, dtype=x.dtype)
+    rec = None
+    if _probe is not None:
+        name = wino_down2_kernel_name(b, cin, cout, d, h, w, cin2) or (
+            "conv3d_wino44_down2_cat_kernel" if cin2 else "conv3d_wino44_down2_kernel")
+        rec = _probe_begin(b, cin, cout, d, h, w, 3, False, b * d * h * w, False, name=name,
+                           mfma_scale=wino_mfma_scale(cout, "conv3d_wino44_kernel"))
+        if rec is not None:
+            nbytes = 4.0 * (b * cin * d * h * w + out.numel()) + 4.0 * cout * cin * 27
+            rec = rec[:3] + (nbytes,) + rec[4:]
+    lib = _lib.load()
+    sp = scale.data_ptr() if scale is not None else None
+    hp = shift.data_ptr() if shift is not None else None
+    flags = LEA_RELU if relu else 0
+    if x2 is None:
+        check(lib.lea_conv3d_bnrelu_wino_down2(
+            x.data_ptr(), xbs, packed.data_ptr(), sp, hp,
+            out.data_ptr(), out.stride(0), b, cin, cout, d, h, w, flags, LEA_F32, _stream()),
+            "lea_conv3d_bnrelu_wino_down2")
+    else:
+        check(lib.lea_conv3d_bnrelu_wino_down2_cat(
+            x.data_ptr(), xbs, x2.data_ptr(), x2bs, cin2, packed.data_ptr(), sp, hp,
+            out.data_ptr(), out.stride(0), b, cin, cout, d, h, w, flags, LEA_F32, _stream()),
+            "lea_conv3d_bnrelu_wino_down2_cat")
+    _probe_end(rec)
+    return out
+
+
+def wino_dp_down2_kernel_name(b, cin, cout, d, h, w, only=False):
+    name = _lib.load().lea_conv3d_wino_dp_down2_kernel_name(b, cin, cout, d, h, w, 1 if only else 0)
+    return name.decode() if name else None
+
+
+def conv3d_wino_dp_down2_supported(x: torch.Tensor, cout: int) -> bool:
     if not x.is_cuda or x.dtype != torch.float32 or x.dim() != 5:
         return False
     b, cin, d, h, w = x.shape
     if x.data_ptr() % 16 or x.stride(0) % 4 or x.stride()[1:] != (d * h * w, h * w, w, 1):
         return False
-    return bool(_lib.load().lea_conv3d_wino_down2_supported(b, cin, cout, d, h, w))
-
-
-def conv3d_bnrelu_wino_down2(x: torch.Tensor, packed: torch.Tensor, cout: int,
-                             scale: torch.Tensor | None, shift: torch.Tensor | None,
-                             relu: bool = True) -> torch.Tensor:
-    _require_cuda(x, packed, scale, shift)
+    return bool(_lib.load().lea_conv3d_wino_dp_down2_supported(b, cin, cout, d, h, w))
+
+
+def conv3d_bnrelu_wino_dp_down2(x: torch.Tensor, packed: torch.Tensor, cout: int,
+                                scale: torch.Tensor | None, shift: torch.Tensor | None, relu: bool,
+                                out: torch.Tensor | None, down: torch.Tensor, accumulate: bool = False,
+                                residual: torch.Tensor | None = None, only: bool = False) -> torch.Tensor:
+    _require_cuda(x, packed, scale, shift, out, down, residual)
     b, cin, d, h, w = x.shape
     xbs = _check_volume_view(x, "x")
-    out = torch.empty((b, cout, d // 2, h // 2, w // 2), device=x.device, dtype=x.dtype)
+    if out is None:
+        if not only or accumulate:
+            raise ValueError("no out: the `only` form without accumulate")
+        ybs = 0
+    else:
+        out, ybs = _conv_out(x.shape, cout, (d, h, w), out, accumulate, x.device, x.dtype)
+    if tuple(down.shape) != (b, cout, d // 2, h // 2, w // 2):
+        raise ValueError(f"down shape {tuple(down.shape)} != {(b, cout, d // 2, h // 2, w // 2)}")
+    dbs = _check_volume_view(down, "down")
+    if accumulate:
+        rptr, rbs = _residual(out, True, residual, ybs)
+    elif residual is not None:
+        _require_cuda(residual)
+        if tuple(residual.shape) != (b, cout, d, h, w):
+            raise ValueError(f"residual shape {tuple(residual.shape)} != {(b, cout, d, h, w)}")
+        rptr, rbs = residual.data_ptr(), _check_volume_view(residual, "residual")
+    else:
+        rptr, rbs = None, 0
+    flags = (LEA_RELU if relu else 0) | (LEA_RESIDUAL if rptr is not None else 0)
     rec = None
     if _probe is not None:
-        name = wino_down2_kernel_name(b, cin, cout, d, h, w) or "conv3d_wino44_down2_kernel"
-        rec = _probe_begin(b, cin, cout, d, h, w, 3, False, b * d * h * w, False, name=name,
-                           mfma_scale=wino_mfma_scale(cout, "conv3d_wino44_kernel"))
+        name = wino_dp_down2_kernel_name(b, cin, cout, d, h, w, only) or "conv3d_wino_dp_down2_kernel"
+        rec = _probe_begin(b, cin, cout, d, h, w, 3, rptr is not None, b * d * h * w, False, name=name,
+                           mfma_scale=wino_mfma_scale(cout, wino_kernel_name(b, cout, d, h, w, cin=cin)))
         if rec is not None:
-            nbytes = 4.0 * (x.numel() + out.numel()) + 4.0 * cout * cin * 27
+            vox = b * cout * d * h * w
+            nbytes = 4.0 * (x.numel() + (vox if rptr is not None else 0) + (0 if only else vox) + down.numel()) \
+                + 4.0 * cout * cin * 27
             rec = rec[:3] + (nbytes,) + rec[4:]
-    check(_lib.load().lea_conv3d_bnrelu_wino_down2(
+    check(_lib.load().lea_conv3d_bnrelu_wino_dp_down2(
         x.data_ptr(), xbs, packed.data_ptr(),
         scale.data_ptr() if scale is not None else None,
         shift.data_ptr() if shift is not None else None,
-        out.data_ptr(), out.stride(0), b, cin, cout, d, h, w, LEA_RELU if relu else 0, LEA_F32, _stream()),
-        "lea_conv3d_bnrelu_wino_down2")
-    _probe_end(rec)
-    return out
+        rptr, rbs, None if only else out.data_ptr(), ybs, down.data_ptr(), dbs, b, cin, cout, d, h, w, flags,
+        LEA_F32, _stream()), "lea_conv3d_bnrelu_wino_dp_down2")
+    _probe_end(rec)
+    return down
 
 
 def conv3d_bnrelu_costvolume_wino(fl: torch.Tensor, fr: torch.Tensor, maxdisp: int,
```

After: 163.5 pairs/s, median of 6. +1.8%, better.
